# SingleRust/single-algebra

Hardware: AMD Instinct MI355X
Metric: sparse_pca_fit_transform_algorithmic_throughput (higher is better)
Workload: dtype f32

## Files before the change

### single-algebra_amd/csrc/common.h

```cpp
#pragma once
#include <hip/hip_runtime.h>

#include <atomic>
#include <cstdint>
#include <cstdio>
#include <stdexcept>
#include <string>
#include <utility>
#include <vector>

#include "../../include/sapca.h"
#include "switches.h"

namespace sapca {

struct Error : std::runtime_error {
  sapca_status code;
  Error(sapca_status c, const std::string& m) : std::runtime_error(m), code(c) {}
};

#define SAPCA_HIP(expr)                                                                        \
  do {                                                                                         \
    hipError_t e_ = (expr);                                                                    \
    if (e_ != hipSuccess)                                                                      \
      throw ::sapca::Error(SAPCA_ERR_HIP, std::string(#expr) + ": " + hipGetErrorString(e_)); \
  } while (0)

#define SAPCA_CHECK(cond, code, msg)                 \
  do {                                               \
    if (!(cond)) throw ::sapca::Error((code), (msg)); \
  } while (0)

inline int64_t round_up(int64_t x, int64_t q) { return (x + q - 1) / q * q; }

struct DevBuf {
  void* p = nullptr;
  size_t cap = 0;
  DevBuf() = default;
  DevBuf(const DevBuf&) = delete;
  DevBuf& operator=(const DevBuf&) = delete;
  ~DevBuf() { release(); }
  void release() {
    if (p) (void)hipFree(p);
    p = nullptr;
    cap = 0;
  }
  void* ensure(size_t bytes) {
    if (bytes > cap) {
      release();
      size_t want = bytes + bytes / 16 + 256;
      hipError_t e = hipMalloc(&p, want);
      if (e != hipSuccess) {
        p = nullptr;
        throw Error(SAPCA_ERR_NOMEM, std::string("hipMalloc(") + std::to_string(want) + "): " + hipGetErrorString(e));
      }
      cap = want;
    }
    return p;
  }
  template <typename U>
  U* as(size_t count) { return static_cast<U*>(ensure(count * sizeof(U))); }
  template <typename U>
  U* ptr() const { return static_cast<U*>(p); }
  bool contains(const void* q) const {
    const char* c = static_cast<const char*>(q);
    return p != nullptr && c >= static_cast<const char*>(p) && c < static_cast<const char*>(p) + cap;
  }
};

template <typename T>
struct CsrView {
  int64_t rows = 0, cols = 0, nnz = 0;
  const int64_t* ptr = nullptr;
  const int32_t* idx = nullptr;
  const T* val = nullptr;
};

struct LdsAttrState {
  std::atomic<int> bytes[64];
  LdsAttrState() { for (auto& b : bytes) b.store(0, std::memory_order_relaxed); }
};
inline void ensure_dynamic_lds(const void* kernel, size_t bytes, LdsAttrState& state) {
  int dev = 0;
  SAPCA_HIP(hipGetDevice(&dev));
  std::atomic<int>& have = state.bytes[dev & 63];
  if (have.load(std::memory_order_acquire) >= (int)bytes) return;
  SAPCA_HIP(hipFuncSetAttribute(kernel, hipFuncAttributeMaxDynamicSharedMemorySize, (int)bytes));
  have.store((int)bytes, std::memory_order_release);
}

struct PinnedBuf {
  void* p = nullptr;
  size_t cap = 0;
  PinnedBuf() = default;
  PinnedBuf(const PinnedBuf&) = delete;
  PinnedBuf& operator=(const PinnedBuf&) = delete;
  ~PinnedBuf() {
    if (p) (void)hipHostFree(p);
  }
  void* ensure(size_t bytes) {
    if (bytes > cap) {
      if (p) (void)hipHostFree(p);
      p = nullptr;
      cap = 0;
      hipError_t e = hipHostMalloc(&p, bytes, hipHostMallocDefault);
      if (e != hipSuccess) {
        p = nullptr;
        throw Error(SAPCA_ERR_NOMEM, std::string("hipHostMalloc(") + std::to_string(bytes) + "): " + hipGetErrorString(e));
      }
      cap = bytes;
    }
    return p;
  }
};

struct TiledOp {
  bool valid = false;
  int64_t rows = 0, cols = 0, total_entries = 0;
  int ldp = 0;
  int elem = 4;
  int tc = 0, nct = 0;
  int nrb = 0;
  int block_rows = 0;
  int nsplit = 1, tiles_per_split = 0;
  int tile_bytes = 0;
  int64_t max_chunk = 0;
  const int32_t* blk_row0 = nullptr;
  int64_t mid_row0 = -1;
  const uint32_t* row_perm = nullptr;
  const int64_t* chunk_off = nullptr;
  const uint32_t* wave_off = nullptr;
  const uint8_t* steps = nullptr;
  const void* ent = nullptr;
  bool dq = false;
  const uint32_t* dq_info = nullptr;
};
struct TiledBuffers {
  DevBuf blk, steps, wave_off, chunk_off, ent, tmp, misc, perm, lens, dq_info, bounds;
  DevBuf seg;
  DevBuf quad_off;
  DevBuf raw;
  PinnedBuf host;
  hipStream_t aux = nullptr;
  hipEvent_t aux_fork = nullptr, aux_join = nullptr;
  TiledBuffers() = default;
  TiledBuffers(const TiledBuffers&) = delete;
  TiledBuffers& operator=(const TiledBuffers&) = delete;
  ~TiledBuffers() {
    if (aux) { (void)hipStreamSynchronize(aux); (void)hipStreamDestroy(aux); }
    if (aux_fork) (void)hipEventDestroy(aux_fork);
    if (aux_join) (void)hipEventDestroy(aux_join);
  }
};

struct Stream {
  hipStream_t s = nullptr;
  bool owned = false;
};

struct EventTimer {
  bool enabled = false;
  hipStream_t s = nullptr;
  std::vector<hipEvent_t> pool;
  size_t used = 0;
  std::vector<std::pair<int, int>> spans;
  int last_closed = -1;
  void begin_collect(hipStream_t st, bool on) {
    enabled = on;
    s = st;
    used = 0;
    spans.clear();
    last_closed = -1;
  }
  int record() {
    if (used == pool.size()) {
      hipEvent_t e;
      SAPCA_HIP(hipEventCreate(&e));
      pool.push_back(e);
    }
    SAPCA_HIP(hipEventRecord(pool[used], s));
    return (int)used++;
  }
  int start() {
    if (!enabled) return -1;
    spans.emplace_back(record(), -1);
    return (int)spans.size() - 1;
  }
  int start_behind_last() {
    if (!enabled) return -1;
    if (last_closed < 0) return start();
    spans.emplace_back(spans[(size_t)last_closed].second, -1);
    return (int)spans.size() - 1;
  }
  void stop(int i) {
    if (i < 0) return;
    spans[(size_t)i].second = record();
    last_closed = i;
  }
  double ms(int i) {
    if (i < 0 || spans[(size_t)i].second < 0) return 0.0;
    float t = 0;
    SAPCA_HIP(hipEventElapsedTime(&t, pool[(size_t)spans[(size_t)i].first], pool[(size_t)spans[(size_t)i].second]));
    return t;
  }
  ~EventTimer() {
    for (hipEvent_t e : pool) (void)hipEventDestroy(e);
  }
};

}
```

### single-algebra_amd/csrc/engine.cpp

```cpp
#include "engine.h"

#include <algorithm>
#include <chrono>
#include <cmath>
#include <cstring>
#include <exception>
#include <memory>
#include <thread>

#include "lanczos.h"
#include "small_svd.h"
#include "spmm_dq.h"

namespace sapca {

namespace {

template <typename T>
int staged_sweep_ldp(int64_t rows, int64_t cols, double entries, int64_t l, int spmm_variant) {
  if (spmm_variant == 1 || rows <= 0 || cols <= 0 || l < 1 || l > k::kMaxPanelWidth) return 0;
  const int ldp = 64;
  const double row_bytes = (double)ldp * sizeof(T);
  const double tile_bytes = 80.0 * 1024.0, block_rows = row_bytes == 256.0 ? 512.0 : 256.0;
  const double chunks = std::ceil((double)rows / block_rows) * std::ceil((double)cols * row_bytes / tile_bytes);
  double floor_entries = sizeof(T) == 4 ? 1e7 : 5e6;
  if (const char* e = dbg_env("SAPCA_TILED_MIN_ENTRIES")) floor_entries = atof(e);
  const bool dense_enough = entries * (sizeof(T) == 4 ? 64.0 : 96.0) >= chunks * tile_bytes && entries >= floor_entries;
  return (spmm_variant == 2 || dense_enough) ? ldp : 0;
}

enum Cat { C_PREPARE, C_STATS, C_SPMM, C_SPMMT, C_ORTHO, C_SMALL, C_LANCZOS, C_TRANSFORM, C_COMM, C_COUNT };

struct Scope {
  sapca_handle_s& h;
  int ev;
  Scope(sapca_handle_s& h_, int cat, bool behind_last = false) : h(h_), ev(behind_last ? h_.timer.start_behind_last() : h_.timer.start()) {
    if (ev >= 0) h.spans.emplace_back(cat, ev);
  }
  ~Scope() {
    try { h.timer.stop(ev); } catch (...) {}
  }
};

void collect_timings(sapca_handle_s& h, bool is_fit) {
  if (!h.timer.enabled) return;
  sapca_timings& t = h.timings;
  if (is_fit) {
    const double keep_upload = t.upload_ms;
    const uint64_t keep_steps = t.lanczos_steps;
    std::memset(&t, 0, sizeof(t));
    t.upload_ms = keep_upload;
    t.lanczos_steps = keep_steps;
  } else {
    t.transform_ms = 0;
    for (int ev : h.held_small.in_transform) t.transform_ms -= h.timer.ms(ev);
  }
  double comm_dev_ms = 0;
  for (auto& sp : h.spans) {
    if (is_fit == (sp.first == C_TRANSFORM)) continue;
    const double ms = h.timer.ms(sp.second);
    switch (sp.first) {
      case C_PREPARE: t.prepare_ms += ms; break;
      case C_STATS: t.stats_ms += ms; break;
      case C_SPMM:
        t.spmm_ms += ms;
        if (t.n_spmm < 32) t.spmm_sweep_ms[t.n_spmm] = ms;
        t.n_spmm++;
        break;
      case C_SPMMT:
        t.spmmt_ms += ms;
        if (t.n_spmmt < 32) t.spmmt_sweep_ms[t.n_spmmt] = ms;
        t.n_spmmt++;
        break;
      case C_ORTHO: t.ortho_ms += ms; break;
      case C_SMALL: t.small_svd_ms += ms; break;
      case C_LANCZOS: t.lanczos_ms += ms; break;
      case C_TRANSFORM: t.transform_ms += ms; break;
      case C_COMM: comm_dev_ms += ms; break;
      default: break;
    }
  }
  if (is_fit) t.comm_ms = comm_dev_ms > 0 ? comm_dev_ms : h.comm.host_ms;
}

using H = sapca_handle_s;

void lazy_stream(hipStream_t& st, hipEvent_t& a, hipEvent_t& b) {
  if (st) return;
  SAPCA_HIP(hipStreamCreateWithFlags(&st, hipStreamNonBlocking));
  SAPCA_HIP(hipEventCreateWithFlags(&a, hipEventDisableTiming));
  SAPCA_HIP(hipEventCreateWithFlags(&b, hipEventDisableTiming));
}
hipStream_t side_stream(H& h) { lazy_stream(h.stream2, h.ev_fork, h.ev_join); return h.stream2; }
hipStream_t stats_stream(H& h) { lazy_stream(h.stream3, h.ev_kept, h.ev_stats); return h.stream3; }
void order_after(hipStream_t later, hipEvent_t ev, hipStream_t earlier) {
  SAPCA_HIP(hipEventRecord(ev, earlier));
  SAPCA_HIP(hipStreamWaitEvent(later, ev, 0));
}
double* stats_dev(H& h, int64_t n) { return h.stats.as<double>((size_t)3 * n + 1 + H::kStatsTail); }
int panel_ld(int k, int ldp) { return k > 128 ? (int)round_up(k, 64) : std::max(ldp, k <= 64 ? 64 : 128); }

template <typename T>
H::PrepKey prep_key_of(const H& h, const CsrView<T>& A) {
  H::PrepKey key;
  key.ptr = A.ptr; key.idx = A.idx; key.val = A.val;
  key.m = (uint64_t)A.rows; key.n = (uint64_t)A.cols; key.nnz = (uint64_t)A.nnz;
  key.mask_version = h.mask_version; key.dtype = Engine<T>::kDtype; key.valid = true;
  return key;
}

int32_t* upload_o2m(H& h, std::vector<int32_t>& o2m32) {
  const size_t n = h.orig_to_masked.size();
  o2m32.resize(n);
  for (size_t j = 0; j < n; ++j) o2m32[j] = (int32_t)h.orig_to_masked[j];
  int32_t* d_o2m = h.o2m_dev.as<int32_t>(std::max<size_t>(n, 1));
  SAPCA_HIP(hipMemcpyAsync(d_o2m, o2m32.data(), n * sizeof(int32_t), hipMemcpyHostToDevice, h.stream));
  return d_o2m;
}
template <typename T>
H::RawCsr compact_a(H& h, const CsrView<T>& A, const int32_t* d_o2m, int64_t n_used, int32_t* drop_col = nullptr,
                    T* drop_val = nullptr, unsigned long long* amax_bits = nullptr) {
  const CsrBuf<T> ca = csr_buffers<T>(h.ca_ptr, h.ca_idx, h.ca_val, A.rows, A.nnz);
  int64_t nnz_used = 0;
  k::compact_columns(A, d_o2m, ca.ptr, ca.idx, ca.val, &nnz_used, h.scratch, h.stream, drop_col, drop_val, amax_bits);
  return ca.raw(A.rows, n_used, nnz_used);
}

enum class AtFrom { Nothing, FormatFromA, FormatFromCompacted, CompactedTransposed, Transposed };
enum class StatsFrom { Upload, Scatter, FormatBuild, KeptAndDropped, Transposed };
enum class StatsTo { AllReduce, MainCopy, SideChain, ScatterSide };

struct PrepPlan {
  int64_t m = 0, n = 0, nnz = 0, n_used = 0;
  bool masked = false;
  int tiled_ldp = 0;
  int at_nct = 0;
  AtFrom at = AtFrom::Transposed;
  StatsFrom stats = StatsFrom::Transposed;
  StatsTo deliver = StatsTo::MainCopy;
};

template <typename T>
struct PrepOutcome {
  int64_t nnz_used = 0;
  bool at_direct = false;
  bool a_aside = false, ok_a = false;
  CsrView<T> At;
  const uint64_t* at_packed = nullptr;
  bool at_seg_ready = false;
};

struct MaskMaps {
  std::vector<int32_t> o2m32, sel;
  int32_t *d_o2m = nullptr, *d_sel = nullptr;
};

struct Aside {
  std::thread t;
  std::exception_ptr err;
  ~Aside() { if (t.joinable()) t.join(); }
  void join() { if (t.joinable()) t.join(); if (err) std::rethrow_exception(err); }
};

template <typename T>
PrepPlan plan_preparation(H& h, const CsrView<T>& A) {
  PrepPlan p;
  const int64_t m = p.m = A.rows, n = p.n = A.cols, nnz = p.nnz = A.nnz;
  p.masked = !h.mask.empty();
  const int64_t n_used = p.n_used = p.masked ? (int64_t)std::count_if(h.mask.begin(), h.mask.end(), [](uint8_t b) { return b != 0; }) : n;
  if (h.opt.method == SAPCA_RANDOM && m > 0 && n > 0 && n_used > 0) {
    const int64_t l = std::min<int64_t>((int64_t)(h.opt.n_components + h.opt.n_oversamples), std::min<int64_t>(m, n_used));
    p.tiled_ldp = staged_sweep_ldp<T>(m, n_used, (double)nnz * ((double)n_used / (double)n), l, h.opt.spmm_variant);
  }
  const bool at_tile_major = p.tiled_ldp != 0 && dbg_env("SAPCA_AT_NATURAL") == nullptr;
  p.at_nct = at_tile_major ? k::tiled_tile_count(m, p.tiled_ldp * (int)sizeof(T) / 4) : 0;

  bool from_upload = h.up_stats.valid && A.ptr == h.in_ptr.p && A.idx == h.in_idx.p && A.val == h.in_val.p &&
                     h.up_stats.m == (uint64_t)m && h.up_stats.n == (uint64_t)n && h.up_stats.nnz == (uint64_t)nnz &&
                     h.up_stats.dtype == Engine<T>::kDtype && n > 0 && !h.comm.active();
  if (from_upload) {
    SAPCA_HIP(hipEventSynchronize(h.up_stats_done));
    if (*static_cast<const int*>(h.up_stats.flag.p) != 0) h.up_stats.valid = from_upload = false;
  }
  const bool lz_scatter = h.opt.method == SAPCA_LANCZOS && n_used > 0 && n_used <= m && m >= 4096 && nnz > 0 &&
                          k::scatter_fits(n_used) && dbg_env("SAPCA_LANCZOS_TRANSPOSE") == nullptr;
  const bool bucket_route = sizeof(T) == 4 && at_tile_major;
  if (lz_scatter) p.at = AtFrom::Nothing;
  else if (!p.masked) p.at = bucket_route ? AtFrom::FormatFromA : AtFrom::Transposed;
  else p.at = bucket_route && n_used <= 65536 && dbg_env("SAPCA_AT_SORT") == nullptr ? AtFrom::FormatFromCompacted : AtFrom::CompactedTransposed;

  p.stats = from_upload ? StatsFrom::Upload : lz_scatter ? StatsFrom::Scatter : p.masked ? StatsFrom::KeptAndDropped
            : p.at == AtFrom::FormatFromA ? StatsFrom::FormatBuild : StatsFrom::Transposed;
  if (h.comm.active()) p.deliver = StatsTo::AllReduce;
  else if (p.stats == StatsFrom::Scatter) p.deliver = StatsTo::ScatterSide;
  else if (p.stats == StatsFrom::KeptAndDropped && dbg_env("SAPCA_MASK_STATS_INLINE") == nullptr) p.deliver = StatsTo::SideChain;
  return p;
}

void mask_maps(H& h, const PrepPlan& p, MaskMaps& maps) {
  h.cols_to_use.clear();
  h.orig_to_masked.clear();
  h.has_mask_maps = p.masked;
  if (!p.masked) return;
  h.orig_to_masked.assign((size_t)p.n, -1);
  for (int64_t j = 0; j < p.n; ++j)
    if (h.mask[(size_t)j]) {
      h.orig_to_masked[(size_t)j] = (int64_t)h.cols_to_use.size();
      h.cols_to_use.push_back((uint64_t)j);
    }
  if (p.n_used == 0) throw Error(SAPCA_ERR_SVD, "SVD computation failed: the mask selects no feature");
  maps.sel.assign(h.cols_to_use.begin(), h.cols_to_use.end());
  maps.d_o2m = upload_o2m(h, maps.o2m32);
  maps.d_sel = h.sel_rows_dev.as<int32_t>((size_t)p.n_used);
  SAPCA_HIP(hipMemcpyAsync(maps.d_sel, maps.sel.data(), (size_t)p.n_used * sizeof(int32_t), hipMemcpyHostToDevice, h.stream));
}

template <typename T>
void drop_sums(H& h, const PrepPlan& p, int64_t nnz_used, double* dst) {
  const CsrBuf<T> work = csr_buffers<T>(h.at_ptr, h.at_idx, h.at_val, p.n, p.nnz);
  k::sums_by_column(h.drop_col.ptr<int32_t>(), h.drop_val.ptr<T>(), p.nnz - nnz_used, p.n, work.ptr, work.idx, work.val, dst,
                    dst + p.n, h.drop_tmp, h.stream3);
}

template <typename T>
void compact_and_drop_sums(H& h, const CsrView<T>& A, const PrepPlan& p, const MaskMaps& maps, PrepOutcome<T>& out) {
  hipStream_t s = h.stream;
  Scope sc(h, C_PREPARE);
  const bool pairs = p.stats == StatsFrom::KeptAndDropped;
  const size_t cap = (size_t)std::max<int64_t>(p.nnz, 1);
  h.a_used = compact_a(h, A, maps.d_o2m, p.n_used, pairs ? h.drop_col.as<int32_t>(cap) : nullptr, pairs ? h.drop_val.as<T>(cap) : nullptr,
                       p.at == AtFrom::Nothing ? h.lz_scalars.as<unsigned long long>(4) : nullptr);
  out.nnz_used = h.a_used.nnz;
  if (!pairs) return;
  hipStream_t s3 = stats_stream(h);
  if (!h.ev_drop) SAPCA_HIP(hipEventCreateWithFlags(&h.ev_drop, hipEventDisableTiming));
  double* d_stats = stats_dev(h, p.n);
  SAPCA_HIP(hipMemsetAsync(d_stats + 2 * p.n, 0, (size_t)p.n * sizeof(double), s));
  if (p.deliver != StatsTo::SideChain) {
    order_after(s3, h.ev_drop, s);
    drop_sums<T>(h, p, out.nnz_used, d_stats);
    SAPCA_HIP(hipEventRecord(h.ev_drop, s3));
  } else if (h.opt.method != SAPCA_RANDOM) {
    double* d_drop = h.drop_stats.as<double>((size_t)2 * p.n);
    order_after(s3, h.ev_drop, s);
    drop_sums<T>(h, p, out.nnz_used, d_drop);
  }
}

template <typename T>
void start_a_format_aside(H& h, const CsrView<T>& A, const PrepPlan& p, PrepOutcome<T>& out, Aside& aside) {
  side_stream(h);
  SAPCA_HIP(hipEventRecord(h.ev_fork, h.stream));
  h.tiled_a = TiledOp();
  out.a_aside = true;
  const CsrView<T> src = p.masked ? Engine<T>::view(h.a_used) : A;
  aside.t = std::thread([&h, &p, &out, &aside, src] {
    try {
      SAPCA_HIP(hipSetDevice(h.device));
      SAPCA_HIP(hipStreamWaitEvent(h.stream2, h.ev_fork, 0));
      if (p.tiled_ldp != 0) out.ok_a = k::build_tiled(src, p.tiled_ldp, h.tiled_a, h.tb_a, h.stream2, k::QuadSource::csr());
      SAPCA_HIP(hipEventRecord(h.ev_join, h.stream2));
    } catch (...) {
      aside.err = std::current_exception();
    }
  });
}

void scatter_kept_sums(H& h, const PrepPlan& p, const double* d_part, const int32_t* d_sel) {
  double* d_stats = stats_dev(h, p.n);
  if (p.deliver != StatsTo::SideChain) SAPCA_HIP(hipStreamWaitEvent(h.stream, h.ev_drop, 0));
  k::scatter_pairs(d_part, d_part + p.n_used, d_sel, p.n_used, d_stats, d_stats + p.n, h.stream);
}

template <typename T>
void at_format_direct(H& h, const CsrView<T>& A, const PrepPlan& p, const MaskMaps& maps, PrepOutcome<T>& out) {
  if constexpr (sizeof(T) == 4) {
    if (p.masked && out.nnz_used <= 0) return;
    Scope sc(h, C_PREPARE);
    const CsrView<T> src = p.masked ? Engine<T>::view(h.a_used) : A;
    int64_t* t_ptr = (p.masked ? h.cat_ptr : h.at_ptr).template as<int64_t>((size_t)src.cols + 1);
    double* d_sums = p.masked ? h.scratch2.as<double>((size_t)2 * p.n_used + 2) : stats_dev(h, p.n);
    h.tiled_at = TiledOp();
    out.at_direct = k::build_tiled_at_direct(src, p.tiled_ldp, h.tiled_at, h.tb_at, t_ptr,
                                             p.stats == StatsFrom::Upload ? nullptr : d_sums, h.scratch, h.stream);
    if (!out.at_direct) return;
    if (!p.masked) out.At = CsrView<T>{p.n, p.m, p.nnz, t_ptr, nullptr, nullptr};
    else h.at_used = {p.n_used, p.m, out.nnz_used, t_ptr, nullptr, nullptr};
    if (p.stats == StatsFrom::KeptAndDropped) scatter_kept_sums(h, p, d_sums, maps.d_sel);
  }
}

template <typename T>
void at_transpose(H& h, const CsrView<T>& A, const PrepPlan& p, const MaskMaps& maps, PrepOutcome<T>& out) {
  Scope sc(h, C_PREPARE);
  if (p.masked) {
    const CsrBuf<T> cat = csr_buffers<T>(h.cat_ptr, h.cat_idx, h.cat_val, p.n_used, p.nnz);
    k::transpose_csr(Engine<T>::view(h.a_used), cat.ptr, cat.idx, cat.val, h.scratch, h.stream, p.at_nct, nullptr);
    h.at_used = cat.raw(p.n_used, p.m, out.nnz_used);
    if (p.stats != StatsFrom::KeptAndDropped) return;
    double* d_part = h.scratch2.as<double>((size_t)2 * p.n_used + 2);
    k::row_sums(Engine<T>::view(h.at_used), d_part, d_part + p.n_used, h.stream);
    scatter_kept_sums(h, p, d_part, maps.d_sel);
  } else {
    const CsrBuf<T> at = csr_buffers<T>(h.at_ptr, h.at_idx, h.at_val, p.n, p.nnz);
    k::transpose_csr(A, at.ptr, at.idx, at.val, h.scratch, h.stream, p.at_nct,
                     (p.at_nct != 0 && dbg_env("SAPCA_AT_UNPACK") == nullptr) ? &out.at_packed : nullptr);
    out.At = CsrView<T>{p.n, p.m, p.nnz, at.ptr, at.idx, at.val};
  }
}

template <typename T>
void column_statistics(H& h, const CsrView<T>& A, const PrepPlan& p, PrepOutcome<T>& out) {
  hipStream_t s = h.stream;
  const int64_t m = p.m, n = p.n;
  double* sums = static_cast<double*>(h.stats_host.ensure(((size_t)2 * n + 1) * sizeof(double)));
  {
    Scope sc(h, C_STATS);
    double* d_stats = stats_dev(h, n);
    switch (p.stats == StatsFrom::FormatBuild && !out.at_direct ? StatsFrom::Transposed : p.stats) {
      case StatsFrom::Upload:
        SAPCA_HIP(hipMemcpyAsync(d_stats, h.up_stats.out.p, (size_t)3 * n * sizeof(double), hipMemcpyDeviceToDevice, s));
        break;
      case StatsFrom::Scatter: {
        const bool side = p.deliver == StatsTo::ScatterSide;
        hipStream_t st = side ? stats_stream(h) : s;
        if (side) order_after(st, h.ev_kept, s);
        k::colstats_scatter(A, h.lz_scalars.ptr<unsigned long long>(), d_stats, d_stats + n, d_stats + 2 * n, side ? h.drop_tmp : h.scratch, st);
        if (side) {
          SAPCA_HIP(hipMemcpyAsync(sums, d_stats, (size_t)2 * n * sizeof(double), hipMemcpyDeviceToHost, st));
          SAPCA_HIP(hipEventRecord(h.ev_stats, st));
        }
        break;
      }
      case StatsFrom::FormatBuild:
        k::row_lengths_f64(out.At.ptr, n, d_stats + 2 * n, s);
        break;
      case StatsFrom::KeptAndDropped: break;
      case StatsFrom::Transposed:
        if constexpr (sizeof(T) == 4) {
          if (out.at_packed) {
            k::at_stats_index(out.At.ptr, out.at_packed, n, m, p.tiled_ldp, h.tb_at, d_stats, d_stats + n, s);
            out.at_seg_ready = true;
          }
        }
        if (!out.at_seg_ready) k::row_sums(out.At, d_stats, d_stats + n, s);
        k::row_lengths_f64(out.At.ptr, n, d_stats + 2 * n, s);
        break;
    }
    sums[(size_t)2 * n] = (double)m;
    h.stats_on_side = p.deliver == StatsTo::SideChain || p.deliver == StatsTo::ScatterSide;
    if (p.deliver == StatsTo::MainCopy) {
      SAPCA_HIP(hipMemcpyAsync(sums, d_stats, (size_t)2 * n * sizeof(double), hipMemcpyDeviceToHost, s));
    } else if (p.deliver == StatsTo::AllReduce) {
      double* tail = h.stats_tail;
      const uint32_t nr = h.comm.nranks;
      const bool ride = Engine<T>::vote_rides(h);
      const size_t ntail = 1 + (ride ? (size_t)nr + 1 : 0);
      std::fill(tail, tail + ntail, 0.0);
      tail[0] = (double)m;
      if (ride && h.tiled_at.valid) {
        tail[1] = 1.0;
        tail[2 + h.comm.rank] = (double)Engine<T>::piece_vote(h, h.tiled_at.ldp);
      }
      SAPCA_HIP(hipMemcpyAsync(d_stats + 3 * n, tail, ntail * sizeof(double), hipMemcpyHostToDevice, s));
      { Scope cs(h, C_COMM); h.comm.allreduce(d_stats, (uint64_t)3 * n + ntail, 1, s); }
      SAPCA_HIP(hipMemcpyAsync(sums, d_stats, (size_t)2 * n * sizeof(double), hipMemcpyDeviceToHost, s));
      SAPCA_HIP(hipMemcpyAsync(tail, d_stats + 3 * n, ntail * sizeof(double), hipMemcpyDeviceToHost, s));
    }
  }
  h.stats_cols = n;
  h.vote_ready = false;
  if (p.deliver == StatsTo::AllReduce) {
    SAPCA_HIP(hipStreamSynchronize(s));
    sums[(size_t)2 * n] = h.stats_tail[0];
    if (Engine<T>::vote_rides(h) && (uint32_t)std::llround(h.stats_tail[1]) == h.comm.nranks) {
      h.vote_cut = (int64_t)*std::min_element(h.stats_tail + 2, h.stats_tail + 2 + h.comm.nranks);
      h.vote_ready = true;
    }
    h.m_global = (uint64_t)std::llround(sums[(size_t)2 * n]);
    h.stats_pending = false;
    Engine<T>::finish_statistics(h);
  } else {
    h.m_global = (uint64_t)m;
    h.stats_pending = true;
  }
}

template <typename T>
void build_formats(H& h, const PrepPlan& p, PrepOutcome<T>& out, Aside& aside) {
  hipStream_t s = h.stream;
  if (!out.a_aside) h.tiled_a = TiledOp();
  if (!out.at_direct) h.tiled_at = TiledOp();
  if (p.tiled_ldp == 0) return;
  Scope sc(h, C_PREPARE);
  const CsrView<T> at = Engine<T>::view(h.at_used);
  bool ok_at = out.at_direct;
  const k::QuadSource at_rows = p.at_nct != 0 ? k::QuadSource::tile_major() : k::QuadSource::csr();
  if constexpr (sizeof(T) == 4) {
    if (!ok_at)
      ok_at = k::build_tiled(at, p.tiled_ldp, h.tiled_at, h.tb_at, s,
                             out.at_packed ? k::QuadSource::tile_major_packed(out.at_packed, out.at_seg_ready) : at_rows);
    if (out.at_packed && !ok_at) {
      k::unpack_transposed(out.at_packed, p.nnz, const_cast<int32_t*>(out.At.idx), const_cast<float*>(out.At.val), s);
      out.at_packed = nullptr;
      ok_at = k::build_tiled(at, p.tiled_ldp, h.tiled_at, h.tb_at, s, at_rows);
    }
  } else {
    ok_at = k::build_tiled(at, p.tiled_ldp, h.tiled_at, h.tb_at, s, at_rows);
  }
  aside.join();
  const bool ok_a = out.ok_a;
  ok_at = ok_at && ok_a;
  if (h.opt.verbose)
    fprintf(stderr, "sapca: tile-major formats%s: A %s (nrb %d, nct %d, split %d, %lld entries), A^T %s (nrb %d, nct %d, split %d, %lld entries)\n",
            sizeof(T) == 8 ? " (f64)" : "", ok_a ? "ok" : "no", h.tiled_a.nrb, h.tiled_a.nct, h.tiled_a.nsplit,
            (long long)h.tiled_a.total_entries, ok_at ? "ok" : "no", h.tiled_at.nrb, h.tiled_at.nct, h.tiled_at.nsplit,
            (long long)h.tiled_at.total_entries);
  if (ok_a && ok_at) return;
  h.tiled_a = TiledOp();
  h.tiled_at = TiledOp();
  if (out.at_direct) {
    const CsrView<T> src = Engine<T>::view(h.a_used);
    const CsrBuf<T> t = p.masked ? csr_buffers<T>(h.cat_ptr, h.cat_idx, h.cat_val, src.cols, p.nnz)
                                 : csr_buffers<T>(h.at_ptr, h.at_idx, h.at_val, src.cols, p.nnz);
    k::transpose_csr(src, t.ptr, t.idx, t.val, h.scratch, s, 0, nullptr);
    h.at_used = t.raw(src.cols, src.rows, src.nnz);
  }
}

template <typename T>
void queue_side_statistics(H& h, const PrepPlan& p, const PrepOutcome<T>& out, const MaskMaps& maps) {
  const int64_t n = p.n;
  double* d_stats = stats_dev(h, n);
  double* d_drop = h.drop_stats.as<double>((size_t)2 * n);
  order_after(h.stream3, h.ev_kept, h.stream);
  if (h.opt.method == SAPCA_RANDOM) drop_sums<T>(h, p, out.nnz_used, d_drop);
  k::copy_selected(d_stats, d_stats + n, maps.d_sel, p.n_used, d_drop, d_drop + n, h.stream3);
  SAPCA_HIP(hipMemcpyAsync(h.stats_host.p, d_drop, (size_t)2 * n * sizeof(double), hipMemcpyDeviceToHost, h.stream3));
  SAPCA_HIP(hipEventRecord(h.ev_stats, h.stream3));
}

}

template <typename T>
void Engine<T>::prepare(H& h, const CsrView<T>& A) {
  hipStream_t s = h.stream;
  if (!h.mask.empty() && (int64_t)h.mask.size() != A.cols)
    throw Error(SAPCA_ERR_MASK_LEN, "The mask vector length and the number of features (columns) have to be the same!");
  h.prep_key.valid = false;
  if (h.stream3) SAPCA_HIP(hipStreamSynchronize(h.stream3));
  h.stats_pending = false;
  h.stats_on_side = false;
  h.lz_scatter = false;

  const PrepPlan p = plan_preparation(h, A);
  const bool lz_scatter = p.at == AtFrom::Nothing;
  PrepOutcome<T> out;
  MaskMaps maps;
  Aside aside;
  mask_maps(h, p, maps);
  if (lz_scatter && !p.masked) {
    k::absmax(A.val, p.nnz, h.lz_scalars.as<unsigned long long>(4), s);
  }
  h.lz_scatter = lz_scatter;
  if (p.masked) compact_and_drop_sums(h, A, p, maps, out);
  if (p.masked || p.at == AtFrom::FormatFromA) start_a_format_aside(h, A, p, out, aside);
  if (p.at == AtFrom::FormatFromA || p.at == AtFrom::FormatFromCompacted) at_format_direct(h, A, p, maps, out);
  const bool a_aside_late = p.tiled_ldp != 0 && !out.a_aside;
  if (a_aside_late) order_after(side_stream(h), h.ev_fork, s);
  if (!lz_scatter && !out.at_direct) at_transpose(h, A, p, maps, out);
  if (a_aside_late) {
    h.tiled_a = TiledOp();
    out.ok_a = k::build_tiled(A, p.tiled_ldp, h.tiled_a, h.tb_a, h.stream2, k::QuadSource::csr());
    SAPCA_HIP(hipEventRecord(h.ev_join, h.stream2));
    out.a_aside = true;
  }

  column_statistics(h, A, p, out);
  if (!p.masked) {
    h.a_used = {p.m, p.n, p.nnz, A.ptr, A.idx, A.val};
    h.at_used = {p.n, p.m, p.nnz, out.At.ptr, out.At.idx, out.At.val};
  } else if (lz_scatter) {
    h.at_used = {p.n_used, p.m, out.nnz_used, nullptr, nullptr, nullptr};
  }

  build_formats(h, p, out, aside);
  aside.join();
  if (out.a_aside) SAPCA_HIP(hipStreamWaitEvent(s, h.ev_join, 0));
  if (p.deliver == StatsTo::SideChain) queue_side_statistics(h, p, out, maps);

  h.prep_key = prep_key_of(h, A);
}

template <typename T>
void Engine<T>::finish_statistics(H& h) {
  const int64_t n = h.stats_cols;
  const double* sums = static_cast<const double*>(h.stats_host.p);
  const double mg = (double)h.m_global;
  const bool masked = h.has_mask_maps;
  h.prep_mean.assign((size_t)n, 0.0);
  h.prep_total_var = 0;
  if (h.opt.center) {
    for (int64_t j = 0; j < n; ++j) h.prep_mean[(size_t)j] = (double)(T)(sums[(size_t)j] / mg);
    auto var_of = [&](int64_t j) {
      const double mean = sums[(size_t)j] / mg;
      return (sums[(size_t)n + j] - mean * sums[(size_t)j]) / (mg - 1.0);
    };
    if (masked) for (uint64_t j : h.cols_to_use) h.prep_total_var += var_of((int64_t)j);
    else for (int64_t j = 0; j < n; ++j) h.prep_total_var += var_of(j);
  }
  h.q3_cancels = false;
  if (h.opt.center && masked)
    for (uint64_t j : h.cols_to_use) {
      const double sj = sums[(size_t)j], qj = sums[(size_t)n + j];
      if (qj > 0 && sj * sj > 0.25 * mg * qj) { h.q3_cancels = true; break; }
    }
  h.stats_pending = false;
}

template <typename T>
void Engine<T>::normalize(H& h, T* P, int64_t rows, int l, int ld, int normalizer, bool sharded, const NormalizeExtras<T>& x) {
  hipStream_t s = h.stream;
  if (normalizer == SAPCA_NORM_NONE) {
    if (x.src) k::materialize(P, rows, ld, *x.src, s);
    if (x.vec_out) k::weighted_colsum(P, rows, ld, x.w, x.vec_out, h.scratch2, s);
    return;
  }
  Scope sc(h, C_ORTHO, x.behind_sweep);
  const SmallLayout lay(h.small, ld);
  double *G = lay.gram(), *wsum = x.vec_out ? lay.wsum() : nullptr;
  const int passes = x.passes > 0 ? x.passes : (normalizer == SAPCA_NORM_QR ? 2 : 1);
  for (int pass = 0; pass < passes; ++pass) {
    k::gram(P, rows, ld, G, h.scratch2, s, pass == 0 ? x.src : nullptr, x.w, wsum);
    if (sharded && h.comm.active()) { Scope cs(h, C_COMM); h.comm.allreduce(G, (uint64_t)ld * ld, 1, s); }
    double* Rout = pass == 0 ? x.R1 : x.R2;
    k::chol_inv(G, l, ld, Rout ? Rout : lay.r_scratch(), lay.r_inv(), lay.info(), s, wsum,
                sizeof(T) == 4 ? reinterpret_cast<float*>(x.vec_out) : nullptr, sizeof(T) == 8 ? reinterpret_cast<double*>(x.vec_out) : nullptr);
    T* Q = ld <= 128 ? P : h.panel_wide.as<T>((size_t)std::max<int64_t>(rows, 1) * ld);
    k::panel_gemm(P, rows, ld, lay.r_inv(), ld, Q, s, true);
    if (Q != P) SAPCA_HIP(hipMemcpyAsync(P, Q, (size_t)rows * ld * sizeof(T), hipMemcpyDeviceToDevice, s));
  }
}

template <typename T>
bool Engine<T>::vote_rides(const H& h) {
  return sizeof(T) == 4 && h.comm.active() && h.opt.method == SAPCA_RANDOM && h.opt.spmm_variant != 1 &&
         (size_t)h.comm.nranks + 2 <= H::kStatsTail;
}

template <typename T>
int64_t Engine<T>::piece_vote(H& h, int ld) {
  const char* ov = getenv("SAPCA_AT_OVERLAP");
  const bool enabled = ov != nullptr ? atoi(ov) != 0 : h.comm.mode != Comm::RCCL;
  if (!enabled || !h.comm.has_side_lane() || !k::spmm_tiled_pieces_ok(h.tiled_at, 2, ld)) return 0;
  std::vector<int64_t> b;
  k::spmm_tiled_piece_bounds(h.tiled_at, 2, b, h.stream);
  return b[1];
}

namespace {

enum class AtSweep { OnePiece, TwoPieces };
enum class SmallSvd { GramHost, GramHostHeldBack, GramDevice, QrJacobi };

struct AtPieces {
  AtSweep sweep = AtSweep::OnePiece;
  int64_t cut = 0, r1 = 0;
  int wgs = 240;
};
struct RandomizedPlan {
  int64_t m = 0, n_used = 0;
  int l = 0, ld = 0, k = 0, ldk = 0, q = 0;
  int norm = 0, variant = 0;
  bool center = false, tiled = false;
  bool cov = false;
  bool scale = false;
  SmallSvd small = SmallSvd::GramHost;
  AtPieces at;
};

template <typename T>
struct FitPanels {
  T *X, *Y;
  SmallLayout lay;
  const T* mu;
  T *cvec, *sv;
  bool cvec_current = false;
  k::PanelSource<T> src;
  const T *d = nullptr, *dmu = nullptr;
};

template <typename T>
RandomizedPlan plan_randomized(H& h) {
  RandomizedPlan p;
  p.m = h.a_used.rows; p.n_used = h.a_used.cols;
  p.k = (int)h.opt.n_components; p.ldk = (int)round_up(p.k, 16);
  const int64_t l_req = (int64_t)h.opt.n_components + (int64_t)h.opt.n_oversamples;
  p.l = (int)std::min<int64_t>(l_req, std::min<int64_t>((int64_t)h.m_global, p.n_used));
  SAPCA_CHECK(p.l <= k::kMaxPanelWidth, SAPCA_ERR_ARG, "n_components + n_oversamples above 1024 is not supported");
  p.tiled = h.tiled_a.valid && h.tiled_at.valid;
  p.ld = (p.l > 128 || p.tiled || h.comm.active()) ? panel_ld(p.l, p.tiled ? h.tiled_a.ldp : 0) : (int)round_up(p.l, 16);
  p.q = (int)h.opt.n_power_iterations; p.norm = h.opt.normalizer;
  p.cov = h.covar.active();
  p.scale = h.scale_fit != 0;
  p.center = h.opt.center != 0 && !p.cov;
  p.variant = h.opt.spmm_variant;
  p.small = sizeof(T) == 8 ? SmallSvd::QrJacobi : k::sym_eig_device_ok(p.l) ? SmallSvd::GramDevice
            : h.held_small.defer ? SmallSvd::GramHostHeldBack : SmallSvd::GramHost;
  return p;
}

template <typename T>
AtPieces agree_on_at_pieces(H& h, const RandomizedPlan& p) {
  AtPieces at;
  h.at_sweep_pieces = 1u;
  if (sizeof(T) != 4 || !h.comm.active() || p.variant == 1) return at;
  hipStream_t s = h.stream;
  const bool mine = h.tiled_at.valid && k::spmm_tiled_pieces_ok(h.tiled_at, 2, p.ld);
  if (h.vote_ready) {
    at.cut = h.vote_cut;
    SAPCA_CHECK(at.cut == 0 || mine, SAPCA_ERR_COMM, "internal: the ranks agreed on a two-piece A^T sweep this rank cannot run");
  } else {
    const uint32_t nr = h.comm.nranks;
    std::vector<double> votes((size_t)nr, 0.0);
    votes[h.comm.rank] = mine ? (double)Engine<T>::piece_vote(h, p.ld) : 0.0;
    double* d_votes = h.votes.as<double>(nr);
    SAPCA_HIP(hipMemcpyAsync(d_votes, votes.data(), nr * sizeof(double), hipMemcpyHostToDevice, s));
    h.comm.allreduce(d_votes, nr, 1, s);
    SAPCA_HIP(hipMemcpyAsync(votes.data(), d_votes, nr * sizeof(double), hipMemcpyDeviceToHost, s));
    SAPCA_HIP(hipStreamSynchronize(s));
    at.cut = (int64_t)*std::min_element(votes.begin(), votes.end());
  }
  if (!mine || at.cut <= 0 || at.cut >= p.n_used) return at;
  std::vector<int64_t> piece_rows;
  k::spmm_tiled_piece_bounds(h.tiled_at, 2, piece_rows, s);
  at.sweep = AtSweep::TwoPieces;
  at.r1 = piece_rows[1];
  h.at_sweep_pieces = 2u;
  hipDeviceProp_t pr;
  if (hipGetDeviceProperties(&pr, h.device) == hipSuccess) at.wgs = std::max(16, pr.multiProcessorCount - 16);
  lazy_stream(h.stream_comm, h.ev_piece, h.ev_comm);
  return at;
}

template <typename T>
void load_omega(H& h, const RandomizedPlan& p, FitPanels<T>& f) {
  hipStream_t s = h.stream;
  if (h.omega.empty()) {
    k::gaussian_panel(f.X, p.n_used, p.l, p.ld, h.opt.random_seed, s);
    return;
  }
  SAPCA_CHECK((int64_t)h.omega_rows == p.n_used && (int64_t)h.omega_cols >= p.l, SAPCA_ERR_ARG,
              "injected Omega must be (features seen by the SVD) x (n_components + n_oversamples)");
  std::vector<T> tmp((size_t)p.n_used * p.l);
  for (int64_t r = 0; r < p.n_used; ++r)
    for (int j = 0; j < p.l; ++j) tmp[(size_t)r * p.l + j] = (T)h.omega[(size_t)r * h.omega_cols + j];
  T* stage = h.scratch2.as<T>(tmp.size());
  SAPCA_HIP(hipMemcpyAsync(stage, tmp.data(), tmp.size() * sizeof(T), hipMemcpyHostToDevice, s));
  k::add_padding(stage, p.n_used, p.l, f.X, p.ld, s);
  SAPCA_HIP(hipStreamSynchronize(s));
}

template <typename T>
void sweep_a(H& h, const RandomizedPlan& p, FitPanels<T>& f, bool behind_normalize) {
  hipStream_t s = h.stream;
  if (p.scale) {
    Scope sc(h, C_ORTHO, behind_normalize);
    k::scale_panel_rows(f.X, p.n_used, p.ld, f.d, s);
  }
  if (p.center && !f.cvec_current) {
    k::weighted_colsum(f.X, p.n_used, p.ld, f.mu, f.cvec, h.scratch2, s);
    behind_normalize = false;
  }
  f.cvec_current = false;
  Scope sc(h, C_SPMM, behind_normalize);
  k::spmm(Engine<T>::view(h.a_used), &h.tiled_a, f.X, p.ld, f.Y, p.ld, p.ld, p.center ? f.cvec : nullptr, p.variant, h.split_scratch, s);
}

template <typename T>
double* covar_s(H& h, int ld) { return h.covar_s.as<double>((size_t)k::kCovarCols * (size_t)std::max(ld, 16)); }

template <typename T>
void covar_basis_sweep(H& h, const RandomizedPlan& p, FitPanels<T>& f) {
  hipStream_t s = h.stream;
  constexpr int kq = k::kCovarCols;
  T* Q = h.covar_q.as<T>((size_t)p.m * kq);
  SAPCA_HIP(hipMemcpyAsync(Q, h.covar.q_t.data(), (size_t)p.m * kq * sizeof(T), hipMemcpyHostToDevice, s));
  T* Gp = h.panel_xs.as<T>(((size_t)std::max<int64_t>(p.n_used, 1) + 1) * p.ld);
  T* G = h.covar_g.as<T>((size_t)p.n_used * kq);
  k::add_padding(Q, p.m, kq, f.Y, p.ld, s);
  {
    Scope sc(h, C_SPMMT);
    k::spmm(Engine<T>::view(h.at_used), &h.tiled_at, f.Y, p.ld, Gp, p.ld, p.ld, (const T*)nullptr, p.variant, h.split_scratch, s);
  }
  k::strip_padding(Gp, p.n_used, p.ld, kq, G, s);
  if (p.scale) k::scale_panel_rows(G, p.n_used, kq, f.d, s);
}

template <typename T>
void covar_model_products(H& h, const RandomizedPlan& p) {
  hipStream_t s = h.stream;
  constexpr int kq = k::kCovarCols;
  Scope sc(h, C_ORTHO);
  const int ldc = (int)round_up(p.k, p.k > 128 ? 64 : 16);
  h.covar.ldc = ldc;
  T* W = h.panel_w.as<T>((size_t)std::max<int64_t>(p.n_used, 1) * ldc);
  double* C = h.covar_c.as<double>((size_t)kq * ldc);
  double* GG = covar_s<T>(h, kq);
  const T* G = h.covar_g.ptr<T>();
  k::scaled_transpose(h.components_dev.ptr<T>(), p.n_used, p.k, nullptr, W, ldc, s);
  k::panel_qt_y(W, G, p.n_used, ldc, C, h.scratch2, s);
  k::panel_qt_y(G, G, p.n_used, kq, GG, h.scratch2, s);
  void* host = h.covar_host.ensure((size_t)kq * kq * sizeof(double));
  SAPCA_HIP(hipMemcpyAsync(host, GG, (size_t)kq * kq * sizeof(double), hipMemcpyDeviceToHost, s));
}

template <typename T>
void covar_project(H& h, const RandomizedPlan& p, FitPanels<T>& f, bool behind_at) {
  Scope sc(h, C_ORTHO);
  double* S = covar_s<T>(h, p.ld);
  k::panel_qt_y(f.Y, h.covar_q.ptr<T>(), p.m, p.ld, S, h.scratch2, h.stream);
  if (behind_at) k::panel_sub_qs(f.X, h.covar_g.ptr<T>(), p.n_used, p.ld, p.ld, S, p.ld, h.stream);
  else k::panel_sub_qs(f.Y, h.covar_q.ptr<T>(), p.m, p.ld, p.ld, S, p.ld, h.stream);
}

template <typename T>
void sweep_at_one_piece(H& h, const RandomizedPlan& p, FitPanels<T>& f, bool behind_normalize) {
  hipStream_t s = h.stream;
  f.src = k::PanelSource<T>();
  {
    Scope sc(h, C_SPMMT, behind_normalize);
    k::spmm(Engine<T>::view(h.at_used), &h.tiled_at, f.Y, p.ld, f.X, p.ld, p.ld, (const T*)nullptr, p.variant, h.split_scratch, s,
            h.comm.active() || p.cov ? nullptr : &f.src);
  }
  if (!f.src.parts) { f.src.parts = f.X; f.src.nsplit = 1; }
  if (h.comm.active()) {
    Scope cs(h, C_COMM);
    h.comm.allreduce(f.X, (uint64_t)p.n_used * p.ld + (p.center ? (uint64_t)p.ld : 0), Engine<T>::kDtype, s);
  }
  if (p.center) { f.src.mu = f.mu; f.src.sv = f.sv; }
}

template <typename T>
void sweep_at_two_pieces(H& h, const RandomizedPlan& p, FitPanels<T>& f) {
  if constexpr (sizeof(T) == 4) {
    hipStream_t s = h.stream;
    const int64_t cut = p.at.cut, r1 = p.at.r1;
    f.src = k::PanelSource<T>();
    {
      Scope sc(h, C_SPMMT);
      k::spmm_tiled_piece(h.tiled_at, 0, 2, p.at.wgs, 0, r1, f.Y, p.ld, f.X, p.ld, p.ld, h.split_scratch, s);
      SAPCA_HIP(hipEventRecord(h.ev_piece, s));
      k::spmm_tiled_piece(h.tiled_at, 1, 2, p.at.wgs, r1, p.n_used - r1, f.Y, p.ld, f.X, p.ld, p.ld, h.split_scratch2, s);
    }
    Scope cs(h, C_COMM);
    SAPCA_HIP(hipStreamWaitEvent(h.stream_comm, h.ev_piece, 0));
    h.comm.allreduce(f.X, (uint64_t)cut * p.ld, Engine<T>::kDtype, h.stream_comm, 1);
    SAPCA_HIP(hipEventRecord(h.ev_comm, h.stream_comm));
    h.comm.allreduce(f.X + (size_t)cut * p.ld, (uint64_t)(p.n_used - cut) * p.ld + (p.center ? (uint64_t)p.ld : 0), Engine<T>::kDtype, s);
    SAPCA_HIP(hipStreamWaitEvent(s, h.ev_comm, 0));
    f.src.parts = f.X; f.src.nsplit = 1;
    if (p.center) { f.src.mu = f.mu; f.src.sv = f.sv; }
  }
}

template <typename T>
void sweep_at(H& h, const RandomizedPlan& p, FitPanels<T>& f, bool behind_normalize) {
  p.at.sweep == AtSweep::TwoPieces ? sweep_at_two_pieces(h, p, f) : sweep_at_one_piece(h, p, f, behind_normalize);
  if (p.scale) {
    Scope sc(h, C_ORTHO);
    k::finish_scaled_panel(f.X, p.n_used, p.ld, f.src, f.d, h.stream);
    f.src = k::PanelSource<T>();
    f.src.parts = f.X; f.src.nsplit = 1;
  }
  if (p.cov) covar_project(h, p, f, true);
}

template <typename T>
void power_iterations(H& h, const RandomizedPlan& p, FitPanels<T>& f) {
  using Extras = NormalizeExtras<T>;
  T* const sv_out = p.center ? f.sv : nullptr;
  const bool y_behind = !p.cov, x_behind = !p.cov && !p.scale && !h.comm.active() && p.at.sweep != AtSweep::TwoPieces;
  const bool normalises = p.norm != SAPCA_NORM_NONE;
  for (int it = 0; it < p.q; ++it) {
    sweep_a(h, p, f, it > 0 && normalises);
    if (p.cov) covar_project(h, p, f, false);
    Engine<T>::normalize(h, f.Y, p.m, p.l, p.ld, p.norm, true, Extras{.passes = 1, .vec_out = sv_out, .behind_sweep = y_behind});
    sweep_at(h, p, f, normalises);
    Engine<T>::normalize(h, f.X, p.n_used, p.l, p.ld, p.norm, false,
                         Extras{.passes = 1, .src = &f.src, .w = p.scale ? f.dmu : f.mu, .vec_out = p.center ? f.cvec : nullptr,
                                .behind_sweep = x_behind});
    f.cvec_current = p.center;
  }
  sweep_a(h, p, f, p.q > 0 && normalises);
  if (p.cov) covar_project(h, p, f, false);
  Engine<T>::normalize(h, f.Y, p.m, p.l, p.ld, SAPCA_NORM_QR, true, Extras{.vec_out = sv_out, .behind_sweep = y_behind});
  sweep_at(h, p, f, true);
}

template <typename T>
void rotate_into_components(H& h, int ld, const double* Mdev, const double** sign_out = nullptr) {
  const int k = (int)h.opt.n_components, ldk = (int)round_up(k, 16);
  const int64_t n_used = h.a_used.cols;
  T* VtT = h.panel_w.as<T>((size_t)std::max<int64_t>(n_used, 1) * ldk);
// ... 144 lines not shown
    h.sing.assign(sv.begin(), sv.begin() + k);
    h.chol_regularised = info_host;
  } catch (...) {
    if (deferred) {
      h.fitted = false;
      h.held_tail.pending = false;
    }
    throw;
  }
}

template <typename T>
void Engine<T>::fit_lanczos(H& h, bool centred) {
  Scope sc(h, C_LANCZOS);
  lanczos_fit<T>(h, centred);
}

void covar_check(H& h, uint64_t m, bool fit, bool then_transform) {
  const bool set = !h.covar_z.empty();
  const bool model = h.covar.model.design > 0;
  if (!fit) {
    if (!h.fitted || (!set && !model)) return;
    SAPCA_CHECK(model, SAPCA_ERR_ARG, "transform: covariates are set, but the model was fitted without covariates");
    SAPCA_CHECK(set, SAPCA_ERR_ARG, "transform: the model was fitted with covariates, but none are set");
    SAPCA_CHECK(h.covar_cols == h.covar.model.cols, SAPCA_ERR_ARG,
                "transform: covariates have " + std::to_string(h.covar_cols) + " columns, the fitted model's " + std::to_string(h.covar.model.cols));
  }
  if (!set) return;
  SAPCA_CHECK(!h.comm.active(), SAPCA_ERR_ARG, "covariates are not supported on a handle that belongs to a communicator");
  SAPCA_CHECK(h.opt.method == SAPCA_RANDOM, SAPCA_ERR_ARG, "covariates need SVDMethod::Random");
  SAPCA_CHECK(!(then_transform || !fit) || h.opt.transform_semantics == SAPCA_TRANSFORM_CENTERED, SAPCA_ERR_ARG,
              "covariates need SAPCA_TRANSFORM_CENTERED: the reference's transform semantics have no meaning on residuals");
  SAPCA_CHECK(h.covar_rows == m, SAPCA_ERR_ARG,
              "covariates have " + std::to_string(h.covar_rows) + " rows, the matrix " + std::to_string(m));
}

void scale_check(H& h, uint64_t m, uint64_t n, bool fit, bool then_transform) {
  const int mode = fit ? h.scale_mode : (h.fitted ? h.scale_model : 0);
  if (mode == SAPCA_SCALE_NONE) return;
  if (fit) {
    SAPCA_CHECK(h.opt.method == SAPCA_RANDOM, SAPCA_ERR_ARG, "column scaling needs SVDMethod::Random");
    if (mode == SAPCA_SCALE_WEIGHTS)
      SAPCA_CHECK(h.scale_weights.size() == n, SAPCA_ERR_ARG,
                  "column scaling has " + std::to_string(h.scale_weights.size()) + " weights, the matrix " + std::to_string(n) + " columns");
    if (mode == SAPCA_SCALE_UNIT_VARIANCE) {
      SAPCA_CHECK(m >= 2 || h.comm.active(), SAPCA_ERR_ARG,
                  "column scaling: unit variance needs at least two rows, the matrix has " + std::to_string(m));
      SAPCA_CHECK(h.covar_z.empty(), SAPCA_ERR_ARG,
                  "column scaling: unit variance of covariate residuals is not supported (" + std::to_string(h.covar_cols) +
                      " covariate columns are set): pass explicit weights");
    }
  }
  SAPCA_CHECK(!(then_transform || !fit) || h.opt.transform_semantics == SAPCA_TRANSFORM_CENTERED, SAPCA_ERR_ARG,
              "column scaling needs SAPCA_TRANSFORM_CENTERED: the reference's transform semantics have no meaning on scaled columns");
}

namespace {

template <typename T>
void column_scale_factors(H& h, int64_t n_used) {
  hipStream_t s = h.stream;
  const int64_t n = h.stats_cols;
  const double* weights = nullptr;
  if (h.scale_fit == SAPCA_SCALE_WEIGHTS) {
    double* w = h.scale_in.as<double>((size_t)std::max<int64_t>(n, 1));
    SAPCA_HIP(hipMemcpyAsync(w, h.scale_weights.data(), (size_t)n * sizeof(double), hipMemcpyHostToDevice, s));
    weights = w;
  }
  const size_t cap = (size_t)std::max<int64_t>(n_used, 1), parts = k::column_scale_partials(n_used);
  double* red = h.scale_red.as<double>(parts + 1);
  const double* stats = h.stats.ptr<double>();
  k::column_scale_factors<T>(stats, stats + n, (double)h.m_global, h.has_mask_maps ? h.sel_rows_dev.ptr<int32_t>() : nullptr, weights, n_used,
                             h.scale_d64.as<double>(cap), h.scale_dt.as<T>(cap), h.scale_w.as<T>(cap), red, red + parts, s);
  void* host = h.scale_host.ensure(sizeof(double));
  SAPCA_HIP(hipMemcpyAsync(host, red + parts, sizeof(double), hipMemcpyDeviceToHost, s));
}

template <typename T>
void covar_fit_basis(H& h) {
  constexpr size_t kq = k::kCovarCols;
  H::Covar& c = h.covar;
  c.fit = {};
  if (h.covar_z.empty()) return;
  const size_t m = (size_t)h.covar_rows, design = (size_t)h.covar_cols + (h.opt.center ? 1 : 0);
  c.q.resize(m * kq);
  c.w.resize(design * kq);
  uint64_t rank = 0;
  SAPCA_CHECK(sapca_covariate_basis(h.covar_z.data(), h.covar_rows, h.covar_cols, h.opt.center ? 1 : 0, c.q.data(), c.w.data(), &rank) == SAPCA_OK,
              SAPCA_ERR_ARG, "covariates: the design matrix was refused");
  c.fit = {h.covar_cols, (uint64_t)design, rank};
  c.q_t.resize(m * kq * sizeof(T));
  T* qt = reinterpret_cast<T*>(c.q_t.data());
  for (size_t i = 0; i < m * kq; ++i) qt[i] = (T)c.q[i];
}

template <typename T>
void covar_rows_basis(H& h) {
  constexpr size_t kq = k::kCovarCols;
  H::Covar& c = h.covar;
  const size_t m = (size_t)h.covar_rows, cols = (size_t)h.covar_cols, off = h.opt.center ? 1 : 0;
  c.q_t.resize(m * kq * sizeof(T));
  T* qt = reinterpret_cast<T*>(c.q_t.data());
  for (size_t i = 0; i < m; ++i)
    for (size_t j = 0; j < kq; ++j) {
      double acc = off ? c.w_model[j] : 0.0;
      for (size_t t = 0; t < cols; ++t) acc += h.covar_z[i * cols + t] * c.w_model[(off + t) * kq + j];
      qt[i * kq + j] = (T)acc;
    }
}

void covar_finish_fit(H& h) {
  constexpr size_t kq = k::kCovarCols;
  H::Covar& c = h.covar;
  if (c.fit.design == 0) return;
  c.w_model = c.w;
  if (!c.active() || !h.opt.center) return;
  const double* GG = static_cast<const double*>(h.covar_host.p);
  const double* sums = static_cast<const double*>(h.stats_host.p);
  const size_t n = (size_t)h.stats_cols;
  double raw = 0, taken = 0;
  const bool scaled = h.scale_model == SAPCA_SCALE_WEIGHTS && h.scale_weights.size() == n;
  auto moment = [&](size_t j) { return scaled ? h.scale_weights[j] * h.scale_weights[j] * sums[n + j] : sums[n + j]; };
  if (h.has_mask_maps) for (uint64_t j : h.cols_to_use) raw += moment((size_t)j);
  else for (size_t j = 0; j < n; ++j) raw += moment(j);
  for (size_t i = 0; i < kq; ++i) taken += GG[i * kq + i];
  h.total_var = (raw - taken) / (double)(h.m_fit - 1);
}

}

template <typename T>
void Engine<T>::fit(H& h, const CsrView<T>& A, bool defer_finish) {
  hipStream_t s = h.stream;
  covar_check(h, (uint64_t)A.rows, true, false);
  scale_check(h, (uint64_t)A.rows, (uint64_t)A.cols, true, false);
  h.scale_fit = h.scale_mode;
  h.held_tail.reset();
  h.held_small.reset();
  covar_fit_basis<T>(h);
  {
    const double lw = (double)(h.opt.n_components + h.opt.n_oversamples) <= 64 ? 64.0 : 128.0;
    h.held_small.defer = defer_finish && h.mask.empty() && h.opt.method == SAPCA_RANDOM && sizeof(T) == 4 &&
                         (h.comm.active() || (double)A.rows * lw * lw <= 400e3 * 64.0 * 64.0) && !h.covar.active() && h.scale_fit == 0;
  }
  h.spans.clear();
  h.comm.host_ms = 0;
  h.timer.begin_collect(s, h.opt.collect_timings != 0);
  const int total_ev = h.timer.start();
  h.fitted = false;
  h.timings.lanczos_steps = 0;
  SAPCA_CHECK(h.opt.n_components > 0, SAPCA_ERR_ARG, "n_components must be positive");
  SAPCA_CHECK(A.rows > 0 && A.cols > 0, SAPCA_ERR_ARG, "empty matrix");
  prepare(h, A);
  const int64_t n_used = h.a_used.cols;
  if ((int64_t)h.opt.n_components > std::min<int64_t>((int64_t)h.m_global - (int64_t)h.covar.fit.rank, n_used))
    throw Error(SAPCA_ERR_SVD, std::string(h.opt.method == SAPCA_RANDOM ? "Randomized SVD" : "SVD") +
                                   " computation failed: n_components exceeds the matrix dimensions");
  SAPCA_CHECK(h.m_global >= 2, SAPCA_ERR_ARG, "need at least two samples");

  auto device_means = [&] {
    T* d_mu = h.mean_used_dev.as<T>((size_t)n_used);
    if (h.opt.center)
      k::mean_from_sums(h.stats.ptr<double>(), (double)h.m_global, h.has_mask_maps ? h.sel_rows_dev.ptr<int32_t>() : nullptr, n_used, d_mu, s);
    else
      SAPCA_HIP(hipMemsetAsync(d_mu, 0, (size_t)n_used * sizeof(T), s));
  };

  if (h.opt.method == SAPCA_RANDOM) {
    device_means();
    if (h.scale_fit) column_scale_factors<T>(h, n_used);
    fit_randomized(h);
  } else {
    const bool centred = h.opt.lanczos_center != 0 && h.opt.center != 0;
    const bool sums_on_side = h.lz_scatter && h.stats_on_side;
    const bool means_first = !sums_on_side || centred;
    if (sums_on_side && centred) SAPCA_HIP(hipStreamWaitEvent(s, h.ev_stats, 0));
    if (means_first) device_means();
    if (centred)
      k::mean_from_sums(h.stats.ptr<double>(), (double)h.m_global, h.has_mask_maps ? h.sel_rows_dev.ptr<int32_t>() : nullptr, n_used,
                        h.lz_mu.as<double>((size_t)n_used), s);
    fit_lanczos(h, centred);
    if (!means_first) {
      SAPCA_HIP(hipStreamWaitEvent(s, h.ev_stats, 0));
      device_means();
    }
  }

  h.k = h.opt.n_components;
  h.n_used = (uint64_t)n_used;
  h.n_cols = (uint64_t)A.cols;
  h.m_fit = h.m_global;
  h.dtype = kDtype;
  h.fitted = true;
  h.scale_model = h.scale_fit;
  h.covar.model = h.covar.fit;
  h.timer.stop(total_ev);
  h.held_tail.total_ev = total_ev;
  h.held_tail.pending = true;
  if (!defer_finish || !h.mask.empty() || h.covar.fit.design > 0) finish_fit(h);
}

namespace {

template <typename T>
void describe_sweeps(H& h) {
  const int64_t n_used = (int64_t)h.n_used;
  const double l = (double)std::min<uint64_t>(h.opt.n_components + h.opt.n_oversamples, std::min<uint64_t>(h.m_global, (uint64_t)n_used));
  h.timings.bytes_per_sweep = (double)h.a_used.nnz * (sizeof(T) + 4) + ((double)h.a_used.rows + 1) * 8 +
                              (double)n_used * l * sizeof(T) + (double)h.a_used.rows * l * sizeof(T);
  const bool tiled = h.opt.method == SAPCA_RANDOM && h.tiled_a.valid && h.tiled_at.valid;
  h.timings.sweep_kernel = !tiled ? 0u : (k::dq_usable(h.tiled_a, 64) && k::dq_usable(h.tiled_at, 64) && h.opt.spmm_variant != 1 ? 2u : 1u);
  h.timings.at_sweep_pieces = h.opt.method == SAPCA_RANDOM ? h.at_sweep_pieces : 0u;
  h.timings.sweep_slots_a = tiled ? (uint64_t)h.tiled_a.total_entries : 0;
  h.timings.sweep_slots_at = tiled ? (uint64_t)h.tiled_at.total_entries : 0;
}

}

template <typename T>
void Engine<T>::finish_fit(H& h) {
  if (!h.held_tail.pending) return;
  if (h.held_small.pending) finish_small_svd(h, nullptr);
  h.held_tail.pending = false;
  hipStream_t s = h.stream;
  const int total_ev = h.held_tail.total_ev;
  if (h.held_tail.sing_l) {
    const int l = h.held_tail.sing_l;
    h.held_tail.sing_l = 0;
    SAPCA_HIP(hipStreamSynchronize(s));
    const double* host = static_cast<const double*>(h.small_host.p);
    const int* host_i = reinterpret_cast<const int*>(host + l);
    bool finite = true;
    for (int i = 0; i < l; ++i) finite = finite && std::isfinite(host[i]);
    if ((host_i[0] & 1) || (host_i[0] & 2) || !finite) {
      h.fitted = false;
      throw Error(SAPCA_ERR_SVD, (host_i[0] & 1) ? "Randomized SVD computation failed: eigensolver did not converge"
                                                 : "Randomized SVD computation failed: non-finite singular value");
    }
    if (h.opt.verbose) fprintf(stderr, "sapca: device eigensolver of the %d x %d Gram: %d sweeps\n", l, l, host_i[1]);
    h.sing.assign(host, host + h.k);
    h.chol_regularised = host_i[2];
  }
  if (h.stats_pending) {
    SAPCA_HIP(hipStreamSynchronize(s));
    if (h.stats_on_side) SAPCA_HIP(hipEventSynchronize(h.ev_stats));
    finish_statistics(h);
  }
  h.mean = h.prep_mean;
  const double nm1 = (double)(h.m_fit - 1);
  h.expl_var.resize(h.k);
  for (uint64_t i = 0; i < h.k; ++i) {
    const T sv = (T)h.sing[i];
    h.expl_var[i] = (double)(T)((T)(sv * sv) / (T)nm1);
  }
  if (h.opt.center) {
    h.total_var = h.prep_total_var;
  } else {
    h.total_var = 0;
    for (uint64_t i = 0; i < h.k; ++i) h.total_var += h.expl_var[i];
  }
  SAPCA_HIP(hipStreamSynchronize(s));
  if (h.scale_model && h.opt.center) h.total_var = *static_cast<const double*>(h.scale_host.p);
  covar_finish_fit(h);
  collect_timings(h, true);
  if (total_ev >= 0) h.timings.fit_total_ms = h.timer.ms(total_ev);
  describe_sweeps<T>(h);
}

namespace {

template <typename T>
struct Projection {
  CsrView<T> Au;
  const TiledOp* top = nullptr;
  int ldk = 0;
  double* d_cnt = nullptr;
  bool prepared = false;
};

template <typename T>
Projection<T> select_projection_operator(H& h, const CsrView<T>& A) {
  hipStream_t s = h.stream;
  const int k = (int)h.k;
  const bool masked = !h.mask.empty(), ref_sem = h.opt.transform_semantics == SAPCA_TRANSFORM_REFERENCE;
  Projection<T> pr;
  pr.ldk = (int)round_up(k, 16);
  pr.prepared = h.prep_key == prep_key_of(h, A);
  if (pr.prepared) {
    if (h.tiled_a.valid && k <= k::kMaxPanelWidth) pr.top = &h.tiled_a;
    pr.Au = Engine<T>::view(h.a_used);
    pr.d_cnt = h.stats.ptr<double>() + 2 * A.cols;
  } else if (masked) {
    h.prep_key.valid = false;
    std::vector<int32_t> o2m32;
    pr.Au = Engine<T>::view(compact_a(h, A, upload_o2m(h, o2m32), (int64_t)h.n_used));
  } else {
    pr.Au = A;
    if (ref_sem) {
      h.prep_key.valid = false;
      pr.d_cnt = stats_dev(h, A.cols) + 2 * A.cols;
      k::column_counts_f64(A.idx, A.nnz, A.cols, pr.d_cnt, h.scratch, s);
      if (h.comm.active()) h.comm.allreduce(pr.d_cnt, (uint64_t)A.cols, 1, s);
    }
  }
  if (!pr.prepared && k <= k::kMaxPanelWidth && pr.Au.nnz > 0) {
    const int ldp_t = staged_sweep_ldp<T>(pr.Au.rows, pr.Au.cols, (double)pr.Au.nnz, k, h.opt.spmm_variant);
    if (ldp_t != 0) {
      h.prep_key.valid = false;
      h.tiled_at = TiledOp();
      h.tiled_a = TiledOp();
      if (k::build_tiled(pr.Au, ldp_t, h.tiled_a, h.tb_a, s, k::QuadSource::csr()) && h.tiled_a.valid) pr.top = &h.tiled_a;
      else h.tiled_a = TiledOp();
    }
  }
  if (pr.top) pr.ldk = panel_ld(k, pr.top->ldp);
  return pr;
}

template <typename T>
void project_unrotated(H& h, const Projection<T>& pr, T* d_out) {
  hipStream_t s = h.stream;
  const int ld = h.held_small.ld, k = (int)h.k;
  const int64_t m = pr.Au.rows, n_used = (int64_t)h.n_used;
  const bool center = h.opt.center != 0, ref_sem = h.opt.transform_semantics == SAPCA_TRANSFORM_REFERENCE;
  const SmallLayout lay(h.small, ld);
  T* cvec = lay.c<T>();
  T* Xs = h.panel_xs.as<T>((size_t)n_used * ld);
  T* Tp = h.panel_y.as<T>((size_t)m * ld);
  k::scale_rows(h.panel_x.ptr<T>(), n_used, ld, ref_sem ? pr.d_cnt : nullptr, Xs, s);
  if (center) k::weighted_colsum(Xs, n_used, ld, h.mean_used_dev.ptr<T>(), cvec, h.scratch2, s);
  k::spmm(pr.Au, h.tiled_a.valid ? &h.tiled_a : nullptr, Xs, ld, Tp, ld, ld, center ? cvec : nullptr, h.opt.spmm_variant, h.split_scratch, s);
  const double* sign = nullptr;
  Engine<T>::finish_small_svd(h, &sign);
  const int ldm = (int)round_up(k, 16);
  k::scale_columns(lay.m(), ld, ldm, k, sign, s);
  k::panel_gemm(Tp, m, ld, lay.m(), ldm, d_out, s, false, k, k);
}

template <typename T>
void project_with_components(H& h, const Projection<T>& pr, T* d_out, bool uncentred = false) {
// ... 83 lines not shown
```

### single-algebra_amd/csrc/engine.h

```cpp
#pragma once
#include <algorithm>
#include <string>
#include <vector>

#include "comm.h"
#include "common.h"
#include "kernels.h"

struct sapca_handle_s {
  sapca_options opt{};
  std::string err;
  int device = 0;
  hipStream_t stream = nullptr;
  bool own_stream = false;
  hipStream_t stream2 = nullptr;
  hipEvent_t ev_fork = nullptr, ev_join = nullptr, ev_drop = nullptr;
  hipStream_t stream3 = nullptr;
  hipStream_t stream_comm = nullptr;
  hipEvent_t ev_piece = nullptr, ev_comm = nullptr;
  hipEvent_t ev_kept = nullptr, ev_stats = nullptr;
  bool stats_on_side = false;

  std::vector<uint8_t> mask;
  uint64_t mask_version = 0;
  std::vector<double> omega;
  size_t omega_rows = 0, omega_cols = 0;

  std::vector<double> covar_z;
  uint64_t covar_rows = 0, covar_cols = 0;
  struct Covar {
    struct Shape { uint64_t cols = 0, design = 0, rank = 0; };
    Shape fit, model;
    std::vector<double> q, w;
    std::vector<double> w_model;
    int ldc = 0;
    std::vector<unsigned char> q_t;
    bool active() const { return fit.rank > 0; }
  } covar;
  sapca::DevBuf covar_q, covar_g, covar_s;
  sapca::DevBuf covar_c;
  sapca::PinnedBuf covar_host;

  int scale_mode = 0;
  std::vector<double> scale_weights;
  int scale_fit = 0, scale_model = 0;
  sapca::DevBuf scale_in, scale_d64, scale_dt, scale_w, scale_red;
  sapca::PinnedBuf scale_host;

  bool fitted = false;
  int dtype = 0;
  uint64_t k = 0, n_used = 0, n_cols = 0, m_fit = 0;
  std::vector<double> sing, expl_var, mean;
  double total_var = 0;
  std::vector<uint64_t> cols_to_use;
  std::vector<int64_t> orig_to_masked;
  bool has_mask_maps = false;
  int chol_regularised = 0;

  struct PrepKey {
    const void *ptr = nullptr, *idx = nullptr, *val = nullptr;
    uint64_t m = 0, n = 0, nnz = 0, mask_version = 0;
    int dtype = -1;
    bool valid = false;
    bool operator==(const PrepKey& o) const {
      return valid && o.valid && ptr == o.ptr && idx == o.idx && val == o.val && m == o.m && n == o.n && nnz == o.nnz &&
             mask_version == o.mask_version && dtype == o.dtype;
    }
  } prep_key;
  struct RawCsr {
    int64_t rows = 0, cols = 0, nnz = 0;
    const void *ptr = nullptr, *idx = nullptr, *val = nullptr;
  } a_used, at_used;
  uint64_t m_global = 0;
  std::vector<double> prep_mean;
  double prep_total_var = 0;
  uint32_t at_sweep_pieces = 1;
  bool lz_scatter = false;
  bool q3_cancels = false;
  sapca::PinnedBuf stats_host;
  sapca::PinnedBuf small_host;
  struct HeldTail {
    bool pending = false;
    int total_ev = -1;
    int sing_l = 0;
    void reset() { pending = false; sing_l = 0; }
  } held_tail;
  struct HeldSmall {
    bool defer = false, pending = false;
    int l = 0, ld = 0;
    hipEvent_t ev = nullptr;
    std::vector<int> in_transform;
    void reset() { defer = pending = false; in_transform.clear(); }
  } held_small;
  sapca::PinnedBuf lanczos_host;
  bool stats_pending = false;
  int64_t stats_cols = 0;
  static constexpr size_t kStatsTail = 72;
  double stats_tail[kStatsTail] = {};
  bool vote_ready = false;
  int64_t vote_cut = 0;

  sapca::DevBuf in_ptr, in_idx, in_val, up64, out_tmp;
  sapca::PinnedBuf up_stage[2];
  hipEvent_t up_done[2] = {nullptr, nullptr};
  struct UpStats {
    sapca::DevBuf work, out;
    sapca::PinnedBuf flag;
    uint64_t m = 0, n = 0, nnz = 0;
    int dtype = -1;
    bool valid = false;
  } up_stats;
  hipEvent_t up_stats_done = nullptr;
  void values_changed() { prep_key.valid = false; up_stats.valid = false; }
  template <typename R>
  void drop_preparation_of(const R& result) {
    if (prep_key.valid && (result.owns(prep_key.ptr) || result.owns(prep_key.idx) || result.owns(prep_key.val))) prep_key.valid = false;
  }
  struct Selection {
    sapca::DevBuf ptr, idx, val, rows, scan, gather, spans, cmap;
    bool owns(const void* q) const { return ptr.contains(q) || idx.contains(q) || val.contains(q); }
  } selection;
  struct Canonical {
    sapca::DevBuf ptr, idx, val, idx2, val2, ctr, rows, long_off, keys, scan;
    bool owns(const void* q) const {
      return ptr.contains(q) || idx.contains(q) || val.contains(q) || idx2.contains(q) || val2.contains(q);
    }
  } canonical;
  struct Knn {
    sapca::DevBuf unit_q, unit_c, bias, part_sc, part_ix, merged;
  } knn;
  struct Tsne {
    sapca::DevBuf p, raw_ptr, nvalid, cursor, raw_idx, raw_val, scan, ctr, rows, long_off, keys, sort_idx, sort_val, out_ptr, out_val;
    sapca::DevBuf part, rep, sum_part, scal, klrow, grad, v, gain, colpart, knn_idx, knn_dist, x, y;
    bool owns(const void* q) const {
      return raw_ptr.contains(q) || out_ptr.contains(q) || raw_idx.contains(q) || sort_idx.contains(q) || out_val.contains(q);
    }
  } tsne;
  struct Kmeans {
    sapca::DevBuf bias, xb, amb, lab0, lab1, cnt, tab, scan, order, partial, shiftpart, ctl, scal, rowd, sum_part, colpart, cols;
    sapca::DevBuf rows, seed_dist, seed_bsum, x, cen, labels;
  } kmeans;
  struct Umap {
    sapca::DevBuf p, raw_ptr, nvalid, cursor, raw_idx, raw_val, scan, ctr, rows, long_off, keys, sort_idx, sort_val, out_ptr, out_val;
    sapca::DevBuf rowsum, sum_part, scal, next, nextn, y2, minmax, knn_idx, knn_dist, x, y;
    bool owns(const void* q) const {
      return raw_ptr.contains(q) || out_ptr.contains(q) || raw_idx.contains(q) || sort_idx.contains(q) || out_val.contains(q);
    }
  } umap;
  struct Louvain {
    sapca::DevBuf lists, long_off, ctr, keys, skeys, k, srow, sq, sum_part, tot0, tot1, lab0, lab1, anchored, ctl, scan;
    sapca::DevBuf flag, renum, cnt, rawcnt, pos, raw_ptr, raw_idx, raw_val, lists2, long_off2, keys2, cnt2;
    sapca::DevBuf agg_ptr[2], agg_idx[2], agg_val[2], in_ptr, in_idx, in_val, labels;
    bool owns(const void* q) const {
      return agg_ptr[0].contains(q) || agg_idx[0].contains(q) || agg_val[0].contains(q) || agg_ptr[1].contains(q) ||
             agg_idx[1].contains(q) || agg_val[1].contains(q);
    }
  } louvain;
  struct Rank {
    sapca::DevBuf group, out, list, scratch;
  } rank;
  sapca::DevBuf at_ptr, at_idx, at_val;
  sapca::DevBuf ca_ptr, ca_idx, ca_val, cat_ptr, cat_idx, cat_val;
  sapca::DevBuf drop_stats, drop_tmp;
  sapca::DevBuf drop_col, drop_val;
  sapca::DevBuf scratch, scratch2;
  sapca::DevBuf panel_x, panel_y, panel_w, panel_xs, panel_wide;
  sapca::DevBuf small;
  sapca::DevBuf stats;
  sapca::DevBuf batch_in, batch_out;
  sapca::DevBuf mean_used_dev, o2m_dev, sel_rows_dev;
  sapca::DevBuf components_dev;
  sapca::DevBuf lanczos_buf;
  sapca::DevBuf lz_mu;
  sapca::DevBuf idx16_a, idx16_b;
  sapca::TiledBuffers tb_a, tb_at;
  sapca::TiledOp tiled_a, tiled_at;
  sapca::DevBuf split_scratch, split_scratch2, votes, lz_scalars;

  sapca::EventTimer timer;
  std::vector<std::pair<int, int>> spans;
  sapca_timings timings{};
  sapca::Comm comm;
};

namespace sapca {

struct SmallLayout {
  size_t ld, W;
  double* base;
  SmallLayout(DevBuf& buf, int ld_, size_t behind = 0)
      : ld((size_t)ld_), W((size_t)std::max(ld_, 128)), base(buf.as<double>(6 * W * W + 64 + 4 * W + behind)) {}
  double* slot(size_t i) const { return base + i * ld * ld; }
  double* gram() const { return slot(0); }
  double* r_inv() const { return slot(1); }
  double* r_scratch() const { return slot(2); }
  double* r1() const { return slot(3); }
  double* r2() const { return slot(4); }
  double* m() const { return slot(5); }
  int* info() const { return reinterpret_cast<int*>(base + 6 * W * W); }
  template <typename T> T* c() const { return reinterpret_cast<T*>(base + 6 * W * W + 64); }
  template <typename T> T* s() const { return c<T>() + W; }
  double* wsum() const { return base + 6 * W * W + 64 + 2 * W; }
  double* behind() const { return base + 6 * W * W + 64 + 4 * W; }
};

template <typename T>
struct CsrBuf {
  int64_t* ptr; int32_t* idx; T* val;
  sapca_handle_s::RawCsr raw(int64_t rows, int64_t cols, int64_t nnz) const { return {rows, cols, nnz, ptr, idx, val}; }
};
template <typename T>
CsrBuf<T> csr_buffers(DevBuf& ptr, DevBuf& idx, DevBuf& val, int64_t rows, int64_t cap) {
  const size_t entries = (size_t)std::max<int64_t>(cap, 1);
  return {ptr.as<int64_t>((size_t)rows + 1), idx.as<int32_t>(entries), val.as<T>(entries)};
}

template <typename T>
CsrView<T> transpose_into_at(sapca_handle_s& h, const CsrView<T>& A) {
  h.prep_key.valid = false;
  const CsrBuf<T> at = csr_buffers<T>(h.at_ptr, h.at_idx, h.at_val, A.cols, A.nnz);
  k::transpose_csr(A, at.ptr, at.idx, at.val, h.scratch, h.stream);
  return CsrView<T>{A.cols, A.rows, A.nnz, at.ptr, at.idx, at.val};
}

void covar_check(sapca_handle_s& h, uint64_t m, bool fit, bool then_transform);
void scale_check(sapca_handle_s& h, uint64_t m, uint64_t n, bool fit, bool then_transform);

template <typename T>
struct NormalizeExtras {
  double *R1 = nullptr, *R2 = nullptr;
  int passes = 0;
  const k::PanelSource<T>* src = nullptr;
  const T* w = nullptr;
  T* vec_out = nullptr;
  bool behind_sweep = false;
};

template <typename T>
struct Engine {
  using H = sapca_handle_s;
  static constexpr int kDtype = sizeof(T) == 8 ? 1 : 0;
  static void prepare(H& h, const CsrView<T>& A);
  static void finish_statistics(H& h);
  static void fit(H& h, const CsrView<T>& A, bool defer_finish = false);
  static void finish_small_svd(H& h, const double** sign_out);
  static void finish_fit(H& h);
  static void transform(H& h, const CsrView<T>& A, T* d_out);
  static void fit_randomized(H& h);
  static void fit_lanczos(H& h, bool centred);
  static bool vote_rides(const H& h);
  static int64_t piece_vote(H& h, int ld);
  static void normalize(H& h, T* P, int64_t rows, int l, int ld, int normalizer, bool sharded, const NormalizeExtras<T>& x);
  static CsrView<T> view(const H::RawCsr& r) {
    CsrView<T> v;
    v.rows = r.rows; v.cols = r.cols; v.nnz = r.nnz;
    v.ptr = static_cast<const int64_t*>(r.ptr);
    v.idx = static_cast<const int32_t*>(r.idx);
    v.val = static_cast<const T*>(r.val);
    return v;
  }
};

}
```

### single-algebra_amd/csrc/kernels.h

```cpp
#pragma once
#include <vector>
#include "common.h"

namespace sapca {
namespace k {

template <typename T>
struct PanelSource {
  const T* parts = nullptr;
  int nsplit = 0;
  int64_t slab_stride = 0;
  const T* mu = nullptr;
  const T* sv = nullptr;
};

void narrow_indices(const uint64_t* ptr64, const uint64_t* idx64, int64_t m, int64_t nnz, int64_t n,
                    int64_t* ptr, int32_t* idx, int* flag, hipStream_t s);
template <typename T>
void transpose_csr(const CsrView<T>& A, int64_t* t_ptr, int32_t* t_idx, T* t_val, DevBuf& scratch, hipStream_t s,
                   int tile_major_nct = 0,
                   const uint64_t** packed_rows_out = nullptr);
void unpack_transposed(const uint64_t* packed, int64_t nnz, int32_t* t_idx, float* t_val, hipStream_t s);
template <typename T>
void row_sums(const CsrView<T>& At, double* sum, double* sumsq, hipStream_t s);
template <typename T>
void compact_columns(const CsrView<T>& A, const int32_t* o2m, int64_t* new_ptr, int32_t* new_idx, T* new_val,
                     int64_t* new_nnz_host, DevBuf& scratch, hipStream_t s, int32_t* drop_col = nullptr, T* drop_val = nullptr,
                     unsigned long long* amax_bits = nullptr);
template <typename T>
void sums_by_column(const int32_t* cols, const T* vals, int64_t count, int64_t n, int64_t* seg, int32_t* keys_out, T* vals_out,
                    double* sum, double* sumsq, DevBuf& scratch, hipStream_t s);
template <typename T> size_t exact_colstats_bytes(int64_t n);
template <typename T> void exact_colstats_reset(void* work, int64_t n, hipStream_t s);
template <typename T> void exact_colstats_scan_values(const T* val, int64_t count, int64_t n, void* work, hipStream_t s);
template <typename T>
void exact_colstats_scan_rows(const int64_t* ptr, const T* val, int64_t rows, const uint32_t* row_bits, int64_t n, void* work,
                              hipStream_t s);
template <typename T>
void exact_colstats_add(const int64_t* ptr, const int32_t* idx, const T* val, int64_t r_lo, int64_t r_hi, int64_t e_lo, int64_t e_hi,
                        int64_t n, void* work, hipStream_t s, const uint32_t* row_bits = nullptr);
template <typename T> void exact_colstats_finish(void* work, int64_t n, double* out, int* nonfinite_host, hipStream_t s);
void copy_selected(const double* a, const double* b, const int32_t* where, int64_t count, double* out_a, double* out_b, hipStream_t s);
void scatter_pairs(const double* a, const double* b, const int32_t* where, int64_t count, double* out_a, double* out_b, hipStream_t s);
template <typename T>
void mean_from_sums(const double* sum, double count, const int32_t* sel, int64_t n_used, T* mu, hipStream_t s);
void row_lengths_f64(const int64_t* ptr, int64_t rows, double* out, hipStream_t s);
void column_counts_f64(const int32_t* idx, int64_t nnz, int64_t n, double* out, DevBuf& scratch, hipStream_t s);

template <typename T>
void normalize_csr(const CsrView<T>& A, T* values, const double* d_sums, double target, bool by_column, double* d_scale,
                   hipStream_t s);
template <typename T>
void log1p_values(T* values, int64_t nnz, hipStream_t s);
template <typename T>
void row_stats(const CsrView<T>& A, bool from_first_value, double* sum, double* sumsq, T* minv, T* maxv, hipStream_t s);

int batch_codes_per_launch();
template <typename T>
void batch_row_stats(const CsrView<T>& R, const int32_t* codes, int lo, int nb, double* sum, double* m2, uint32_t* cnt, hipStream_t s);
template <typename T>
void row_top_n(const CsrView<T>& A, const uint64_t* ns, int n_ns, double* out, hipStream_t s);

void rank_group_sizes(const int32_t* labels, int64_t m, int nk, unsigned long long* group, hipStream_t s);
template <typename T>
void rank_count_nonzero(const CsrView<T>& At, const int32_t* labels, int nk, uint32_t* cnt, hipStream_t s);
template <typename T>
void rank_sums_lds(const CsrView<T>& At, const int32_t* labels, int nk, const unsigned long long* group, int64_t M, long long* rs,
                   uint32_t* cnt, double* tie, hipStream_t s);
template <typename T>
void rank_sums_long(const CsrView<T>& At, const int32_t* labels, int nk, const unsigned long long* group, int64_t M,
                    const int32_t* cols_list, const uint32_t* seg, int nseg, uint32_t total, DevBuf& scratch, long long* rs, uint32_t* cnt,
                    double* tie, hipStream_t s);

template <typename T>
void masked_row_stats(const CsrView<T>& A, const uint32_t* col_bits, double* sum, double* sumsq, double* m2, uint32_t* cnt,
                      hipStream_t s);

void exclusive_scan_i64(int64_t* data, int64_t count, DevBuf& scratch, size_t scratch_offset, hipStream_t s,
                        int64_t* out = nullptr);
void select_rows_offsets(const int64_t* ptr, const uint64_t* rows, int64_t n_rows, int64_t* out_ptr, int64_t* total_host,
                         DevBuf& scratch, hipStream_t s);
template <typename T>
void select_rows_fill(const CsrView<T>& A, const uint64_t* rows, int64_t n_rows, const int64_t* out_ptr, int64_t total,
                      int32_t* out_idx, T* out_val, hipStream_t s);

int64_t select_submatrix_spans(int64_t gtotal);
template <typename T>
void select_submatrix_count(const CsrView<T>& A, const uint64_t* rows, int64_t n_rows, const int64_t* goff, int64_t gtotal,
                            const uint32_t* cmap, bool drop_zeros, int64_t* span_cnt, hipStream_t s);
template <typename T>
void select_submatrix_fill(const CsrView<T>& A, const uint64_t* rows, int64_t n_rows, const int64_t* goff, int64_t gtotal,
                           const uint32_t* cmap, bool drop_zeros, const int64_t* span_base, int64_t* out_ptr, int32_t* out_idx,
                           T* out_val, hipStream_t s);

enum CanonCtr {
  kCtrFirstBadOffset = 0, kCtrFirstOutOfRange, kCtrFirstUnsorted, kCtrFirstDuplicate, kCtrFirstNonfinite, kCtrFirstCount,
  kCtrColsOutOfRange = kCtrFirstCount, kCtrUnsortedRows, kCtrDuplicates, kCtrNonfinite, kCtrStoredZeros,
  kCtrListWave, kCtrListLds, kCtrListLong,
  kCtrLongEntries,
  kCtrMerged,
  kCtrSlots = 16
};
void canon_check_offsets(const int64_t* ptr, int64_t m, int64_t nnz, unsigned long long* ctr, hipStream_t s);
template <typename T>
void canon_check_entries(const CsrView<T>& A, uint32_t* row_bits, unsigned long long* ctr, hipStream_t s);
void canon_list_rows(const int64_t* ptr, const uint32_t* row_bits, int64_t m, uint32_t* lists, unsigned long long* long_off,
                     unsigned long long* ctr, hipStream_t s);
int64_t canon_lds_cap();
template <typename T>
void canon_sort_rows(const CsrView<T>& A, const uint32_t* lists, const unsigned long long* long_off, const int64_t counts[3],
                     unsigned long long* key_space, int32_t* out_idx, T* out_val, uint32_t* distinct, unsigned long long* ctr,
                     hipStream_t s);
void canon_new_lengths(const int64_t* ptr, const uint32_t* row_bits, const uint32_t* distinct, int64_t m, int64_t* new_ptr,
                       hipStream_t s);
template <typename T>
void canon_merge_fill(const int64_t* ptr, const int32_t* idx, const T* val, int64_t m, const int64_t* new_ptr, int32_t* out_idx,
                      T* out_val, hipStream_t s);

void stream_copy16(const void* src, void* dst, int64_t bytes, hipStream_t s);

template <typename T>
void spmm(const CsrView<T>& A, const TiledOp* tiled, const T* X, int ldx, T* Y, int ldy, int ncols,
          const T* cvec, int variant, DevBuf& scratch, hipStream_t s, PanelSource<T>* keep = nullptr);

template <typename T>
void spmm_rows_shifted(const CsrView<T>& A, const T* X, int ldx, T* Y, int ldy, int ncols, const T* shift, hipStream_t s);

bool scatter_fits(int64_t cols);
template <typename T>
void absmax(const T* v, int64_t count, unsigned long long* out_bits, hipStream_t s);
void vecmax(const double* y, int64_t len, unsigned long long* out_bits, hipStream_t s);
template <typename T>
void spmvt_scatter(const CsrView<T>& A, const uint16_t* idx16, const double* y, const unsigned long long* amax_bits,
                   const unsigned long long* ymax_bits, unsigned long long* clear_bits, double* z, DevBuf& scratch, hipStream_t s);
template <typename T>
void colstats_scatter(const CsrView<T>& A, const unsigned long long* amax_bits, double* sum, double* sumsq, double* cnt, DevBuf& scratch,
                      hipStream_t s);

struct AtDirectSrc;
struct QuadSource {
  enum Kind {
    Csr,
    TileMajorCsr,
    TileMajorPacked,
    FromA
  };
  Kind kind = Csr;
  const uint64_t* packed = nullptr;
  bool seg_ready = false;
  const AtDirectSrc* from_a = nullptr;
  static QuadSource csr() { return QuadSource(); }
  static QuadSource tile_major() {
    QuadSource q;
    q.kind = TileMajorCsr;
    return q;
  }
  static QuadSource tile_major_packed(const uint64_t* packed, bool seg_ready) {
    QuadSource q;
    q.kind = TileMajorPacked;
    q.packed = packed;
    q.seg_ready = seg_ready;
    return q;
  }
};
bool build_tiled(const CsrView<float>& S, int ldp, TiledOp& op, TiledBuffers& buf, hipStream_t s, const QuadSource& src);
bool build_tiled(const CsrView<double>& S, int ldp, TiledOp& op, TiledBuffers& buf, hipStream_t s, const QuadSource& src);
bool build_tiled_at_direct(const CsrView<float>& A, int ldp, TiledOp& op, TiledBuffers& buf, int64_t* at_ptr, double* stats,
                           DevBuf& scratch, hipStream_t s);
void at_stats_index(const int64_t* ptr, const uint64_t* packed, int64_t rows, int64_t cols, int ldp, TiledBuffers& buf,
                    double* sum, double* sumsq, hipStream_t s);
int tiled_tile_count(int64_t cols, int ldp);

void spmm_tiled(const TiledOp& op, const float* X, int ldx, float* Y, int ldy, int ncols, const float* cvec, DevBuf& scratch,
                hipStream_t s, PanelSource<float>* keep = nullptr);
bool spmm_tiled_pieces_ok(const TiledOp& op, int npieces, int ldx);
void spmm_tiled_piece_bounds(const TiledOp& op, int npieces, std::vector<int64_t>& bounds, hipStream_t s);
void spmm_tiled_piece(const TiledOp& op, int piece, int npieces, int wgs, int64_t first_row, int64_t row_count, const float* X, int ldx, float* Y,
                      int ldy, int ncols, DevBuf& scratch, hipStream_t s);
void spmm_tiled(const TiledOp& op, const double* X, int ldx, double* Y, int ldy, int ncols, const double* cvec, DevBuf& scratch,
                hipStream_t s, PanelSource<double>* keep = nullptr);

constexpr int kMaxPanelWidth = 1024;

template <typename T>
void materialize(T* P, int64_t rows, int ld, const PanelSource<T>& src, hipStream_t s);
template <typename T>
void gram(T* P, int64_t rows, int ld, double* G, DevBuf& scratch, hipStream_t s, const PanelSource<T>* src = nullptr, const T* w = nullptr,
          double* wsum = nullptr);
void chol_inv(const double* G, int l, int ld, double* R, double* Rinv, int* info, hipStream_t s, const double* wsum = nullptr,
              float* vec32 = nullptr, double* vec64 = nullptr);

bool sym_eig_device_ok(int l);
void sym_eig_device(const double* G, int l, int ld, int k, int ldk, double* M, double* sigma, int* status, hipStream_t s);
template <typename T>
void panel_gemm(const T* P, int64_t rows, int ld, const double* M, int ldo, T* out, hipStream_t s, bool upper = false, int out_stride = 0,
                int out_cols = 0);
template <typename T>
void weighted_colsum(const T* P, int64_t rows, int ld, const T* w, T* out, DevBuf& scratch, hipStream_t s);
template <typename T>
void rank1_subtract(T* Z, int64_t rows, int ld, const T* mu, const T* svec, hipStream_t s);
template <typename T>
void flip_transpose(const T* VtT, int64_t n, int ld, int k, T* components, DevBuf& scratch, hipStream_t s, const double** sign_out = nullptr);
template <typename T>
void scale_rows(const T* P, int64_t rows, int ld, const double* scale, T* out, hipStream_t s);
void scale_columns(double* M, int rows, int ld, int k, const double* sign, hipStream_t s);
template <typename T>
void scaled_transpose(const T* comps, int64_t n, int k, const double* scale, T* W, int ld, hipStream_t s);
template <typename T>
void fill_zero(T* p, int64_t count, hipStream_t s);
template <typename T>
void convert_from_f64(const double* in, T* out, int64_t count, hipStream_t s);
template <typename T>
void strip_padding(const T* in, int64_t rows, int ld, int ncols, T* out, hipStream_t s);
template <typename T>
void add_padding(const T* in, int64_t rows, int ncols, T* out, int ld, hipStream_t s);

constexpr int kCovarCols = 16;
template <typename T>
void panel_qt_y(const T* Y, const T* Q, int64_t rows, int ld, double* S, DevBuf& scratch, hipStream_t s);
template <typename T>
void panel_sub_qs(T* Y, const T* Q, int64_t rows, int ld, int ncols, const double* S, int lds, hipStream_t s);

size_t column_scale_partials(int64_t n_used);
template <typename T>
void column_scale_factors(const double* sum, const double* sumsq, double m, const int32_t* sel, const double* weights, int64_t n_used,
                          double* d64, T* dt, T* w, double* part, double* total, hipStream_t s);
template <typename T>
void scale_panel_rows(T* P, int64_t rows, int ld, const T* d, hipStream_t s);
template <typename T>
void finish_scaled_panel(T* P, int64_t rows, int ld, const PanelSource<T>& src, const T* d, hipStream_t s);

struct KnnPlan {
  int mt = 1, nsplit = 1, tiles_per_split = 1;
  size_t lds_bytes = 0;
};
template <typename T>
KnnPlan knn_plan(int64_t mq, int64_t mc, int k, int n_cus);
template <typename T>
void knn_prepare(const T* x, int64_t ld, int64_t rows, int d, int metric, T* unit, T* bias, hipStream_t s);
template <typename T>
void knn_select(const T* q, int64_t ldq, int64_t mq, const T* c, int64_t ldc, int64_t mc, const T* bias, int d, int metric, int k,
                bool exclude_self, const KnnPlan& plan, T* part_sc, int32_t* part_ix, hipStream_t s);
template <typename T>
void knn_merge(const T* part_sc, const int32_t* part_ix, int64_t mq, int nsplit, int k, int32_t* merged, hipStream_t s);
template <typename T>
void knn_refine(const T* q, int64_t ldq, int64_t mq, const T* c, int64_t ldc, int64_t mc, int d, int metric, const int32_t* sel,
                int64_t sel_stride, int k, int32_t* out_ix, T* out_val, hipStream_t s);

template <typename T>
void tsne_perplexity(const int32_t* idx, const T* dist, int64_t m, int K, double perplexity, double* p, double* beta, hipStream_t s);
void tsne_count(const int32_t* idx, int64_t m, int K, int64_t* len, int32_t* nvalid, hipStream_t s);
void tsne_emit(const int32_t* idx, const double* p, int64_t m, int K, const int64_t* ptr, const int32_t* nvalid, int32_t* cursor,
               int32_t* out_idx, double* out_val, hipStream_t s);
template <typename T>
void tsne_scale(const double* in, int64_t nnz, double inv, T* out, hipStream_t s);
struct TsnePlan {
  int nchunk = 1, tiles_per_chunk = 1;
  bool split = false;
};
TsnePlan tsne_plan(int64_t m, int n_cus);
size_t tsne_sum_parts(int64_t n);
template <typename T>
void tsne_repulsion(const T* y, int64_t ldy, int64_t m, int D, const TsnePlan& plan, double* part, double* rep, double* sum_part, double* z,
                    hipStream_t s);
template <typename T>
void tsne_attraction(const CsrView<T>& P, const T* y, int64_t ldy, int D, double exaggeration, const double* rep, const double* z, T* grad,
                     double* klrow, hipStream_t s);
void tsne_sum(const double* in, int64_t n, double* sum_part, double* out, hipStream_t s);
template <typename T>
void tsne_update(T* y, T* v, T* gain, const T* grad, int64_t m, int D, double momentum, double rate, double* colpart, double* mean,
                 hipStream_t s);
template <typename T>
void tsne_center(T* y, int64_t m, int D, double* colpart, double* mean, bool sum_first, hipStream_t s);
template <typename T>
void tsne_init_state(T* y_or_null, T* v, T* gain, int64_t m, int D, uint32_t seed, hipStream_t s);

template <typename T>
void umap_row_sums(const int32_t* idx, const T* dist, int64_t m, int K, double* rowsum, hipStream_t s);
template <typename T>
void umap_smooth(const int32_t* idx, const T* dist, int64_t m, int K, int n_neighbors, const double* total, double* a, double* sigma,
                 double* rho, hipStream_t s);
template <typename T>
void umap_union_fill(const int64_t* ptr, const int32_t* idx, const double* val, int64_t m, const int64_t* new_ptr, int32_t* out_idx,
                     T* out_val, hipStream_t s);
template <typename T>
void umap_schedule(const T* val, int64_t nnz, int rate, double* wmax, double* next, double* nextn, hipStream_t s);
template <typename T>
void umap_init_panel(const T* x, int64_t ldx, int64_t m, int D, double* minmax, T* y, hipStream_t s);
template <typename T>
void umap_init_random(T* y, int64_t m, int D, uint32_t seed, hipStream_t s);
struct UmapEpoch {
  uint64_t epoch = 0, seed = 0;
  double n_epochs = 1, alpha = 0, a = 1, b = 1, gamma = 1, rate = 0;
};
template <typename T>
void umap_epoch(const CsrView<T>& G, const T* y_in, T* y_out, int D, const UmapEpoch& p, const double* wmax, double* next, double* nextn,
                hipStream_t s);

enum { kKmDone = 0, kKmStrict = 1, kKmIter = 2, kKmChanged = 3, kKmAmbiguous = 4, kKmCtlWords = 8 };
struct KmeansPlan {
  int64_t rows_per_wave = 256, nwaves = 1;
  int slices = 1;
};
KmeansPlan kmeans_plan(int64_t m, int k);
int kmeans_column_slices(int64_t m);
template <typename T>
void kmeans_seed(const T* x, int64_t ldx, int64_t m, int d, int k, uint32_t seed, T* cen, int32_t* rows, double* dist, double* bsum,
                 hipStream_t s);
template <typename T>
void kmeans_rank(const unsigned long long* skip, const T* x, int64_t ldx, int64_t m, const T* cen, int k, const T* bias, const T* xb, int d,
                 int32_t* labels, int32_t* amb_list, unsigned long long* ctl, hipStream_t s);
template <typename T>
void kmeans_refine(const unsigned long long* skip, const T* x, int64_t ldx, int64_t m, const T* cen, int k, int d, int32_t* labels,
                   const int32_t* amb_list, const unsigned long long* ctl, hipStream_t s);
template <typename T>
void kmeans_distances(const T* x, int64_t ldx, int64_t m, const T* cen, int k, int d, const int32_t* labels, T* dist2, double* rowd,
                      hipStream_t s);
void kmeans_sort(const unsigned long long* skip, const int32_t* labels, int64_t m, int k, const KmeansPlan& plan, int64_t* cnt,
                 int64_t* tab, int32_t* order, DevBuf& scan, const int32_t* prev, unsigned long long* ctl, hipStream_t s);
template <typename T>
void kmeans_sums(const unsigned long long* skip, const T* x, int64_t ldx, int64_t m, int d, const int32_t* order, const int64_t* tab,
// ... 58 lines not shown
```

### single-algebra_amd/csrc/tiled_build.hip

```cpp
#include <algorithm>
#include <cmath>
#include <cstdio>
#include <cstdlib>
#include <cstring>
#include <vector>

#include <rocprim/rocprim.hpp>

#include "kernels.h"
#include "quad_format.h"
#include "spmm_dq.h"

namespace sapca {
namespace k {

namespace {

__device__ __forceinline__ void divmod_small(int c, int d, float inv, int& q, int& r) {
  q = (int)((float)c * inv);
  r = c - q * d;
  if (r < 0) { r += d; --q; }
  if (r >= d) { r -= d; ++q; }
}

// ... 131 lines not shown
  const int rb = lo;
  const int lr = (int)(sp - blk_row0[rb]);
  const int qd = lr >> 2;
  const uint32_t g = (uint32_t)(lr & 3);
  const int64_t* __restrict__ coff = chunk_off + (int64_t)rb * nct;
  const uint32_t* __restrict__ qoff = quad_off + ((int64_t)rb * Q_BLOCK_QUADS + qd) * nct;
  const int64_t block_base = coff[0];
  for (int t = lane; t < nct; t += WAVE) cnt[t] = (uint32_t)(coff[t] - block_base) + qoff[t] + g;
  __builtin_amdgcn_wave_barrier();
  const int64_t e0 = ptr[r], e1 = ptr[r + 1];
  E* __restrict__ out = ent + block_base;
  for (int64_t eb = e0; eb < e1; eb += 8 * WAVE) {
    int c[8];
    VT v[8];
#pragma unroll
    for (int u = 0; u < 8; ++u) {
      const int64_t e = eb + u * WAVE + lane;
      c[u] = e < e1 ? idx[e] : -1;
      v[u] = e < e1 ? val[e] : (VT)0;
    }
#pragma unroll
    for (int u = 0; u < 8; ++u) {
      if (c[u] >= 0) {
        int i, t;
        divmod_small(c[u], nct, inv_nct, i, t);
        E x = E();
        x.off = (uint32_t)i * (uint32_t)ldp_bytes;
        x.val = v[u];
        out[atomicAdd(&cnt[t], 4u)] = x;
      }
      __builtin_amdgcn_wave_barrier();
    }
  }
}

constexpr int QF_CAP_MIN = 4096, QF_CAP_MAX = 6144;
template <typename VT>
__device__ __forceinline__ void quad_fill_staged_one(int qi, uint32_t* qf_lds, const int64_t* __restrict__ ptr, const int32_t* __restrict__ idx,
                                                     const VT* __restrict__ val, const int32_t* __restrict__ seg,
                                                     const int32_t* __restrict__ blk_row0, const uint32_t* __restrict__ perm, int nct, int cap,
                                                     float inv_nct, int ldp_bytes, const int64_t* __restrict__ chunk_off,
                                                     const uint32_t* __restrict__ quad_off, typename EntOf<VT>::type* __restrict__ ent) {
  typedef typename EntOf<VT>::type E;
  constexpr int EW = (int)sizeof(E) / 4;
  E* stage = reinterpret_cast<E*>(qf_lds);
  int64_t* gofs = reinterpret_cast<int64_t*>(qf_lds + EW * cap);
  uint32_t* lofs = qf_lds + EW * cap + 2 * nct;
  uint32_t* cnt_all = lofs + nct + 1;
  const int rb = qi / Q_BLOCK_QUADS, qd = qi % Q_BLOCK_QUADS;
  const int row0 = blk_row0[rb], nrows = blk_row0[rb + 1] - row0;
  if (4 * qd >= nrows) return;
  const int wave = threadIdx.x / WAVE, lane = threadIdx.x & (WAVE - 1);
  const int qrows = min(4, nrows - 4 * qd);
  const int64_t s0 = (int64_t)row0 + 4 * qd;
  int64_t rowof[4];
#pragma unroll
  for (int g = 0; g < 4; ++g) rowof[g] = g < qrows ? (perm ? (int64_t)perm[s0 + g] : s0 + g) : 0;
  const int64_t* __restrict__ coff = chunk_off + (int64_t)rb * nct;
  const uint32_t* __restrict__ qoff = quad_off + ((int64_t)rb * Q_BLOCK_QUADS + qd) * nct;
  for (int t = threadIdx.x; t < nct; t += 256) {
    int mx = 0;
    for (int g = 0; g < qrows; ++g) {
      const int32_t* sg = seg + rowof[g] * (nct + 1);
      mx = max(mx, sg[t + 1] - sg[t]);
    }
    lofs[t + 1] = (uint32_t)q_steps(mx) * 4u;
    gofs[t] = coff[t] + (int64_t)qoff[t];
    for (int g = 0; g < 4; ++g) cnt_all[g * nct + t] = 0;
  }
  if (threadIdx.x == 0) lofs[0] = 0;
  __syncthreads();
  if (wave == 0) {
    uint32_t carry = 0;
    for (int t0 = 0; t0 < nct; t0 += WAVE) {
      const int t = t0 + lane;
      const uint32_t v = t < nct ? lofs[t + 1] : 0u;
      uint32_t x = v;
#pragma unroll
      for (int off = 1; off < WAVE; off <<= 1) {
        const uint32_t y = __shfl_up(x, off);
        if (lane >= off) x += y;
      }
      if (t < nct) lofs[t + 1] = carry + x;
      carry += __shfl(x, WAVE - 1);
    }
  }
  __syncthreads();
  const uint32_t total = lofs[nct];
  const bool staged = total <= (uint32_t)cap;
  if (staged) {
    uint64_t* z = reinterpret_cast<uint64_t*>(stage);
    for (uint32_t i = threadIdx.x; i < total * (EW / 2); i += 256) z[i] = 0;
  } else {
    if (wave < qrows) {
      const int32_t* sg = seg + rowof[wave] * (nct + 1);
      for (int t = lane; t < nct; t += WAVE) {
        const uint32_t steps = (lofs[t + 1] - lofs[t]) / 4u;
        E* dst = ent + gofs[t];
        for (uint32_t k = (uint32_t)(sg[t + 1] - sg[t]); k < steps; ++k) dst[k * 4u + wave] = E();
      }
    } else {
      for (int t = lane; t < nct; t += WAVE) {
        const uint32_t steps = (lofs[t + 1] - lofs[t]) / 4u;
        E* dst = ent + gofs[t];
        for (uint32_t k = 0; k < steps; ++k) dst[k * 4u + wave] = E();
      }
    }
  }
  __syncthreads();
  if (wave < qrows) {
    const int64_t r = rowof[wave];
    const int64_t e0 = ptr[r], e1 = ptr[r + 1];
    uint32_t* cnt = cnt_all + (size_t)wave * nct;
    for (int64_t eb = e0; eb < e1; eb += 8 * WAVE) {
      int c[8];
      VT v[8];
#pragma unroll
      for (int u = 0; u < 8; ++u) {
        const int64_t e = eb + u * WAVE + lane;
        c[u] = e < e1 ? idx[e] : -1;
        v[u] = e < e1 ? val[e] : (VT)0;
      }
#pragma unroll
      for (int u = 0; u < 8; ++u) {
        if (c[u] >= 0) {
          int i, t;
          divmod_small(c[u], nct, inv_nct, i, t);
          E x = E();
          x.off = (uint32_t)i * (uint32_t)ldp_bytes;
          x.val = v[u];
          const uint32_t k = atomicAdd(&cnt[t], 1u);
          if (staged) stage[lofs[t] + k * 4u + (uint32_t)wave] = x;
          else ent[gofs[t] + k * 4u + (uint32_t)wave] = x;
        }
        __builtin_amdgcn_wave_barrier();
      }
    }
  }
  if (!staged) return;
  __syncthreads();
  for (int t = wave; t < nct; t += 4) {
    const uint32_t lo = lofs[t], n = lofs[t + 1] - lo;
    E* dst = ent + gofs[t];
    for (uint32_t j = lane; j < n; j += WAVE) dst[j] = stage[lo + j];
  }
}

template <typename VT>
__global__ void __launch_bounds__(256)
quad_fill_staged_kernel(const int64_t* __restrict__ ptr, const int32_t* __restrict__ idx, const VT* __restrict__ val,
                        const int32_t* __restrict__ seg, const int32_t* __restrict__ blk_row0,
                        const uint32_t* __restrict__ perm, int nct, int cap, float inv_nct,
                        int ldp_bytes, const int64_t* __restrict__ chunk_off, const uint32_t* __restrict__ quad_off,
                        typename EntOf<VT>::type* __restrict__ ent, int nquads_all) {
  extern __shared__ __attribute__((aligned(16))) uint32_t qf_lds[];
  for (int qi = blockIdx.x; qi < nquads_all; qi += gridDim.x) {
    quad_fill_staged_one<VT>(qi, qf_lds, ptr, idx, val, seg, blk_row0, perm, nct, cap, inv_nct, ldp_bytes, chunk_off, quad_off, ent);
    __syncthreads();
  }
}

__global__ void tile_index_mod_kernel(const int64_t* __restrict__ ptr, const int32_t* __restrict__ idx,
                                      const uint64_t* __restrict__ packed, int64_t rows, int nct, float inv_nct,
                                      int32_t* __restrict__ seg) {
  const int64_t total = rows * (int64_t)(nct + 1);
  int64_t o = (int64_t)blockIdx.x * blockDim.x + threadIdx.x;
  const int64_t stride = (int64_t)gridDim.x * blockDim.x;
  for (; o < total; o += stride) {
    const int64_t r = o / (nct + 1);
    const int t = (int)(o - r * (nct + 1));
    const int64_t e0 = ptr[r], e1 = ptr[r + 1];
    int64_t lo = e0, hi = e1;
    while (lo < hi) {
      const int64_t mid = (lo + hi) >> 1;
      int q, tm;
      divmod_small(packed ? (int)(packed[mid] >> 32) : idx[mid], nct, inv_nct, q, tm);
      if (tm < t) lo = mid + 1; else hi = mid;
    }
    seg[o] = (int32_t)(lo - e0);
  }
}

__global__ void at_stats_index_kernel(const int64_t* __restrict__ ptr, const uint64_t* __restrict__ packed, int64_t rows,
                                      int nct, float inv_nct, double* __restrict__ sum, double* __restrict__ sumsq,
                                      int32_t* __restrict__ seg) {
  const int lane = threadIdx.x & (WAVE - 1);
  const int64_t wave = ((int64_t)blockIdx.x * blockDim.x + threadIdx.x) / WAVE;
  const int64_t nwaves = (int64_t)gridDim.x * blockDim.x / WAVE;
  for (int64_t r = wave; r < rows; r += nwaves) {
    const int64_t e0 = ptr[r], e1 = ptr[r + 1];
    int32_t* sg = seg + r * (nct + 1);
    double a = 0, b = 0;
    int carry = -1;
    for (int64_t eb = e0; eb < e1; eb += WAVE) {
      const int64_t e = eb + lane;
      const bool valid = e < e1;
      int t = nct;
      if (valid) {
        const uint64_t pv = packed[e];
        const double v = (double)__uint_as_float((uint32_t)pv);
        a += v;
        b += v * v;
        int q;
        divmod_small((int)(pv >> 32), nct, inv_nct, q, t);
      }
      int tprev = __shfl_up(t, 1);
      if (lane == 0) tprev = carry;
      if (valid || e == e1)
        for (int tt = tprev + 1; tt <= t; ++tt) sg[tt] = (int32_t)(e - e0);
      carry = __shfl(t, WAVE - 1);
    }
    if (((e1 - e0) & (WAVE - 1)) == 0)
      for (int tt = carry + 1 + lane; tt <= nct; tt += WAVE) sg[tt] = (int32_t)(e1 - e0);
#pragma unroll
    for (int off = WAVE / 2; off > 0; off >>= 1) {
      a += __shfl_xor(a, off);
      b += __shfl_xor(b, off);
    }
    if (lane == 0) {
      sum[r] = a;
      if (sumsq) sumsq[r] = b;
    }
  }
}

__global__ void row_len_iota_kernel(const int64_t* __restrict__ ptr, int64_t rows, uint32_t* __restrict__ len,
                                    uint32_t* __restrict__ iota) {
  const int64_t r = (int64_t)blockIdx.x * blockDim.x + threadIdx.x;
  if (r < rows) {
    len[r] = (uint32_t)(ptr[r + 1] - ptr[r]);
    iota[r] = (uint32_t)r;
  }
}

__global__ void __launch_bounds__(256)
natural_quad_slots_kernel(const int64_t* __restrict__ ptr, int64_t rows, unsigned long long* __restrict__ out) {
  __shared__ unsigned long long red[4];
  unsigned long long acc = 0;
  const int64_t nq = (rows + 3) / 4;
  for (int64_t qd = (int64_t)blockIdx.x * blockDim.x + threadIdx.x; qd < nq; qd += (int64_t)gridDim.x * blockDim.x) {
    int64_t mx = 0;
    for (int g = 0; g < 4 && 4 * qd + g < rows; ++g) mx = max(mx, ptr[4 * qd + g + 1] - ptr[4 * qd + g]);
    acc += (unsigned long long)(4 * mx);
  }
#pragma unroll
  for (int off = WAVE / 2; off > 0; off >>= 1) acc += __shfl_xor(acc, off);
  if ((threadIdx.x & (WAVE - 1)) == 0) red[threadIdx.x / WAVE] = acc;
  __syncthreads();
  if (threadIdx.x == 0) atomicAdd(out, red[0] + red[1] + red[2] + red[3]);
}

template <bool SEG_LDS, typename VT = float>
__global__ void __launch_bounds__(256)
quad_fill_runs_kernel(const int64_t* __restrict__ ptr, const int32_t* __restrict__ idx, const VT* __restrict__ val,
                      const uint64_t* __restrict__ packed, const int32_t* __restrict__ seg, const int32_t* __restrict__ blk_row0,
                      const uint32_t* __restrict__ perm, int nct, float inv_nct, int ldp_bytes,
                      const int64_t* __restrict__ chunk_off, const uint32_t* __restrict__ quad_off,
                      typename EntOf<VT>::type* __restrict__ ent) {
  typedef typename EntOf<VT>::type Ent;
  extern __shared__ int32_t sg_lds[];
  const int rb = blockIdx.x / Q_BLOCK_QUADS, qd = blockIdx.x % Q_BLOCK_QUADS;
  const int row0 = blk_row0[rb], nrows = blk_row0[rb + 1] - row0;
  if (4 * qd >= nrows) return;
  const int wave = threadIdx.x / WAVE, lane = threadIdx.x & (WAVE - 1);
  const int qrows = min(4, nrows - 4 * qd);
  const int64_t s0q = (int64_t)row0 + 4 * qd;
  if (SEG_LDS) {
    for (int i = threadIdx.x; i < 4 * (nct + 1); i += 256) {
      const int g = i / (nct + 1);
      const int64_t rg = g < qrows ? (perm ? (int64_t)perm[s0q + g] : s0q + g) : 0;
      sg_lds[i] = g < qrows ? seg[rg * (nct + 1) + (i - g * (nct + 1))] : 0;
    }
    __syncthreads();
  }
  const int g = lane & 3, k0 = lane >> 2;
  const int64_t myrow = g < qrows ? (perm ? (int64_t)perm[s0q + g] : s0q + g) : -1;
  const int64_t base = myrow >= 0 ? ptr[myrow] : 0;
  const int32_t* mysg = SEG_LDS ? sg_lds + g * (nct + 1) : seg + (myrow >= 0 ? myrow : 0) * (nct + 1);
  const int64_t* __restrict__ coff = chunk_off + (int64_t)rb * nct;
  const uint32_t* __restrict__ qoff = quad_off + ((int64_t)rb * Q_BLOCK_QUADS + qd) * nct;
  int s_nx = 0, e_nx = 0;
  int64_t d_nx = 0;
  if (!SEG_LDS && wave < nct) {
    s_nx = myrow >= 0 ? mysg[wave] : 0;
    e_nx = myrow >= 0 ? mysg[wave + 1] : 0;
    d_nx = coff[wave] + qoff[wave];
  }
  for (int t = wave; t < nct; t += 4) {
    int s0, len;
    Ent* dst;
    if (SEG_LDS) {
      s0 = mysg[t];
      len = mysg[t + 1] - s0;
      dst = ent + coff[t] + qoff[t];
    } else {
      s0 = s_nx;
      len = e_nx - s_nx;
      dst = ent + d_nx;
      if (t + 4 < nct) {
        s_nx = myrow >= 0 ? mysg[t + 4] : 0;
        e_nx = myrow >= 0 ? mysg[t + 5] : 0;
        d_nx = coff[t + 4] + qoff[t + 4];
      }
    }
    int qmax = max(len, __shfl_xor(len, 1));
    qmax = q_steps(max(qmax, __shfl_xor(qmax, 2)));
    for (int k = k0; k < qmax; k += 16) {
      Ent x{};
// ... 124 lines not shown
    const int64_t row_e0 = e0;
    for (int64_t base = e0; base < e1; base += 8 * WAVE) {
      const int64_t eb = base + lane;
      int c[8];
#pragma unroll
      for (int u = 0; u < 8; ++u) c[u] = eb + u * WAVE < e1 ? idx[eb + u * WAVE] : -1;
      if (bnd) {
#pragma unroll
        for (int u = 0; u < 8; ++u) {
          const bool valid = c[u] >= 0;
          const unsigned long long valids = __ballot(valid);
          if (valids == 0ull) break;
          const int b = (int)((float)max(c[u], 0) * blk_scale);
          const int up = __builtin_amdgcn_update_dpp(0, b, 0x138, 0xf, 0xf, false);
          const int prev = lane == 0 ? lastb : up;
          if (valid && b != prev)
            for (int j = prev + 1; j <= b; ++j) bnd_row[j] = (uint32_t)(eb + u * WAVE - row_e0);
          if (valid && b < prev) *disorder = 1;
          lastb = __builtin_amdgcn_readlane(b, __builtin_popcountll(valids) - 1);
        }
      }
#pragma unroll
      for (int u = 0; u < 8; ++u)
        if (c[u] >= 0) atomicAdd(&atd_h32[c[u] >> 1], 1u << (16 * (c[u] & 1)));
    }
    if (bnd)
      for (int j = lastb + 1 + lane; j <= nrb; j += WAVE) bnd_row[j] = (uint32_t)(e1 - row_e0);
    r = rn;
    e0 = n0;
    e1 = n1;
  }
  __syncthreads();
  uint32_t* out = reinterpret_cast<uint32_t*>(cnt16 + (int64_t)t * n2);
  for (int i = threadIdx.x; i < nw; i += nthreads) out[i] = atd_h32[i];
}

__global__ void __launch_bounds__(1024)
atd_rowlen_kernel(const uint16_t* __restrict__ cnt16, int64_t n, int64_t n2, int nct, int64_t* __restrict__ len,
                  unsigned long long* __restrict__ natural_slots) {
  __shared__ uint32_t part[16][64];
  const int lane = threadIdx.x & 63, grp = threadIdx.x >> 6;
  const int64_t c = (int64_t)blockIdx.x * 64 + lane;
  const int per = (nct + 15) / 16;
  uint32_t a = 0;
  if (c < n) {
    const int t1 = min(nct, (grp + 1) * per);
    int t = grp * per;
    for (; t + 8 <= t1; t += 8) {
      uint32_t v[8];
#pragma unroll
      for (int u = 0; u < 8; ++u) v[u] = cnt16[(int64_t)(t + u) * n2 + c];
#pragma unroll
      for (int u = 0; u < 8; ++u) a += v[u];
    }
    for (; t < t1; ++t) a += cnt16[(int64_t)t * n2 + c];
  }
  part[grp][lane] = a;
  __syncthreads();
  if (grp == 0) {
    int64_t total = 0;
    if (c < n)
      for (int g = 0; g < 16; ++g) total += part[g][lane];
    if (c <= n) len[c] = total;
    if (natural_slots) {
      int64_t mx = max(total, __shfl_xor(total, 1));
      mx = max(mx, __shfl_xor(mx, 2));
      unsigned long long acc = (lane & 3) == 0 ? (unsigned long long)(4 * mx) : 0ull;
#pragma unroll
      for (int off = WAVE / 2; off > 0; off >>= 1) acc += __shfl_xor(acc, off);
      if (lane == 0 && acc) atomicAdd(natural_slots, acc);
    }
  }
}

__global__ void atd_colmap_kernel(const int32_t* __restrict__ blk, int nrb, const uint32_t* __restrict__ perm, int64_t rows,
                                  uint32_t* __restrict__ colmap) {
  const int64_t sp = (int64_t)blockIdx.x * blockDim.x + threadIdx.x;
  if (sp >= rows) return;
  int lo = 0, hi = nrb;
  while (lo + 1 < hi) {
    const int mid = (lo + hi) >> 1;
    if ((int64_t)blk[mid] <= sp) lo = mid; else hi = mid;
  }
  const int64_t row = perm ? (int64_t)perm[sp] : sp;
  colmap[row] = ((uint32_t)lo << 10) | (uint32_t)(sp - blk[lo]);
}

__global__ void __launch_bounds__(256)
atd_scatter_kernel(const int64_t* __restrict__ ptr, const int32_t* __restrict__ idx, const float* __restrict__ val, int64_t m, int nct,
                   int tc, const uint32_t* __restrict__ colmap, const int64_t* __restrict__ bucket_off, uint32_t* __restrict__ cursor,
                   uint2* __restrict__ bucket) {
  const int lane = threadIdx.x & (WAVE - 1);
  const int xcd = blockIdx.x & 7;
  const int64_t wave = (int64_t)(blockIdx.x >> 3) * (blockDim.x / WAVE) + threadIdx.x / WAVE;
  const int64_t nwaves = (int64_t)(gridDim.x >> 3) * (blockDim.x / WAVE);
  const int tiles_x = (nct - xcd + 7) / 8;
  const int64_t items = (int64_t)tiles_x * tc;
  constexpr int UB = 10;
  for (int64_t item = wave; item < items; item += nwaves) {
    const int i = (int)(item / tiles_x), t = xcd + 8 * (int)(item - (int64_t)i * tiles_x);
    const int64_t r = (int64_t)t + (int64_t)i * nct;
    if (r >= m) continue;
    const int64_t e1 = ptr[r + 1];
    for (int64_t eb = ptr[r]; eb < e1; eb += UB * WAVE) {
      int cc[UB];
      uint32_t cmv[UB];
      float vv[UB];
      int64_t base[UB];
      int mine[UB];
#pragma unroll
      for (int u = 0; u < UB; ++u) {
        const int64_t e = eb + u * WAVE + lane;
        cc[u] = e < e1 ? idx[e] : -1;
        vv[u] = e < e1 ? val[e] : 0.f;
      }
#pragma unroll
      for (int u = 0; u < UB; ++u) cmv[u] = cc[u] >= 0 ? colmap[cc[u]] : 0xffffffffu;
#pragma unroll
      for (int u = 0; u < UB; ++u) {
        const uint32_t rb = cmv[u] >> 10;
        const uint32_t prev = __shfl_up(rb, 1);
        const bool valid = cc[u] >= 0;
        const bool leader = valid && (lane == 0 || rb != prev);
        const unsigned long long leaders = __ballot(leader), valids = __ballot(valid);
        const unsigned long long upto = leaders & ((2ull << lane) - 1ull);
        mine[u] = upto ? 63 - __builtin_clzll(upto) : 0;
        base[u] = 0;
        if (leader) {
          const unsigned long long above = leaders & ~((2ull << lane) - 1ull);
          const int next = above ? __builtin_ctzll(above) : __builtin_popcountll(valids);
          const int64_t b = (int64_t)rb * nct + t;
          base[u] = bucket_off[b] + (int64_t)atomicAdd(&cursor[b], (uint32_t)(next - lane));
        }
      }
#pragma unroll
      for (int u = 0; u < UB; ++u) {
        const int64_t b0 = __shfl(base[u], mine[u]);
        if (cc[u] >= 0)
          bucket[b0 + (lane - mine[u])] = make_uint2(((cmv[u] & 1023u) << 9) | (uint32_t)i, __float_as_uint(vv[u]));
      }
    }
  }
}

constexpr int ATD_STAGE_ENT = 4096;

template <bool GATHER>
__global__ void __launch_bounds__(ATD_THREADS, 8)
atd_fill_kernel(const uint2* __restrict__ bucket, const int64_t* __restrict__ bucket_off, const int32_t* __restrict__ blk_row0,
                const uint32_t* __restrict__ perm, int nct, int ldp_bytes, const int64_t* __restrict__ chunk_off,
                const uint32_t* __restrict__ quad_off, const uint16_t* __restrict__ steps, Ent* __restrict__ ent,
                double* __restrict__ psum, double* __restrict__ psq, int64_t n,
                const int32_t* __restrict__ a_idx, const float* __restrict__ a_val, const uint32_t* __restrict__ bnd,
                const int64_t* __restrict__ a_ptr, int64_t a_rows, int tc, int nrb_all) {
  constexpr int MASK_WORDS_ALL = QBLOCK_ROWS * ATD_MASK_WORDS;
  __shared__ __attribute__((aligned(16))) uint32_t pool[MASK_WORDS_ALL + 2 * ATD_STAGE_ENT];
  uint32_t* mask = pool;
  Ent* stage = reinterpret_cast<Ent*>(pool + MASK_WORDS_ALL);
  __shared__ uint32_t qoff_s[Q_BLOCK_QUADS + 1];
  __shared__ uint32_t wtot[Q_BLOCK_QUADS / WAVE];
  __shared__ uint16_t len_s[QBLOCK_ROWS];
  __shared__ int64_t run_lo[GATHER ? 32 * ATD_MASK_WORDS : 1];
  __shared__ uint32_t run_pre[GATHER ? 32 * ATD_MASK_WORDS + 1 : 1];
  __shared__ uint32_t rtot[GATHER ? 32 * ATD_MASK_WORDS / WAVE : 1];
  int rb, t;
  if constexpr (GATHER) {
    const int xcd = blockIdx.x & 7, j = blockIdx.x >> 3;
    t = xcd + 8 * (j / nrb_all);
    rb = j % nrb_all;
    if (t >= nct) return;
  } else {
    rb = (int)(blockIdx.x / nct);
    t = (int)(blockIdx.x % nct);
  }
  const int64_t chunk = (int64_t)rb * nct + t;
  const int row0 = blk_row0[rb], nrows = blk_row0[rb + 1] - row0;
  const int nquads = (nrows + 3) / 4;
  for (int i = threadIdx.x; i < QBLOCK_ROWS * ATD_MASK_WORDS; i += ATD_THREADS) mask[i] = 0u;
  if (threadIdx.x < Q_BLOCK_QUADS) {
    const int q = threadIdx.x, lane = q & (WAVE - 1);
    const uint32_t sz = q < nquads ? 4u * (uint32_t)steps[chunk * Q_BLOCK_QUADS + q] : 0u;
    uint32_t inc = sz;
#pragma unroll
    for (int off = 1; off < WAVE; off <<= 1) {
      const uint32_t y = __shfl_up(inc, off);
      if (lane >= off) inc += y;
    }
    qoff_s[q + 1] = inc;
    if (lane == WAVE - 1) wtot[q / WAVE] = inc;
  }
  if constexpr (GATHER) {
    if (threadIdx.x < 32 * ATD_MASK_WORDS) {
      const int i = threadIdx.x, lane = i & (WAVE - 1);
      const uint32_t* br = bnd + ((int64_t)t * tc + i) * (nrb_all + 1) + rb;
      const int64_t arow = (int64_t)t + (int64_t)i * nct;
      const int64_t e0 = (i < tc && arow < a_rows) ? a_ptr[arow] : 0;
      const int64_t lo = i < tc ? e0 + br[0] : 0;
      const int64_t hi = i < tc ? e0 + br[1] : 0;
      run_lo[i] = lo;
      uint32_t inc = hi > lo ? (uint32_t)(hi - lo) : 0u;
#pragma unroll
      for (int off = 1; off < WAVE; off <<= 1) {
        const uint32_t y = __shfl_up(inc, off);
        if (lane >= off) inc += y;
      }
      run_pre[i + 1] = inc;
      if (lane == WAVE - 1) rtot[i / WAVE] = inc;
    }
  }
  __syncthreads();
  if (threadIdx.x < Q_BLOCK_QUADS) {
    uint32_t add = 0;
    for (int w = 0; w < (int)threadIdx.x / WAVE; ++w) add += wtot[w];
    qoff_s[threadIdx.x + 1] += add;
    if (threadIdx.x == 0) qoff_s[0] = 0u;
  }
  if constexpr (GATHER) {
    if (threadIdx.x < 32 * ATD_MASK_WORDS) {
      uint32_t add = 0;
      for (int w = 0; w < (int)threadIdx.x / WAVE; ++w) add += rtot[w];
      run_pre[threadIdx.x + 1] += add;
      if (threadIdx.x == 0) run_pre[0] = 0u;
    }
  }
  __syncthreads();
  const int64_t b0 = GATHER ? 0 : bucket_off[chunk];
  const int64_t b1 = GATHER ? (int64_t)(uint32_t)__builtin_amdgcn_readfirstlane((int)run_pre[32 * ATD_MASK_WORDS]) : bucket_off[chunk + 1];
  constexpr int HOLD = 10;
  uint16_t* row_of = reinterpret_cast<uint16_t*>(stage);
  if constexpr (GATHER) {
    if (threadIdx.x < 3 * 32 * ATD_MASK_WORDS) {
      const uint32_t i = threadIdx.x / 3u;
      const uint32_t k1 = min(run_pre[i + 1], (uint32_t)(HOLD * ATD_THREADS));
      for (uint32_t k = run_pre[i] + threadIdx.x % 3u; k < k1; k += 3u) row_of[k] = (uint16_t)i;
    }
    __syncthreads();
  }
  auto fetch = [&](int64_t f, bool tabled) -> uint2 {
    if constexpr (GATHER) {
      int lo = 0;
      if (tabled) {
        lo = row_of[f];
      } else {
        int hi = 32 * ATD_MASK_WORDS - 1;
        while (lo < hi) {
          const int mid = (lo + hi + 1) >> 1;
          if ((int64_t)run_pre[mid] <= f) lo = mid; else hi = mid - 1;
        }
      }
      const int64_t e = run_lo[lo] + (f - (int64_t)run_pre[lo]);
      return make_uint2(((uint32_t)(a_idx[e] - row0) << 9) | (uint32_t)lo, __float_as_uint(a_val[e]));
    } else {
      return bucket[f];
    }
  };
  Ent* dst = ent + chunk_off[chunk];
  uint2 kv[HOLD];
#pragma unroll
  for (int u = 0; u < HOLD; ++u) {
    const int64_t e = b0 + threadIdx.x + (int64_t)u * ATD_THREADS;
    kv[u] = e < b1 ? fetch(e, true) : make_uint2(0xffffffffu, 0u);
  }
#pragma unroll
  for (int u = 0; u < HOLD; ++u)
    if (kv[u].x != 0xffffffffu) {
      const uint32_t slot = kv[u].x >> 9, i = kv[u].x & 511u;
      atomicOr(&mask[slot * ATD_MASK_WORDS + (i >> 5)], 1u << (i & 31u));
    }
  for (int64_t e = b0 + threadIdx.x + (int64_t)HOLD * ATD_THREADS; e < b1; e += ATD_THREADS) {
    const uint32_t key = fetch(e, false).x;
    const uint32_t slot = key >> 9, i = key & 511u;
    atomicOr(&mask[slot * ATD_MASK_WORDS + (i >> 5)], 1u << (i & 31u));
  }
  __syncthreads();
  const bool held = b1 - b0 <= (int64_t)HOLD * ATD_THREADS;
  uint16_t* pre = reinterpret_cast<uint16_t*>(stage);
  for (int slot = threadIdx.x; slot < QBLOCK_ROWS; slot += ATD_THREADS) {
    uint32_t run = 0;
#pragma unroll
    for (int w = 0; w < ATD_MASK_WORDS; ++w) {
      if (held) pre[slot * ATD_MASK_WORDS + w] = (uint16_t)run;
      run += __builtin_popcount(mask[slot * ATD_MASK_WORDS + w]);
    }
    len_s[slot] = (uint16_t)run;
  }
  __syncthreads();
  auto rank_of = [&](uint32_t slot, uint32_t i) {
    const uint32_t* mk = mask + slot * ATD_MASK_WORDS;
    uint32_t rank = __builtin_popcount(mk[i >> 5] & ((1u << (i & 31u)) - 1u));
    if (held) return rank + (uint32_t)pre[slot * ATD_MASK_WORDS + (i >> 5)];
    for (uint32_t w = 0; w < (i >> 5); ++w) rank += __builtin_popcount(mk[w]);
    return rank;
  };
#pragma unroll
  for (int u = 0; u < HOLD; ++u) {
    if (kv[u].x != 0xffffffffu) {
      const uint32_t slot = kv[u].x >> 9, i = kv[u].x & 511u;
      kv[u].x = (qoff_s[slot >> 2] + rank_of(slot, i) * 4u + (slot & 3u)) | (i << 23);
    }
    asm volatile("" ::: "memory");
  }
  const uint32_t HALF = held ? (uint32_t)(MASK_WORDS_ALL / 2 + ATD_STAGE_ENT) / 2u : (uint32_t)ATD_STAGE_ENT / 2u;
  Ent* const image = held ? reinterpret_cast<Ent*>(pool) : stage;
  __syncthreads();
  auto row_len = [&](int slot) { return (int)len_s[slot]; };
  int half = 0;
  for (int q0 = 0; q0 < nquads; half ^= 1) {
    int q1 = q0 + 1;
    {
      int lo = q0 + 1, hi = nquads;
      while (lo < hi) {
        const int mid = (lo + hi + 1) >> 1;
        if (qoff_s[mid] - qoff_s[q0] <= HALF) lo = mid; else hi = mid - 1;
      }
      q1 = __builtin_amdgcn_readfirstlane(lo);
    }
    Ent* st = image + (half ? HALF : 0u);
    const uint32_t o0 = (uint32_t)__builtin_amdgcn_readfirstlane((int)qoff_s[q0]);
    const uint32_t size = (uint32_t)__builtin_amdgcn_readfirstlane((int)qoff_s[q1]) - o0;
    for (int slot = 4 * q0 + (int)threadIdx.x; slot < 4 * q1; slot += ATD_THREADS) {
      const uint32_t qo = qoff_s[slot >> 2], nsteps = (qoff_s[(slot >> 2) + 1] - qo) / 4u;
      const uint32_t o = qo - o0 + (uint32_t)(slot & 3);
#pragma clang loop vectorize(disable) unroll(disable)
      for (uint32_t k = slot < nrows ? (uint32_t)row_len(slot) : 0u; k < nsteps; ++k) st[o + 4u * k] = Ent{0u, 0.f};
    }
    auto place = [&](uint32_t slot, uint32_t i, uint32_t rank, uint32_t vbits) {
      const int q = (int)(slot >> 2);
      if (q < q0 || q >= q1) return;
      Ent x;
      x.off = i * (uint32_t)ldp_bytes;
      x.val = __uint_as_float(vbits);
      st[qoff_s[q] - o0 + rank * 4u + (slot & 3u)] = x;
    };
#pragma unroll
    for (int u = 0; u < HOLD; ++u) {
      const uint32_t at = (kv[u].x & 0x7fffffu) - o0;
      if (at < size) {
        Ent x;
        x.off = (kv[u].x >> 23) * (uint32_t)ldp_bytes;
        x.val = __uint_as_float(kv[u].y);
        st[at] = x;
      }
    }
    for (int64_t e = b0 + threadIdx.x + (int64_t)HOLD * ATD_THREADS; e < b1; e += ATD_THREADS) {
      const uint2 x = fetch(e, false);
      const uint32_t slot = x.x >> 9, i = x.x & 511u;
      const int q = (int)(slot >> 2);
      if (q >= q0 && q < q1) place(slot, i, rank_of(slot, i), x.y);
    }
    __syncthreads();
    {
      const uint4* src4 = reinterpret_cast<const uint4*>(st);
      uint4* dst4 = reinterpret_cast<uint4*>(dst + o0);
      for (uint32_t i = threadIdx.x; i < size / 2; i += ATD_THREADS) dst4[i] = src4[i];
    }
    if (psum) {
      const int pairs = 2 * (min(4 * q1, nrows) - 4 * q0);
      for (int pr = (int)threadIdx.x; pr < pairs; pr += ATD_THREADS) {
        const int slot = 4 * q0 + (pr >> 1), part = pr & 1;
        const int len = row_len(slot);
        const uint32_t o = qoff_s[slot >> 2] - o0 + (uint32_t)(slot & 3);
        double a = 0, b = 0;
#pragma clang loop vectorize(disable) unroll(disable)
        for (int k = part; k < len; k += 2) {
          const double v = (double)st[o + 4u * k].val;
          a += v;
          b += v * v;
        }
        a += __shfl_xor(a, 1);
        b += __shfl_xor(b, 1);
        if (part == 0) {
          const int64_t row = perm ? (int64_t)perm[row0 + slot] : (int64_t)row0 + slot;
          psum[(int64_t)t * n + row] = a;
          psq[(int64_t)t * n + row] = b;
        }
      }
    }
    q0 = q1;
  }
}

__global__ void __launch_bounds__(1024)
atd_stats_reduce_kernel(const double* __restrict__ psum, const double* __restrict__ psq, int64_t n, int nct,
                        double* __restrict__ sum, double* __restrict__ sumsq) {
  __shared__ double pa[16][64], pb[16][64];
  const int lane = threadIdx.x & 63, grp = threadIdx.x >> 6;
  const int64_t c = (int64_t)blockIdx.x * 64 + lane;
  const int per = (nct + 15) / 16;
  double a = 0, b = 0;
  if (c < n)
    for (int t = grp * per; t < min(nct, (grp + 1) * per); ++t) {
      a += psum[(int64_t)t * n + c];
      b += psq[(int64_t)t * n + c];
    }
  pa[grp][lane] = a;
  pb[grp][lane] = b;
  __syncthreads();
  if (grp == 0 && c < n) {
    double x = 0, y = 0;
    for (int g = 0; g < 16; ++g) {
      x += pa[g][lane];
      y += pb[g][lane];
    }
    sum[c] = x;
    sumsq[c] = y;
  }
}

}


struct AtDirectSrc {
  const CsrView<float>* A;
  const uint16_t* cnt16;
  int64_t n2;
  DevBuf* scratch;
  double* stats;
  const uint32_t* bnd;
  int64_t nrb_nat;
  const std::vector<int32_t>* blk_nat;
};

namespace {

struct BuildSwitches {
  static int number(const char* value, int otherwise) { return value ? atoi(value) : otherwise; }
  bool no_dq = dbg_on("SAPCA_NO_DQ");
  bool no_rowsort = dbg_on("SAPCA_NO_ROWSORT"), rowsort_always = dbg_on("SAPCA_ROWSORT_ALWAYS");
  bool fill_direct = dbg_on("SAPCA_FILL_DIRECT"), qf_cap_fixed = dbg_on("SAPCA_QF_CAP_FIXED");
  bool at_sort = dbg_on("SAPCA_AT_SORT");
  bool at_buckets = dbg_on("SAPCA_AT_BUCKETS");
  bool debug = dbg_on("SAPCA_DEBUG");
  int dq_block_rows = number(dbg_env("SAPCA_DQ_BLOCK_ROWS"), 0), split_wgs = number(dbg_env("SAPCA_SPLIT_WGS"), 0);
  int runs_seg_lds_max = number(dbg_env("SAPCA_RUNS_SEG_LDS_MAX"), 1024);
};

enum MiscWord { kMiscMaxChunk = 0, kMiscTotal = 1, kMiscNaturalSlots = 4, kMiscDisorder = 6, kMiscWords = 8 };
enum PinnedWord { kPinNaturalSlots = 0, kPinMisc = 1, kPinBlocks = 8 };
static_assert(kPinMisc + kMiscDisorder < kPinBlocks, "the read-back run of buf.misc ends ahead of the staged block table");
constexpr size_t kPinBlockTable = 2 * 65536;
inline int64_t* misc_words(TiledBuffers& buf) { return buf.misc.as<int64_t>(kMiscWords); }

void float_blocks(int64_t n, int64_t nrb, std::vector<int32_t>& blk, float& scale) {
  scale = (float)nrb / (float)n;
  auto block_of = [&](int64_t c) { return (int64_t)(int)((float)(int)c * scale); };
  while (block_of(n - 1) > nrb - 1) scale = std::nextafterf(scale, 0.0f);
  blk.assign((size_t)nrb + 1, (int32_t)n);
  int64_t b = 0;
  blk[0] = 0;
  for (int64_t c = 0; c < n; ++c) {
    const int64_t bc = block_of(c);
    while (b < bc) blk[(size_t)++b] = (int32_t)c;
  }
  while (b < nrb) blk[(size_t)++b] = (int32_t)n;
}

int dq_block_rows(int64_t op_rows, const BuildSwitches& sw) {
  return sw.dq_block_rows == 512 || sw.dq_block_rows == 1024 ? sw.dq_block_rows : (op_rows >= 1024 * 16 ? 1024 : 512);
}
void natural_partition(int64_t op_rows, int nct, int block_rows, const BuildSwitches& sw, int64_t& nrb, int& nsplit) {
  nrb = (op_rows + block_rows - 1) / block_rows;
  nsplit = 1;
  if (nrb >= 192) {
    nrb = round_up(nrb, 256);
  } else {
    const int64_t split_wgs = sw.split_wgs > 0 ? sw.split_wgs : (block_rows > 512 ? 256 : 512);
    nsplit = (int)std::min<int64_t>(nct, std::max<int64_t>(1, split_wgs / nrb));
    const int64_t nrb_fit = split_wgs / nsplit;
    if (nrb_fit >= nrb && nrb_fit <= op_rows) nrb = nrb_fit;
  }
}

inline unsigned qf_grid(int64_t nquads) {
#ifdef SAPCA_QF_WGS
  const int64_t wgs = SAPCA_QF_WGS;
#else
  const int64_t wgs = nquads;
#endif
  return (unsigned)std::max<int64_t>(1, std::min<int64_t>(nquads, wgs));
}

struct QuadGeometry {
  int64_t rows = 0, cols = 0, nnz = 0;
  int elem = 4;
  int ldp = 0;
  int tc = 0, nct = 0;
  float inv_nct = 0.f;
  bool dq_candidate = false;
  int block_rows = 0;
  int stage_cap = 0;
  int64_t nrb = 0;
  int nsplit = 1;
  bool empty() const { return rows == 0 || cols == 0 || nnz == 0; }
};

inline int tile_count(int64_t cols, int ldp) { return (int)((cols + q_tile_rows(ldp) - 1) / q_tile_rows(ldp)); }

QuadGeometry quad_geometry(int64_t rows, int64_t cols, int64_t nnz, int elem, int ldp_elems, const BuildSwitches& sw) {
  QuadGeometry g;
  g.rows = rows; g.cols = cols; g.nnz = nnz; g.elem = elem;
  g.ldp = ldp_elems * elem / 4;
  g.tc = q_tile_rows(g.ldp);
  g.nct = tile_count(cols, g.ldp);
  g.dq_candidate = elem == 4 && g.ldp == 64 && !sw.no_dq;
  g.block_rows = g.dq_candidate ? dq_block_rows(rows, sw) : QWAVES * QGROUPS * q_rows_per_group(g.ldp);
  g.stage_cap = q_stage_cap(Q_TILE_BYTES, elem == 4 ? (int)sizeof(Ent) : (int)sizeof(EntD));
  if (g.empty()) return g;
  g.inv_nct = 1.0f / (float)g.nct;
  natural_partition(rows, g.nct, g.block_rows, sw, g.nrb, g.nsplit);
  return g;
}

bool eligible(const QuadGeometry& g, const QuadSource& src) {
  const bool f32 = g.elem == 4, tile_major = src.kind != QuadSource::Csr;
  if (g.empty()) return false;
  if (!f32 && (src.kind == QuadSource::TileMajorPacked || src.kind == QuadSource::FromA)) return false;
  if (g.cols >= (1 << 24) || g.nct > (tile_major ? Q_MAX_TILES_RUNS : 4096)) return false;
  if (src.kind == QuadSource::FromA)
    return g.rows <= ATD_MAX_COLS && g.tc <= 32 * ATD_MASK_WORDS && g.dq_candidate && g.block_rows <= QBLOCK_ROWS;
  return true;
}

template <typename VT>
struct Build {
  const CsrView<VT>& S;
  const QuadGeometry& g;
  const QuadSource& src;
  const BuildSwitches& sw;
  TiledBuffers& buf;
  hipStream_t s;
};

struct Counts {
  int64_t nrb = 0;
  int nsplit = 1, tiles_per_split = 0;
  int64_t nchunks = 0, max_chunk = 0, total = 0, mid_row0 = -1;
  bool rows_in_disorder = false;
  int32_t* d_blk = nullptr;
  uint32_t* d_perm = nullptr;
  uint8_t* d_steps = nullptr;
  uint32_t* d_wave_off = nullptr;
  uint32_t* d_quad_off = nullptr;
  int64_t* d_chunk = nullptr;
  int64_t* d_raw = nullptr;
};

template <typename VT>
const int32_t* index_rows(const Build<VT>& b) {
  const QuadGeometry& g = b.g;
  const CsrView<VT>& S = b.S;
  if (b.src.kind == QuadSource::FromA) return nullptr;
  int32_t* d_seg = b.buf.seg.template as<int32_t>((size_t)S.rows * (g.nct + 1));
  if (b.src.kind == QuadSource::Csr) {
    hipLaunchKernelGGL(tile_hist_kernel, dim3(grid_for(S.rows, 4, 8192)), dim3(256), (size_t)4 * g.nct * sizeof(uint32_t), b.s,
                       S.ptr, S.idx, S.rows, g.nct, g.inv_nct, d_seg);
  } else if (!b.src.seg_ready) {
    hipLaunchKernelGGL(tile_index_mod_kernel, dim3(grid_for(S.rows * (int64_t)(g.nct + 1), 256, 16384)), dim3(256), 0, b.s,
                       S.ptr, S.idx, b.src.packed, S.rows, g.nct, g.inv_nct, d_seg);
  }
  return d_seg;
}

template <typename VT>
uint32_t* sort_rows_by_length(const Build<VT>& b, std::vector<uint32_t>& sorted_len) {
  const CsrView<VT>& S = b.S;
  hipStream_t s = b.s;
  uint32_t* d_len = b.buf.lens.template as<uint32_t>((size_t)2 * S.rows);
  uint32_t* d_len_sorted = d_len + S.rows;
  uint32_t* d_iota = b.buf.perm.template as<uint32_t>((size_t)2 * S.rows);
  uint32_t* d_perm = d_iota + S.rows;
  hipLaunchKernelGGL(row_len_iota_kernel, dim3(grid_for(S.rows, 256, 1 << 30)), dim3(256), 0, s, S.ptr, S.rows, d_len, d_iota);
  size_t sb = 0;
  SAPCA_HIP(rocprim::radix_sort_pairs_desc(nullptr, sb, d_len, d_len_sorted, d_iota, d_perm, (size_t)S.rows, 0u, 32u, s));
  char* tmp = static_cast<char*>(b.buf.tmp.ensure(sb + 256));
  SAPCA_HIP(rocprim::radix_sort_pairs_desc(tmp, sb, d_len, d_len_sorted, d_iota, d_perm, (size_t)S.rows, 0u, 32u, s));
  sorted_len.resize((size_t)S.rows);
  SAPCA_HIP(hipMemcpyAsync(sorted_len.data(), d_len_sorted, sorted_len.size() * sizeof(uint32_t), hipMemcpyDeviceToHost, s));
  SAPCA_HIP(hipStreamSynchronize(s));
  return d_perm;
}

template <typename VT>
void queue_natural_slots(const Build<VT>& b, int64_t* pinned) {
  const CsrView<VT>& S = b.S;
  unsigned long long* d_slots = reinterpret_cast<unsigned long long*>(misc_words(b.buf)) + kMiscNaturalSlots;
  if (b.src.kind != QuadSource::FromA) {
    SAPCA_HIP(hipMemsetAsync(d_slots, 0, sizeof(unsigned long long), b.s));
    hipLaunchKernelGGL(natural_quad_slots_kernel, dim3(grid_for((S.rows + 3) / 4, 256, 1024)), dim3(256), 0, b.s, S.ptr, S.rows, d_slots);
  }
  SAPCA_HIP(hipMemcpyAsync(pinned + kPinNaturalSlots, d_slots, sizeof(unsigned long long), hipMemcpyDeviceToHost, b.s));
}

std::vector<int32_t> cut_blocks(const QuadGeometry& g, const QuadSource& src, const std::vector<uint32_t>* sorted_len, int64_t& nrb) {
  std::vector<int32_t> blk;
  if (sorted_len) {
    const double budget = (double)g.nnz / (double)nrb;
    blk.push_back(0);
    double acc = 0;
    int in_block = 0;
    for (int64_t r = 0; r < g.rows; ++r) {
      acc += (*sorted_len)[(size_t)r];
      ++in_block;
      const bool last = r + 1 == g.rows;
      if (last || in_block == g.block_rows || acc >= budget * (double)blk.size()) {
        blk.push_back((int32_t)(r + 1));
        in_block = 0;
      }
    }
    nrb = (int64_t)blk.size() - 1;
  } else if (src.kind == QuadSource::FromA && src.from_a->bnd && nrb == src.from_a->nrb_nat) {
    blk = *src.from_a->blk_nat;
  } else {
    blk.resize((size_t)nrb + 1);
    for (int64_t b = 0; b <= nrb; ++b) blk[(size_t)b] = (int32_t)(g.rows * b / nrb);
  }
  return blk;
}

template <typename VT>
void count_once(const Build<VT>& b, const int32_t* d_seg, const std::vector<int32_t>& blk, int64_t* pinned, Counts& c) {
  const int nct = b.g.nct;
  TiledBuffers& buf = b.buf;
  hipStream_t s = b.s;
  const AtDirectSrc* from_a = b.src.kind == QuadSource::FromA ? b.src.from_a : nullptr;
  c.nchunks = c.nrb * nct;
  c.mid_row0 = blk[(size_t)(c.nrb / 2)];
  c.d_blk = buf.blk.as<int32_t>((size_t)c.nrb + 1);
  c.d_steps = buf.steps.as<uint8_t>((size_t)c.nchunks * Q_BLOCK_QUADS * 2);
  c.d_wave_off = buf.wave_off.as<uint32_t>((size_t)c.nchunks * QWAVES);
  c.d_quad_off = buf.quad_off.as<uint32_t>((size_t)c.nchunks * Q_BLOCK_QUADS);
  c.d_chunk = buf.chunk_off.as<int64_t>((size_t)c.nchunks + 1);
  if (blk.size() <= kPinBlockTable) {
    std::memcpy(pinned + kPinBlocks, blk.data(), blk.size() * sizeof(int32_t));
    SAPCA_HIP(hipMemcpyAsync(c.d_blk, pinned + kPinBlocks, blk.size() * sizeof(int32_t), hipMemcpyHostToDevice, s));
  } else {
    SAPCA_HIP(hipMemcpyAsync(c.d_blk, blk.data(), blk.size() * sizeof(int32_t), hipMemcpyHostToDevice, s));
  }
  const dim3 grid((unsigned)(c.nrb * ((nct + QC_TILES - 1) / QC_TILES)));
  if (from_a) {
    c.d_raw = buf.raw.as<int64_t>((size_t)c.nchunks + 1);
    hipLaunchKernelGGL(quad_count_kernel, grid, dim3(Q_BLOCK_QUADS), 0, s, d_seg, c.d_blk, c.d_perm, nct, reinterpret_cast<uint16_t*>(c.d_steps),
                       (uint32_t*)nullptr, c.d_wave_off, c.d_chunk, from_a->cnt16, from_a->n2, c.d_raw);
  } else {
    hipLaunchKernelGGL(quad_count_kernel, grid, dim3(Q_BLOCK_QUADS), 0, s, d_seg, c.d_blk, c.d_perm, nct, reinterpret_cast<uint16_t*>(c.d_steps),
                       c.d_quad_off, c.d_wave_off, c.d_chunk);
  }
  int64_t* d_misc = misc_words(buf);
  launch_small_scan(c.d_chunk, c.d_raw, c.nchunks, d_misc + kMiscMaxChunk, s);
  const int words = (from_a ? kMiscDisorder : kMiscTotal) + 1;
  SAPCA_HIP(hipMemcpyAsync(pinned + kPinMisc, d_misc, words * sizeof(int64_t), hipMemcpyDeviceToHost, s));
  SAPCA_HIP(hipStreamSynchronize(s));
  if (from_a) c.rows_in_disorder = pinned[kPinMisc + kMiscDisorder] != 0;
  c.max_chunk = pinned[kPinMisc + kMiscMaxChunk];
  c.total = pinned[kPinMisc + kMiscTotal];
}

template <typename VT>
bool count_chunks(const Build<VT>& b, const int32_t* d_seg, Counts& c) {
  const QuadGeometry& g = b.g;
  int64_t* pinned = static_cast<int64_t*>(b.buf.host.ensure((kPinBlocks + kPinBlockTable / 2 + 2) * sizeof(int64_t)));
  std::vector<uint32_t> sorted_len;
  bool sort_rows = !b.sw.no_rowsort, speculate = false;
  if (sort_rows && !b.sw.rowsort_always) {
    queue_natural_slots(b, pinned);
    speculate = true;
    sort_rows = false;
  }
  if (sort_rows) c.d_perm = sort_rows_by_length(b, sorted_len);
  c.nrb = g.nrb;
  c.nsplit = g.nsplit;
  for (int attempt = 0;; ++attempt) {
    c.tiles_per_split = (g.nct + c.nsplit - 1) / c.nsplit;
    c.nsplit = (g.nct + c.tiles_per_split - 1) / c.tiles_per_split;
    const std::vector<int32_t> blk = cut_blocks(g, b.src, sort_rows ? &sorted_len : nullptr, c.nrb);
    count_once(b, d_seg, blk, pinned, c);
    if (speculate) {
      speculate = false;
      if ((double)(unsigned long long)pinned[kPinNaturalSlots] > 1.10 * (double)g.nnz) {
        sort_rows = true;
        c.d_perm = sort_rows_by_length(b, sorted_len);
        attempt = -1;
        continue;
      }
    }
    if (b.sw.debug)
      fprintf(stderr, "sapca: build_tiled rows %lld cols %lld nrb %lld nct %d split %d max_chunk %lld (cap %d) total %lld\n",
              (long long)g.rows, (long long)g.cols, (long long)c.nrb, g.nct, c.nsplit,
              (long long)c.max_chunk, g.stage_cap, (long long)c.total);
    if (c.max_chunk <= g.stage_cap || g.dq_candidate) return true;
    if (attempt == 3 || c.nrb * 2 > g.rows) return false;
    c.nrb *= 2;
    if (c.nsplit > 1) c.nsplit = std::max(1, c.nsplit / 2);
  }
}

void publish(TiledOp& op, const QuadGeometry& g, const Counts& c, const void* d_ent) {
  op.rows = g.rows; op.cols = g.cols; op.ldp = g.ldp * 4 / g.elem; op.elem = g.elem; op.tc = g.tc; op.nct = g.nct;
  op.nrb = (int)c.nrb; op.block_rows = g.block_rows; op.max_chunk = c.max_chunk;
  op.nsplit = c.nsplit; op.tiles_per_split = c.tiles_per_split; op.total_entries = c.total; op.tile_bytes = Q_TILE_BYTES;
  op.mid_row0 = c.mid_row0;
  op.blk_row0 = c.d_blk; op.row_perm = c.d_perm; op.chunk_off = c.d_chunk; op.wave_off = c.d_wave_off; op.steps = c.d_steps; op.ent = d_ent;
}

template <typename VT>
bool fork_dq_tables(TiledOp& op, TiledBuffers& buf, hipStream_t s) {
  bool dq_ok;
  op.valid = true;
  if constexpr (sizeof(VT) == 4) {
    if (!buf.aux) {
      SAPCA_HIP(hipStreamCreateWithFlags(&buf.aux, hipStreamNonBlocking));
      SAPCA_HIP(hipEventCreateWithFlags(&buf.aux_fork, hipEventDisableTiming));
      SAPCA_HIP(hipEventCreateWithFlags(&buf.aux_join, hipEventDisableTiming));
    }
    SAPCA_HIP(hipEventRecord(buf.aux_fork, s));
    SAPCA_HIP(hipStreamWaitEvent(buf.aux, buf.aux_fork, 0));
    dq_ok = dq_build_tables(op, buf, buf.aux);
    SAPCA_HIP(hipEventRecord(buf.aux_join, buf.aux));
  } else {
    dq_ok = dq_build_tables(op, buf, s);
  }
  op.valid = false;
  return dq_ok;
}

enum class Fill {
  Gather,
  Buckets,
  Runs,
  Staged,
  Direct
};
struct FillChoice { Fill fill; int qf_cap; };

FillChoice choose_fill(const QuadGeometry& g, const QuadSource& src, const Counts& c, const BuildSwitches& sw) {
  const bool f32 = g.elem == 4;
  const int64_t op_rows = g.rows, total = c.total;
  const int qf_cap_max = f32 ? QF_CAP_MAX : QF_CAP_MIN;
  const double quad_avg = (double)total / std::max(1.0, (double)op_rows / 4.0);
  const int qf_cap_fit = (int)std::min<int64_t>(qf_cap_max, std::max<int64_t>(2048, round_up((int64_t)(1.12 * quad_avg) + 64, 256)));
  const int qf_cap = (!f32 || sw.qf_cap_fixed) ? ((double)total <= 0.85 * QF_CAP_MIN * ((double)op_rows / 4.0) ? QF_CAP_MIN : qf_cap_max) : qf_cap_fit;
  if (src.kind == QuadSource::FromA) {
    const bool gather = src.from_a->bnd != nullptr && c.d_perm == nullptr && c.nrb == src.from_a->nrb_nat && !c.rows_in_disorder && !sw.at_buckets;
    return {gather ? Fill::Gather : Fill::Buckets, qf_cap};
  }
  if (src.kind != QuadSource::Csr) return {Fill::Runs, qf_cap};
  const bool staged = !sw.fill_direct && (double)total <= 0.93 * qf_cap_max * ((double)op_rows / 4.0) && g.nct <= 768;
  return {staged ? Fill::Staged : Fill::Direct, qf_cap};
}

void launch_fill_from_a(const QuadGeometry& g, const AtDirectSrc& a, const Counts& c, bool gather, Ent* d_ent, hipStream_t s) {
  const CsrView<float>& A = *a.A;
  const int nct = g.nct, nrb = (int)c.nrb;
  const int64_t op_rows = g.rows;
  const uint16_t* d_steps = reinterpret_cast<const uint16_t*>(c.d_steps);
  const size_t a_col = round_up((size_t)op_rows * sizeof(uint32_t), 256), a_bucket = gather ? 0 : round_up((size_t)A.nnz * sizeof(uint2), 256);
  const size_t a_part = a.stats ? round_up((size_t)nct * op_rows * sizeof(double), 256) : 0;
  char* base = static_cast<char*>(a.scratch->ensure(a_col + a_bucket + 2 * a_part + (size_t)c.nchunks * sizeof(uint32_t) + 256));
  uint32_t* d_colmap = reinterpret_cast<uint32_t*>(base);
  uint2* d_bucket = reinterpret_cast<uint2*>(base + a_col);
  double* d_psum = a.stats ? reinterpret_cast<double*>(base + a_col + a_bucket) : nullptr;
  double* d_psq = a.stats ? reinterpret_cast<double*>(base + a_col + a_bucket + a_part) : nullptr;
  if (gather) {
    hipLaunchKernelGGL(atd_fill_kernel<true>, dim3((unsigned)(8 * ((nct + 7) / 8) * nrb)), dim3(ATD_THREADS), 0, s, (const uint2*)nullptr,
                       (const int64_t*)nullptr, c.d_blk, c.d_perm, nct, g.ldp * 4, c.d_chunk, c.d_quad_off, d_steps, d_ent,
                       d_psum, d_psq, op_rows, A.idx, A.val, a.bnd, A.ptr, A.rows, g.tc, nrb);
  } else {
    hipLaunchKernelGGL(atd_colmap_kernel, dim3((unsigned)((op_rows + 255) / 256)), dim3(256), 0, s, c.d_blk, nrb, c.d_perm, op_rows,
                       d_colmap);
    uint32_t* d_cursor = reinterpret_cast<uint32_t*>(base + a_col + a_bucket + 2 * a_part);
    SAPCA_HIP(hipMemsetAsync(d_cursor, 0, (size_t)c.nchunks * sizeof(uint32_t), s));
    hipLaunchKernelGGL(atd_scatter_kernel, dim3((unsigned)std::min<int64_t>(round_up((A.rows + 3) / 4, 8), 4096)), dim3(256), 0, s, A.ptr,
                       A.idx, A.val, A.rows, nct, g.tc, d_colmap, c.d_raw, d_cursor, d_bucket);
    hipLaunchKernelGGL(atd_fill_kernel<false>, dim3((unsigned)c.nchunks), dim3(ATD_THREADS), 0, s, d_bucket, c.d_raw, c.d_blk, c.d_perm, nct, g.ldp * 4,
                       c.d_chunk, c.d_quad_off, d_steps, d_ent, d_psum, d_psq, op_rows,
                       (const int32_t*)nullptr, (const float*)nullptr, (const uint32_t*)nullptr, (const int64_t*)nullptr, (int64_t)0, g.tc, nrb);
  }
  if (a.stats)
    hipLaunchKernelGGL(atd_stats_reduce_kernel, dim3((unsigned)((op_rows + 63) / 64)), dim3(1024), 0, s, d_psum, d_psq, op_rows, nct,
                       a.stats, a.stats + op_rows);
}

template <typename VT>
void launch_fill(const Build<VT>& b, const Counts& c, const int32_t* d_seg, const FillChoice& f, typename EntOf<VT>::type* d_ent) {
  typedef typename EntOf<VT>::type E;
  const QuadGeometry& g = b.g;
  const CsrView<VT>& S = b.S;
  hipStream_t s = b.s;
  const int nct = g.nct, nrb = (int)c.nrb, ldp_bytes = g.ldp * 4;
  const int nquads = nrb * Q_BLOCK_QUADS;
  switch (f.fill) {
    case Fill::Gather:
    case Fill::Buckets:
      if constexpr (sizeof(VT) == 4) launch_fill_from_a(g, *b.src.from_a, c, f.fill == Fill::Gather, d_ent, s);
      break;
    case Fill::Runs:
      if (nct <= b.sw.runs_seg_lds_max)
        hipLaunchKernelGGL((quad_fill_runs_kernel<true, VT>), dim3((unsigned)nquads), dim3(256), (size_t)4 * (nct + 1) * sizeof(int32_t), s,
                           S.ptr, S.idx, S.val, b.src.packed, d_seg, c.d_blk, c.d_perm, nct, g.inv_nct, ldp_bytes, c.d_chunk, c.d_quad_off, d_ent);
      else
        hipLaunchKernelGGL((quad_fill_runs_kernel<false, VT>), dim3((unsigned)nquads), dim3(256), 0, s,
                           S.ptr, S.idx, S.val, b.src.packed, d_seg, c.d_blk, c.d_perm, nct, g.inv_nct, ldp_bytes, c.d_chunk, c.d_quad_off, d_ent);
      break;
    case Fill::Staged: {
      const size_t fill_lds = (size_t)f.qf_cap * sizeof(E) + ((size_t)7 * nct + 1) * sizeof(uint32_t);
      static LdsAttrState attr;
      ensure_dynamic_lds(reinterpret_cast<const void*>(&quad_fill_staged_kernel<VT>), fill_lds, attr);
      hipLaunchKernelGGL(quad_fill_staged_kernel<VT>, dim3(qf_grid(nquads)), dim3(256), fill_lds, s, S.ptr, S.idx, S.val, d_seg, c.d_blk,
                         c.d_perm, nct, f.qf_cap, g.inv_nct, ldp_bytes, c.d_chunk, c.d_quad_off, d_ent, nquads);
      break;
    }
    case Fill::Direct:
      hipLaunchKernelGGL(quad_fill_kernel<VT>, dim3((unsigned)((S.rows + 3) / 4)), dim3(256), (size_t)4 * nct * sizeof(uint32_t), s,
                         S.ptr, S.idx, S.val, S.rows, c.d_blk, c.d_perm, nrb, nct, g.inv_nct, ldp_bytes, c.d_chunk, c.d_quad_off, d_ent);
      break;
  }
}

template <typename VT>
bool build_quads(const CsrView<VT>& S, const QuadGeometry& g, const QuadSource& src, const BuildSwitches& sw, TiledOp& op,
                 TiledBuffers& buf, hipStream_t s) {
  typedef typename EntOf<VT>::type E;
  constexpr bool f32 = sizeof(VT) == 4;
  const Build<VT> b{S, g, src, sw, buf, s};
  const int32_t* d_seg = index_rows(b);
  Counts c;
  if (!count_chunks(b, d_seg, c)) return false;
  E* d_ent = reinterpret_cast<E*>(buf.ent.ensure((size_t)(c.total + ENT_SLACK) * sizeof(E)));
  publish(op, g, c, d_ent);
  const bool dq_ok = fork_dq_tables<VT>(op, buf, s);
  if (f32 && !dq_ok && (g.block_rows > 512 || c.max_chunk > g.stage_cap)) {
    SAPCA_HIP(hipStreamWaitEvent(s, buf.aux_join, 0));
    return false;
  }
  const FillChoice f = choose_fill(g, src, c, sw);
  if (f.fill != Fill::Direct) SAPCA_HIP(hipMemsetAsync(d_ent + c.total, 0, (size_t)ENT_SLACK * sizeof(E), s));
  else SAPCA_HIP(hipMemsetAsync(d_ent, 0, (size_t)(c.total + ENT_SLACK) * sizeof(E), s));
  launch_fill<VT>(b, c, d_seg, f, d_ent);
  SAPCA_HIP(hipGetLastError());
  if (f32) SAPCA_HIP(hipStreamWaitEvent(s, buf.aux_join, 0));
  op.valid = true;
  return true;
}

template <typename VT>
bool build_tiled_t(const CsrView<VT>& S, int ldp_elems, TiledOp& op, TiledBuffers& buf, hipStream_t s, const QuadSource& src) {
  SAPCA_CHECK(ldp_elems == 64, SAPCA_ERR_ARG, "tiled sweep: panels must have 64 columns");
  SAPCA_CHECK(src.kind != QuadSource::FromA, SAPCA_ERR_ARG, "tiled sweep: the A -> A^T route starts in build_tiled_at_direct");
  op = TiledOp();
  const BuildSwitches sw{};
  const QuadGeometry g = quad_geometry(S.rows, S.cols, S.nnz, (int)sizeof(VT), ldp_elems, sw);
  return eligible(g, src) && build_quads<VT>(S, g, src, sw, op, buf, s);
}

}

bool build_tiled(const CsrView<float>& S, int ldp, TiledOp& op, TiledBuffers& buf, hipStream_t s, const QuadSource& src) {
  return build_tiled_t<float>(S, ldp, op, buf, s, src);
}
bool build_tiled(const CsrView<double>& S, int ldp, TiledOp& op, TiledBuffers& buf, hipStream_t s, const QuadSource& src) {
  return build_tiled_t<double>(S, ldp, op, buf, s, src);
}

bool build_tiled_at_direct(const CsrView<float>& A, int ldp, TiledOp& op, TiledBuffers& buf, int64_t* at_ptr, double* stats,
                           DevBuf& scratch, hipStream_t s) {
  op = TiledOp();
  const BuildSwitches sw{};
  if (sw.at_sort || ldp != 64) return false;
  const int64_t m = A.rows, n = A.cols;
  const QuadGeometry g = quad_geometry(n, m, A.nnz, (int)sizeof(float), ldp, sw);
  QuadSource src;
  src.kind = QuadSource::FromA;
  if (!eligible(g, src)) return false;
  const int nct = g.nct, tc = g.tc;
  const int64_t n2 = round_up(n, 2);
  uint16_t* cnt16 = buf.seg.as<uint16_t>((size_t)nct * n2);
  const int64_t nrb_nat = g.nrb;
  uint32_t* bnd = nullptr;
  if (!sw.at_buckets && nrb_nat <= 4096) {
    try {
      bnd = buf.bounds.as<uint32_t>((size_t)(nrb_nat + 1) * (size_t)nct * tc);
    } catch (const Error&) {
      (void)hipGetLastError();
      bnd = nullptr;
    }
  }
  const size_t hist_lds = (size_t)n2 * 2;
  static LdsAttrState hist_attr;
  ensure_dynamic_lds(reinterpret_cast<const void*>(&atd_hist_kernel), hist_lds, hist_attr);
  std::vector<int32_t> blk_nat;
  float blk_scale = 0.f;
  if (bnd) float_blocks(n, nrb_nat, blk_nat, blk_scale);
  int64_t* d_disorder = misc_words(buf) + kMiscDisorder;
  unsigned long long* d_slots = reinterpret_cast<unsigned long long*>(misc_words(buf)) + kMiscNaturalSlots;
  SAPCA_HIP(hipMemsetAsync(d_disorder, 0, sizeof(int64_t), s));
  hipLaunchKernelGGL(atd_hist_kernel, dim3((unsigned)nct), dim3((size_t)n2 * 2 > 52 * 1024 ? ATD_HIST_THREADS_WIDE : ATD_HIST_THREADS),
                     hist_lds, s, A.ptr, A.idx, m, nct, tc, n2, cnt16, blk_scale, (int)nrb_nat, bnd, d_disorder, d_slots);
  hipLaunchKernelGGL(atd_rowlen_kernel, dim3((unsigned)((n + 64) / 64)), dim3(1024), 0, s, cnt16, n, n2, nct, at_ptr, d_slots);
  launch_small_scan(at_ptr, nullptr, n, nullptr, s);
  SAPCA_HIP(hipGetLastError());
  CsrView<float> At;
  At.rows = n; At.cols = m; At.nnz = A.nnz; At.ptr = at_ptr; At.idx = nullptr; At.val = nullptr;
  const AtDirectSrc from_a{&A, cnt16, n2, &scratch, stats, bnd, nrb_nat, &blk_nat};
  src.from_a = &from_a;
  return build_quads<float>(At, g, src, sw, op, buf, s);
}

void at_stats_index(const int64_t* ptr, const uint64_t* packed, int64_t rows, int64_t cols, int ldp, TiledBuffers& buf,
                    double* sum, double* sumsq, hipStream_t s) {
  if (rows == 0) return;
  const int nct = tile_count(cols, ldp);
  int32_t* d_seg = buf.seg.as<int32_t>((size_t)rows * (nct + 1));
  hipLaunchKernelGGL(at_stats_index_kernel, dim3(grid_for(rows * WAVE, 256, 4096)), dim3(256), 0, s, ptr, packed, rows, nct,
                     1.0f / (float)nct, sum, sumsq, d_seg);
  SAPCA_HIP(hipGetLastError());
}

int tiled_tile_count(int64_t cols, int ldp) { return tile_count(cols, ldp); }

}
}
```

Before: 1374.

## Speculate tiled build sizes from the previous build to avoid host sync

The tiled quad build now forecasts entry counts from the previous build's shape, so it can skip the blocking host read-back after counting. Fills launch immediately into the existing buffer. A device verdict kernel makes them exit early, and the host redoes the count if the forecast capacity, natural slots or row order disagree. It also defers the statistics D2H copy and the side-stream join, and generates the Gaussian Omega panel on the side stream. The cost is extra complexity and a possible wasted pass when speculation fails. It relies on later calls reusing similar matrices, with a fallback that keeps results correct.

```diff
diff --git a/single-algebra_amd/csrc/common.h b/single-algebra_amd/csrc/common.h
--- a/single-algebra_amd/csrc/common.h
+++ b/single-algebra_amd/csrc/common.h
@@ -143,6 +143,12 @@
   PinnedBuf host;
   hipStream_t aux = nullptr;
   hipEvent_t aux_fork = nullptr, aux_join = nullptr;
+  struct LastBuild {
+    bool valid = false, natural = false;
+    int kind = -1, elem = 0;
+    int64_t rows = 0, cols = 0, nnz = 0, total = 0;
+  } last;
+  hipEvent_t counted = nullptr;
   TiledBuffers() = default;
   TiledBuffers(const TiledBuffers&) = delete;
   TiledBuffers& operator=(const TiledBuffers&) = delete;
@@ -150,6 +156,7 @@
     if (aux) { (void)hipStreamSynchronize(aux); (void)hipStreamDestroy(aux); }
     if (aux_fork) (void)hipEventDestroy(aux_fork);
     if (aux_join) (void)hipEventDestroy(aux_join);
+    if (counted) (void)hipEventDestroy(counted);
   }
 };
 
diff --git a/single-algebra_amd/csrc/engine.cpp b/single-algebra_amd/csrc/engine.cpp
--- a/single-algebra_amd/csrc/engine.cpp
+++ b/single-algebra_amd/csrc/engine.cpp
@@ -138,6 +138,7 @@
   AtFrom at = AtFrom::Transposed;
   StatsFrom stats = StatsFrom::Transposed;
   StatsTo deliver = StatsTo::MainCopy;
+  bool speculate = false;
 };
 
 template <typename T>
@@ -194,6 +195,7 @@
   if (h.comm.active()) p.deliver = StatsTo::AllReduce;
   else if (p.stats == StatsFrom::Scatter) p.deliver = StatsTo::ScatterSide;
   else if (p.stats == StatsFrom::KeptAndDropped && dbg_env("SAPCA_MASK_STATS_INLINE") == nullptr) p.deliver = StatsTo::SideChain;
+  p.speculate = sizeof(T) == 4 && !p.masked && p.at == AtFrom::FormatFromA && !h.comm.active();
   return p;
 }
 
@@ -258,7 +260,7 @@
     try {
       SAPCA_HIP(hipSetDevice(h.device));
       SAPCA_HIP(hipStreamWaitEvent(h.stream2, h.ev_fork, 0));
-      if (p.tiled_ldp != 0) out.ok_a = k::build_tiled(src, p.tiled_ldp, h.tiled_a, h.tb_a, h.stream2, k::QuadSource::csr());
+      if (p.tiled_ldp != 0) out.ok_a = k::build_tiled(src, p.tiled_ldp, h.tiled_a, h.tb_a, h.stream2, k::QuadSource::csr(), p.speculate);
       SAPCA_HIP(hipEventRecord(h.ev_join, h.stream2));
     } catch (...) {
       aside.err = std::current_exception();
@@ -282,7 +284,7 @@
     double* d_sums = p.masked ? h.scratch2.as<double>((size_t)2 * p.n_used + 2) : stats_dev(h, p.n);
     h.tiled_at = TiledOp();
     out.at_direct = k::build_tiled_at_direct(src, p.tiled_ldp, h.tiled_at, h.tb_at, t_ptr,
-                                             p.stats == StatsFrom::Upload ? nullptr : d_sums, h.scratch, h.stream);
+                                             p.stats == StatsFrom::Upload ? nullptr : d_sums, h.scratch, h.stream, p.speculate);
     if (!out.at_direct) return;
     if (!p.masked) out.At = CsrView<T>{p.n, p.m, p.nnz, t_ptr, nullptr, nullptr};
     else h.at_used = {p.n_used, p.m, out.nnz_used, t_ptr, nullptr, nullptr};
@@ -350,7 +352,7 @@
     sums[(size_t)2 * n] = (double)m;
     h.stats_on_side = p.deliver == StatsTo::SideChain || p.deliver == StatsTo::ScatterSide;
     if (p.deliver == StatsTo::MainCopy) {
-      SAPCA_HIP(hipMemcpyAsync(sums, d_stats, (size_t)2 * n * sizeof(double), hipMemcpyDeviceToHost, s));
+      h.stats_copy_queued = false;
     } else if (p.deliver == StatsTo::AllReduce) {
       double* tail = h.stats_tail;
       const uint32_t nr = h.comm.nranks;
@@ -428,6 +430,13 @@
   }
 }
 
+void queue_statistics_copy(H& h) {
+  if (h.stats_copy_queued) return;
+  h.stats_copy_queued = true;
+  const size_t n = (size_t)h.stats_cols;
+  SAPCA_HIP(hipMemcpyAsync(h.stats_host.p, h.stats.ptr<double>(), 2 * n * sizeof(double), hipMemcpyDeviceToHost, h.stream));
+}
+
 template <typename T>
 void queue_side_statistics(H& h, const PrepPlan& p, const PrepOutcome<T>& out, const MaskMaps& maps) {
   const int64_t n = p.n;
@@ -451,6 +460,8 @@
   if (h.stream3) SAPCA_HIP(hipStreamSynchronize(h.stream3));
   h.stats_pending = false;
   h.stats_on_side = false;
+  h.stats_copy_queued = true;
+  h.prep_a_aside = false;
   h.lz_scatter = false;
 
   const PrepPlan p = plan_preparation(h, A);
@@ -486,7 +497,9 @@
 
   build_formats(h, p, out, aside);
   aside.join();
-  if (out.a_aside) SAPCA_HIP(hipStreamWaitEvent(s, h.ev_join, 0));
+  h.a_join_pending = out.a_aside && p.speculate && h.opt.method == SAPCA_RANDOM;
+  if (out.a_aside && !h.a_join_pending) SAPCA_HIP(hipStreamWaitEvent(s, h.ev_join, 0));
+  h.prep_a_aside = out.a_aside;
   if (p.deliver == StatsTo::SideChain) queue_side_statistics(h, p, out, maps);
 
   h.prep_key = prep_key_of(h, A);
@@ -647,9 +660,17 @@
 void load_omega(H& h, const RandomizedPlan& p, FitPanels<T>& f) {
   hipStream_t s = h.stream;
   if (h.omega.empty()) {
-    k::gaussian_panel(f.X, p.n_used, p.l, p.ld, h.opt.random_seed, s);
+    if (p.tiled && h.stream2 && h.prep_a_aside) {
+      k::gaussian_panel(f.X, p.n_used, p.l, p.ld, h.opt.random_seed, h.stream2);
+      order_after(s, h.ev_join, h.stream2);
+      h.a_join_pending = false;
+    } else {
+      Engine<T>::join_side_stream(h);
+      k::gaussian_panel(f.X, p.n_used, p.l, p.ld, h.opt.random_seed, s);
+    }
     return;
   }
+  Engine<T>::join_side_stream(h);
   SAPCA_CHECK((int64_t)h.omega_rows == p.n_used && (int64_t)h.omega_cols >= p.l, SAPCA_ERR_ARG,
               "injected Omega must be (features seen by the SVD) x (n_components + n_oversamples)");
   std::vector<T> tmp((size_t)p.n_used * p.l);
@@ -1100,6 +1121,10 @@
   SAPCA_CHECK(h.opt.n_components > 0, SAPCA_ERR_ARG, "n_components must be positive");
   SAPCA_CHECK(A.rows > 0 && A.cols > 0, SAPCA_ERR_ARG, "empty matrix");
   prepare(h, A);
+  struct JoinGuard {
+    H& h;
+    ~JoinGuard() { if (h.a_join_pending && h.stream2) { (void)hipStreamWaitEvent(h.stream, h.ev_join, 0); h.a_join_pending = false; } }
+  } join_guard{h};
   const int64_t n_used = h.a_used.cols;
   if ((int64_t)h.opt.n_components > std::min<int64_t>((int64_t)h.m_global - (int64_t)h.covar.fit.rank, n_used))
     throw Error(SAPCA_ERR_SVD, std::string(h.opt.method == SAPCA_RANDOM ? "Randomized SVD" : "SVD") +
@@ -1134,6 +1159,7 @@
     }
   }
 
+  queue_statistics_copy(h);
   h.k = h.opt.n_components;
   h.n_used = (uint64_t)n_used;
   h.n_cols = (uint64_t)A.cols;
diff --git a/single-algebra_amd/csrc/engine.h b/single-algebra_amd/csrc/engine.h
--- a/single-algebra_amd/csrc/engine.h
+++ b/single-algebra_amd/csrc/engine.h
@@ -20,6 +20,9 @@
   hipEvent_t ev_piece = nullptr, ev_comm = nullptr;
   hipEvent_t ev_kept = nullptr, ev_stats = nullptr;
   bool stats_on_side = false;
+  bool stats_copy_queued = true;
+  bool a_join_pending = false;
+  bool prep_a_aside = false;
 
   std::vector<uint8_t> mask;
   uint64_t mask_version = 0;
@@ -247,6 +250,11 @@
   static void finish_fit(H& h);
   static void transform(H& h, const CsrView<T>& A, T* d_out);
   static void fit_randomized(H& h);
+  static void join_side_stream(H& h) {
+    if (!h.a_join_pending) return;
+    h.a_join_pending = false;
+    SAPCA_HIP(hipStreamWaitEvent(h.stream, h.ev_join, 0));
+  }
   static void fit_lanczos(H& h, bool centred);
   static bool vote_rides(const H& h);
   static int64_t piece_vote(H& h, int ld);
diff --git a/single-algebra_amd/csrc/kernels.h b/single-algebra_amd/csrc/kernels.h
--- a/single-algebra_amd/csrc/kernels.h
+++ b/single-algebra_amd/csrc/kernels.h
@@ -163,10 +163,12 @@
     return q;
   }
 };
-bool build_tiled(const CsrView<float>& S, int ldp, TiledOp& op, TiledBuffers& buf, hipStream_t s, const QuadSource& src);
-bool build_tiled(const CsrView<double>& S, int ldp, TiledOp& op, TiledBuffers& buf, hipStream_t s, const QuadSource& src);
+bool build_tiled(const CsrView<float>& S, int ldp, TiledOp& op, TiledBuffers& buf, hipStream_t s, const QuadSource& src,
+                 bool speculate = false);
+bool build_tiled(const CsrView<double>& S, int ldp, TiledOp& op, TiledBuffers& buf, hipStream_t s, const QuadSource& src,
+                 bool speculate = false);
 bool build_tiled_at_direct(const CsrView<float>& A, int ldp, TiledOp& op, TiledBuffers& buf, int64_t* at_ptr, double* stats,
-                           DevBuf& scratch, hipStream_t s);
+                           DevBuf& scratch, hipStream_t s, bool speculate = false);
 void at_stats_index(const int64_t* ptr, const uint64_t* packed, int64_t rows, int64_t cols, int ldp, TiledBuffers& buf,
                     double* sum, double* sumsq, hipStream_t s);
 int tiled_tile_count(int64_t cols, int ldp);
diff --git a/single-algebra_amd/csrc/tiled_build.hip b/single-algebra_amd/csrc/tiled_build.hip
--- a/single-algebra_amd/csrc/tiled_build.hip
+++ b/single-algebra_amd/csrc/tiled_build.hip
@@ -307,8 +307,9 @@
                         const int32_t* __restrict__ seg, const int32_t* __restrict__ blk_row0,
                         const uint32_t* __restrict__ perm, int nct, int cap, float inv_nct,
                         int ldp_bytes, const int64_t* __restrict__ chunk_off, const uint32_t* __restrict__ quad_off,
-                        typename EntOf<VT>::type* __restrict__ ent, int nquads_all) {
+                        typename EntOf<VT>::type* __restrict__ ent, int nquads_all, const int64_t* __restrict__ skip) {
   extern __shared__ __attribute__((aligned(16))) uint32_t qf_lds[];
+  if (skip && *skip) return;
   for (int qi = blockIdx.x; qi < nquads_all; qi += gridDim.x) {
     quad_fill_staged_one<VT>(qi, qf_lds, ptr, idx, val, seg, blk_row0, perm, nct, cap, inv_nct, ldp_bytes, chunk_off, quad_off, ent);
     __syncthreads();
@@ -739,8 +740,9 @@
                 const uint32_t* __restrict__ quad_off, const uint16_t* __restrict__ steps, Ent* __restrict__ ent,
                 double* __restrict__ psum, double* __restrict__ psq, int64_t n,
                 const int32_t* __restrict__ a_idx, const float* __restrict__ a_val, const uint32_t* __restrict__ bnd,
-                const int64_t* __restrict__ a_ptr, int64_t a_rows, int tc, int nrb_all) {
+                const int64_t* __restrict__ a_ptr, int64_t a_rows, int tc, int nrb_all, const int64_t* __restrict__ skip) {
   constexpr int MASK_WORDS_ALL = QBLOCK_ROWS * ATD_MASK_WORDS;
+  if (skip && *skip) return;
   __shared__ __attribute__((aligned(16))) uint32_t pool[MASK_WORDS_ALL + 2 * ATD_STAGE_ENT];
   uint32_t* mask = pool;
   Ent* stage = reinterpret_cast<Ent*>(pool + MASK_WORDS_ALL);
@@ -994,6 +996,21 @@
   }
 }
 
+__global__ void __launch_bounds__(256)
+spec_verdict_kernel(const int64_t* __restrict__ total, const unsigned long long* __restrict__ natural_slots,
+                    const int64_t* __restrict__ disorder, int64_t cap_entries, int64_t nnz, int64_t* __restrict__ verdict,
+                    uint64_t* __restrict__ ent_words, int words_per_entry, int slack_words) {
+  const int64_t n = *total;
+  int64_t v = 0;
+  if (n > cap_entries) v |= 1;
+  if ((double)*natural_slots > 1.10 * (double)nnz) v |= 2;
+  if (disorder && *disorder != 0) v |= 4;
+  if (threadIdx.x == 0) *verdict = v;
+  if (v != 0) return;
+  uint64_t* z = ent_words + n * words_per_entry;
+  for (int i = threadIdx.x; i < slack_words; i += blockDim.x) z[i] = 0;
+}
+
 }
 
 
@@ -1020,11 +1037,12 @@
   bool debug = dbg_on("SAPCA_DEBUG");
   int dq_block_rows = number(dbg_env("SAPCA_DQ_BLOCK_ROWS"), 0), split_wgs = number(dbg_env("SAPCA_SPLIT_WGS"), 0);
   int runs_seg_lds_max = number(dbg_env("SAPCA_RUNS_SEG_LDS_MAX"), 1024);
+  int64_t spec_cap = dbg_env("SAPCA_SPEC_CAP") ? atoll(dbg_env("SAPCA_SPEC_CAP")) : -1;
 };
 
-enum MiscWord { kMiscMaxChunk = 0, kMiscTotal = 1, kMiscNaturalSlots = 4, kMiscDisorder = 6, kMiscWords = 8 };
-enum PinnedWord { kPinNaturalSlots = 0, kPinMisc = 1, kPinBlocks = 8 };
-static_assert(kPinMisc + kMiscDisorder < kPinBlocks, "the read-back run of buf.misc ends ahead of the staged block table");
+enum MiscWord { kMiscMaxChunk = 0, kMiscTotal = 1, kMiscNaturalSlots = 4, kMiscDisorder = 6, kMiscVerdict = 7, kMiscWords = 8 };
+enum PinnedWord { kPinNaturalSlots = 0, kPinMisc = 1, kPinBlocks = 16 };
+static_assert(kPinMisc + kMiscVerdict < kPinBlocks, "the read-back run of buf.misc ends ahead of the staged block table");
 constexpr size_t kPinBlockTable = 2 * 65536;
 inline int64_t* misc_words(TiledBuffers& buf) { return buf.misc.as<int64_t>(kMiscWords); }
 
@@ -1123,6 +1141,8 @@
   int nsplit = 1, tiles_per_split = 0;
   int64_t nchunks = 0, max_chunk = 0, total = 0, mid_row0 = -1;
   bool rows_in_disorder = false;
+  bool speculated = false;
+  int64_t cap_entries = 0;
   int32_t* d_blk = nullptr;
   uint32_t* d_perm = nullptr;
   uint8_t* d_steps = nullptr;
@@ -1133,11 +1153,12 @@
 };
 
 template <typename VT>
-const int32_t* index_rows(const Build<VT>& b) {
+const int32_t* index_rows(const Build<VT>& b, bool indexed) {
   const QuadGeometry& g = b.g;
   const CsrView<VT>& S = b.S;
   if (b.src.kind == QuadSource::FromA) return nullptr;
   int32_t* d_seg = b.buf.seg.template as<int32_t>((size_t)S.rows * (g.nct + 1));
+  if (indexed) return d_seg;
   if (b.src.kind == QuadSource::Csr) {
     hipLaunchKernelGGL(tile_hist_kernel, dim3(grid_for(S.rows, 4, 8192)), dim3(256), (size_t)4 * g.nct * sizeof(uint32_t), b.s,
                        S.ptr, S.idx, S.rows, g.nct, g.inv_nct, d_seg);
@@ -1168,14 +1189,14 @@
 }
 
 template <typename VT>
-void queue_natural_slots(const Build<VT>& b, int64_t* pinned) {
+void queue_natural_slots(const Build<VT>& b, int64_t* pinned, bool read_back) {
   const CsrView<VT>& S = b.S;
   unsigned long long* d_slots = reinterpret_cast<unsigned long long*>(misc_words(b.buf)) + kMiscNaturalSlots;
   if (b.src.kind != QuadSource::FromA) {
     SAPCA_HIP(hipMemsetAsync(d_slots, 0, sizeof(unsigned long long), b.s));
     hipLaunchKernelGGL(natural_quad_slots_kernel, dim3(grid_for((S.rows + 3) / 4, 256, 1024)), dim3(256), 0, b.s, S.ptr, S.rows, d_slots);
   }
-  SAPCA_HIP(hipMemcpyAsync(pinned + kPinNaturalSlots, d_slots, sizeof(unsigned long long), hipMemcpyDeviceToHost, b.s));
+  if (read_back) SAPCA_HIP(hipMemcpyAsync(pinned + kPinNaturalSlots, d_slots, sizeof(unsigned long long), hipMemcpyDeviceToHost, b.s));
 }
 
 std::vector<int32_t> cut_blocks(const QuadGeometry& g, const QuadSource& src, const std::vector<uint32_t>* sorted_len, int64_t& nrb) {
@@ -1204,8 +1225,10 @@
   return blk;
 }
 
+struct Forecast { int64_t total = 0, cap_entries = 0; };
 template <typename VT>
-void count_once(const Build<VT>& b, const int32_t* d_seg, const std::vector<int32_t>& blk, int64_t* pinned, Counts& c) {
+void count_once(const Build<VT>& b, const int32_t* d_seg, const std::vector<int32_t>& blk, int64_t* pinned, Counts& c,
+                const Forecast* fc = nullptr) {
   const int nct = b.g.nct;
   TiledBuffers& buf = b.buf;
   hipStream_t s = b.s;
@@ -1234,6 +1257,21 @@
   }
   int64_t* d_misc = misc_words(buf);
   launch_small_scan(c.d_chunk, c.d_raw, c.nchunks, d_misc + kMiscMaxChunk, s);
+  if (fc) {
+    typedef typename EntOf<VT>::type E;
+    hipLaunchKernelGGL(spec_verdict_kernel, dim3(1), dim3(256), 0, s, d_misc + kMiscTotal,
+                       reinterpret_cast<const unsigned long long*>(d_misc) + kMiscNaturalSlots,
+                       from_a ? d_misc + kMiscDisorder : (const int64_t*)nullptr, fc->cap_entries, b.g.nnz, d_misc + kMiscVerdict,
+                       buf.ent.template ptr<uint64_t>(), (int)(sizeof(E) / 8), (int)(ENT_SLACK * sizeof(E) / 8));
+    SAPCA_HIP(hipMemcpyAsync(pinned + kPinMisc, d_misc, kMiscWords * sizeof(int64_t), hipMemcpyDeviceToHost, s));
+    if (!buf.counted) SAPCA_HIP(hipEventCreateWithFlags(&buf.counted, hipEventDisableTiming));
+    SAPCA_HIP(hipEventRecord(buf.counted, s));
+    c.speculated = true;
+    c.total = fc->total;
+    c.cap_entries = fc->cap_entries;
+    c.max_chunk = 0;
+    return;
+  }
   const int words = (from_a ? kMiscDisorder : kMiscTotal) + 1;
   SAPCA_HIP(hipMemcpyAsync(pinned + kPinMisc, d_misc, words * sizeof(int64_t), hipMemcpyDeviceToHost, s));
   SAPCA_HIP(hipStreamSynchronize(s));
@@ -1243,13 +1281,22 @@
 }
 
 template <typename VT>
-bool count_chunks(const Build<VT>& b, const int32_t* d_seg, Counts& c) {
+bool count_chunks(const Build<VT>& b, const int32_t* d_seg, Counts& c, const Forecast* fc = nullptr) {
   const QuadGeometry& g = b.g;
   int64_t* pinned = static_cast<int64_t*>(b.buf.host.ensure((kPinBlocks + kPinBlockTable / 2 + 2) * sizeof(int64_t)));
   std::vector<uint32_t> sorted_len;
   bool sort_rows = !b.sw.no_rowsort, speculate = false;
+  if (fc) {
+    queue_natural_slots(b, pinned, false);
+    c.nrb = g.nrb;
+    c.nsplit = g.nsplit;
+    c.tiles_per_split = (g.nct + c.nsplit - 1) / c.nsplit;
+    c.nsplit = (g.nct + c.tiles_per_split - 1) / c.tiles_per_split;
+    count_once(b, d_seg, cut_blocks(g, b.src, nullptr, c.nrb), pinned, c, fc);
+    return true;
+  }
   if (sort_rows && !b.sw.rowsort_always) {
-    queue_natural_slots(b, pinned);
+    queue_natural_slots(b, pinned, true);
     speculate = true;
     sort_rows = false;
   }
@@ -1335,7 +1382,8 @@
   return {staged ? Fill::Staged : Fill::Direct, qf_cap};
 }
 
-void launch_fill_from_a(const QuadGeometry& g, const AtDirectSrc& a, const Counts& c, bool gather, Ent* d_ent, hipStream_t s) {
+void launch_fill_from_a(const QuadGeometry& g, const AtDirectSrc& a, const Counts& c, bool gather, Ent* d_ent, hipStream_t s,
+                         const int64_t* skip) {
   const CsrView<float>& A = *a.A;
   const int nct = g.nct, nrb = (int)c.nrb;
   const int64_t op_rows = g.rows;
@@ -1350,7 +1398,7 @@
   if (gather) {
     hipLaunchKernelGGL(atd_fill_kernel<true>, dim3((unsigned)(8 * ((nct + 7) / 8) * nrb)), dim3(ATD_THREADS), 0, s, (const uint2*)nullptr,
                        (const int64_t*)nullptr, c.d_blk, c.d_perm, nct, g.ldp * 4, c.d_chunk, c.d_quad_off, d_steps, d_ent,
-                       d_psum, d_psq, op_rows, A.idx, A.val, a.bnd, A.ptr, A.rows, g.tc, nrb);
+                       d_psum, d_psq, op_rows, A.idx, A.val, a.bnd, A.ptr, A.rows, g.tc, nrb, skip);
   } else {
     hipLaunchKernelGGL(atd_colmap_kernel, dim3((unsigned)((op_rows + 255) / 256)), dim3(256), 0, s, c.d_blk, nrb, c.d_perm, op_rows,
                        d_colmap);
@@ -1360,7 +1408,8 @@
                        A.idx, A.val, A.rows, nct, g.tc, d_colmap, c.d_raw, d_cursor, d_bucket);
     hipLaunchKernelGGL(atd_fill_kernel<false>, dim3((unsigned)c.nchunks), dim3(ATD_THREADS), 0, s, d_bucket, c.d_raw, c.d_blk, c.d_perm, nct, g.ldp * 4,
                        c.d_chunk, c.d_quad_off, d_steps, d_ent, d_psum, d_psq, op_rows,
-                       (const int32_t*)nullptr, (const float*)nullptr, (const uint32_t*)nullptr, (const int64_t*)nullptr, (int64_t)0, g.tc, nrb);
+                       (const int32_t*)nullptr, (const float*)nullptr, (const uint32_t*)nullptr, (const int64_t*)nullptr, (int64_t)0, g.tc, nrb,
+                       (const int64_t*)nullptr);
   }
   if (a.stats)
     hipLaunchKernelGGL(atd_stats_reduce_kernel, dim3((unsigned)((op_rows + 63) / 64)), dim3(1024), 0, s, d_psum, d_psq, op_rows, nct,
@@ -1368,7 +1417,8 @@
 }
 
 template <typename VT>
-void launch_fill(const Build<VT>& b, const Counts& c, const int32_t* d_seg, const FillChoice& f, typename EntOf<VT>::type* d_ent) {
+void launch_fill(const Build<VT>& b, const Counts& c, const int32_t* d_seg, const FillChoice& f, typename EntOf<VT>::type* d_ent,
+                 const int64_t* skip) {
   typedef typename EntOf<VT>::type E;
   const QuadGeometry& g = b.g;
   const CsrView<VT>& S = b.S;
@@ -1378,7 +1428,7 @@
   switch (f.fill) {
     case Fill::Gather:
     case Fill::Buckets:
-      if constexpr (sizeof(VT) == 4) launch_fill_from_a(g, *b.src.from_a, c, f.fill == Fill::Gather, d_ent, s);
+      if constexpr (sizeof(VT) == 4) launch_fill_from_a(g, *b.src.from_a, c, f.fill == Fill::Gather, d_ent, s, skip);
       break;
     case Fill::Runs:
       if (nct <= b.sw.runs_seg_lds_max)
@@ -1393,7 +1443,7 @@
       static LdsAttrState attr;
       ensure_dynamic_lds(reinterpret_cast<const void*>(&quad_fill_staged_kernel<VT>), fill_lds, attr);
       hipLaunchKernelGGL(quad_fill_staged_kernel<VT>, dim3(qf_grid(nquads)), dim3(256), fill_lds, s, S.ptr, S.idx, S.val, d_seg, c.d_blk,
-                         c.d_perm, nct, f.qf_cap, g.inv_nct, ldp_bytes, c.d_chunk, c.d_quad_off, d_ent, nquads);
+                         c.d_perm, nct, f.qf_cap, g.inv_nct, ldp_bytes, c.d_chunk, c.d_quad_off, d_ent, nquads, skip);
       break;
     }
     case Fill::Direct:
@@ -1403,53 +1453,117 @@
   }
 }
 
+enum class BuildMode { Wait, Speculate, Redo };
+
+template <typename VT>
+bool forecast(const Build<VT>& b, Forecast& fc) {
+  const QuadGeometry& g = b.g;
+  const TiledBuffers::LastBuild& last = b.buf.last;
+  if (sizeof(VT) != 4 || !g.dq_candidate || !last.valid || last.elem != 4 || last.kind != (int)b.src.kind || last.nnz <= 0) return false;
+  const bool same = last.rows == g.rows && last.cols == g.cols && last.nnz == g.nnz;
+  if (same && !last.natural) return false;
+  if (b.sw.fill_direct || b.sw.no_rowsort || b.sw.rowsort_always) return false;
+  if (b.src.kind == QuadSource::FromA) {
+    if (!b.src.from_a->bnd || b.sw.at_buckets) return false;
+  } else if (b.src.kind != QuadSource::Csr) {
+    return false;
+  }
+  if ((size_t)g.nrb + 1 > kPinBlockTable) return false;
+  const int64_t held = (int64_t)(b.buf.ent.cap / sizeof(Ent)) - ENT_SLACK;
+  if (held <= 0 || held >= (int64_t)1 << 34) return false;
+  fc.cap_entries = b.sw.spec_cap >= 0 ? std::min(held, b.sw.spec_cap) : held;
+  fc.total = same ? last.total : (int64_t)((double)g.nnz * ((double)last.total / (double)last.nnz));
+  Counts probe;
+  probe.total = fc.total;
+  probe.nrb = g.nrb;
+  const Fill fill = choose_fill(g, b.src, probe, b.sw).fill;
+  return fill == Fill::Staged || fill == Fill::Gather;
+}
+
 template <typename VT>
 bool build_quads(const CsrView<VT>& S, const QuadGeometry& g, const QuadSource& src, const BuildSwitches& sw, TiledOp& op,
-                 TiledBuffers& buf, hipStream_t s) {
+                 TiledBuffers& buf, hipStream_t s, BuildMode mode) {
   typedef typename EntOf<VT>::type E;
   constexpr bool f32 = sizeof(VT) == 4;
   const Build<VT> b{S, g, src, sw, buf, s};
-  const int32_t* d_seg = index_rows(b);
+  const int32_t* d_seg = index_rows(b, mode == BuildMode::Redo);
   Counts c;
-  if (!count_chunks(b, d_seg, c)) return false;
-  E* d_ent = reinterpret_cast<E*>(buf.ent.ensure((size_t)(c.total + ENT_SLACK) * sizeof(E)));
+  Forecast fc;
+  const bool speculative = mode == BuildMode::Speculate && forecast(b, fc);
+  if (!count_chunks(b, d_seg, c, speculative ? &fc : nullptr)) return false;
+  int64_t* const d_misc = misc_words(buf);
+  int64_t* const pinned = static_cast<int64_t*>(buf.host.p);
+  E* d_ent = c.speculated ? buf.ent.ptr<E>() : reinterpret_cast<E*>(buf.ent.ensure((size_t)(c.total + ENT_SLACK) * sizeof(E)));
+  if (c.speculated) c.total = c.cap_entries;
   publish(op, g, c, d_ent);
-  const bool dq_ok = fork_dq_tables<VT>(op, buf, s);
+  bool dq_ok = fork_dq_tables<VT>(op, buf, s);
+  if (c.speculated) c.total = fc.total;
+  if (c.speculated && !dq_ok) {
+    SAPCA_HIP(hipEventSynchronize(buf.counted));
+    c.speculated = false;
+    c.rows_in_disorder = src.kind == QuadSource::FromA && pinned[kPinMisc + kMiscDisorder] != 0;
+    c.max_chunk = pinned[kPinMisc + kMiscMaxChunk];
+    c.total = pinned[kPinMisc + kMiscTotal];
+    if ((pinned[kPinMisc + kMiscVerdict] & 2) != 0) return build_quads<VT>(S, g, src, sw, op, buf, s, BuildMode::Redo);
+    d_ent = reinterpret_cast<E*>(buf.ent.ensure((size_t)(c.total + ENT_SLACK) * sizeof(E)));
+    publish(op, g, c, d_ent);
+    dq_ok = fork_dq_tables<VT>(op, buf, s);
+  }
   if (f32 && !dq_ok && (g.block_rows > 512 || c.max_chunk > g.stage_cap)) {
     SAPCA_HIP(hipStreamWaitEvent(s, buf.aux_join, 0));
     return false;
   }
   const FillChoice f = choose_fill(g, src, c, sw);
-  if (f.fill != Fill::Direct) SAPCA_HIP(hipMemsetAsync(d_ent + c.total, 0, (size_t)ENT_SLACK * sizeof(E), s));
-  else SAPCA_HIP(hipMemsetAsync(d_ent, 0, (size_t)(c.total + ENT_SLACK) * sizeof(E), s));
-  launch_fill<VT>(b, c, d_seg, f, d_ent);
+  const int64_t* const skip = c.speculated ? d_misc + kMiscVerdict : nullptr;
+  if (!c.speculated) {
+    if (f.fill != Fill::Direct) SAPCA_HIP(hipMemsetAsync(d_ent + c.total, 0, (size_t)ENT_SLACK * sizeof(E), s));
+    else SAPCA_HIP(hipMemsetAsync(d_ent, 0, (size_t)(c.total + ENT_SLACK) * sizeof(E), s));
+  }
+  launch_fill<VT>(b, c, d_seg, f, d_ent, skip);
   SAPCA_HIP(hipGetLastError());
   if (f32) SAPCA_HIP(hipStreamWaitEvent(s, buf.aux_join, 0));
+  TiledBuffers::LastBuild& last = buf.last;
+  if (c.speculated) {
+    SAPCA_HIP(hipEventSynchronize(buf.counted));
+    if (pinned[kPinMisc + kMiscVerdict] != 0) {
+      if (sw.debug) fprintf(stderr, "sapca: build_tiled speculation refused (verdict %lld): counting again\n", (long long)pinned[kPinMisc + kMiscVerdict]);
+      op = TiledOp();
+      return build_quads<VT>(S, g, src, sw, op, buf, s, BuildMode::Redo);
+    }
+    op.total_entries = c.total = pinned[kPinMisc + kMiscTotal];
+    op.max_chunk = c.max_chunk = pinned[kPinMisc + kMiscMaxChunk];
+    if (sw.debug) fprintf(stderr, "sapca: build_tiled speculation held (total %lld, forecast %lld, capacity %lld)\n", (long long)c.total,
+                          (long long)fc.total, (long long)c.cap_entries);
+  }
+  last.valid = true;
+  last.natural = c.d_perm == nullptr && !c.rows_in_disorder;
+  last.kind = (int)src.kind; last.elem = g.elem;
+  last.rows = g.rows; last.cols = g.cols; last.nnz = g.nnz; last.total = c.total;
   op.valid = true;
   return true;
 }
 
 template <typename VT>
-bool build_tiled_t(const CsrView<VT>& S, int ldp_elems, TiledOp& op, TiledBuffers& buf, hipStream_t s, const QuadSource& src) {
+bool build_tiled_t(const CsrView<VT>& S, int ldp_elems, TiledOp& op, TiledBuffers& buf, hipStream_t s, const QuadSource& src, bool speculate) {
   SAPCA_CHECK(ldp_elems == 64, SAPCA_ERR_ARG, "tiled sweep: panels must have 64 columns");
   SAPCA_CHECK(src.kind != QuadSource::FromA, SAPCA_ERR_ARG, "tiled sweep: the A -> A^T route starts in build_tiled_at_direct");
   op = TiledOp();
   const BuildSwitches sw{};
   const QuadGeometry g = quad_geometry(S.rows, S.cols, S.nnz, (int)sizeof(VT), ldp_elems, sw);
-  return eligible(g, src) && build_quads<VT>(S, g, src, sw, op, buf, s);
-}
-
-}
-
-bool build_tiled(const CsrView<float>& S, int ldp, TiledOp& op, TiledBuffers& buf, hipStream_t s, const QuadSource& src) {
-  return build_tiled_t<float>(S, ldp, op, buf, s, src);
-}
-bool build_tiled(const CsrView<double>& S, int ldp, TiledOp& op, TiledBuffers& buf, hipStream_t s, const QuadSource& src) {
-  return build_tiled_t<double>(S, ldp, op, buf, s, src);
+  return eligible(g, src) && build_quads<VT>(S, g, src, sw, op, buf, s, speculate ? BuildMode::Speculate : BuildMode::Wait);
+}
+
+}
+
+bool build_tiled(const CsrView<float>& S, int ldp, TiledOp& op, TiledBuffers& buf, hipStream_t s, const QuadSource& src, bool speculate) {
+  return build_tiled_t<float>(S, ldp, op, buf, s, src, speculate);
+}
+bool build_tiled(const CsrView<double>& S, int ldp, TiledOp& op, TiledBuffers& buf, hipStream_t s, const QuadSource& src, bool) {
+  return build_tiled_t<double>(S, ldp, op, buf, s, src, false);
 }
 
 bool build_tiled_at_direct(const CsrView<float>& A, int ldp, TiledOp& op, TiledBuffers& buf, int64_t* at_ptr, double* stats,
-                           DevBuf& scratch, hipStream_t s) {
+                           DevBuf& scratch, hipStream_t s, bool speculate) {
   op = TiledOp();
   const BuildSwitches sw{};
   if (sw.at_sort || ldp != 64) return false;
@@ -1489,7 +1603,7 @@
   At.rows = n; At.cols = m; At.nnz = A.nnz; At.ptr = at_ptr; At.idx = nullptr; At.val = nullptr;
   const AtDirectSrc from_a{&A, cnt16, n2, &scratch, stats, bnd, nrb_nat, &blk_nat};
   src.from_a = &from_a;
-  return build_quads<float>(At, g, src, sw, op, buf, s);
+  return build_quads<float>(At, g, src, sw, op, buf, s, speculate ? BuildMode::Speculate : BuildMode::Wait);
 }
 
 void at_stats_index(const int64_t* ptr, const uint64_t* packed, int64_t rows, int64_t cols, int ldp, TiledBuffers& buf,
```

Result: no change. 1371 (-0.2%).
